# safe-autonomous-systems/fluidgym

Measured on AMD Instinct MI355X. Metric: env-steps/sec (batched) + pressure-Poisson HBM GB/s vs roofline, 1/2/4/8 GPUs, higher is better.
Workload: dtype f32; 1 GPU; ChannelJet2D-v0 (2D channel stand-in for 'cylinder Re=100 256x128'), 64 envs/GPU, 25 PISO steps/env step, random jets, stirred by a body force N(0,2.0) redrawn every env step; global_batch=64, parallelism=env-sharded x1, 1 bcast + 1 all_gather per step (RCCL), lanes_per_gpu=2, workload_modified=True, capped_solves=0, floor_released_solves=0, advection_solver_form=two-brick, velocity_solver=on-chip Jacobi sweeps (policy advection_jacobi; 11972 solves settled by

## Files before the change

### fluidgym_amd/csrc/fg_api.hip

```cpp
#include <stdio.h>
#include <string.h>

#include <cmath>
#include <string>
#include <vector>

#include <stdlib.h>

#include "fg_internal.h"
#include "fg_bicg.h"

static thread_local std::string g_last_error;
void fg_set_error(const std::string& msg) { g_last_error = msg; }

extern "C" int fg_abi_version(void) { return FG_ABI_VERSION; }
extern "C" const char* fg_last_error(void) { return g_last_error.c_str(); }

static FgBounds make_bounds(const fg_state* s, int channel) {
    FgBounds b;
    for (int f = 0; f < 6; ++f) {
        b.vel[f] = s->bvel[f];
        b.scal[f] = s->bscal[f];
        b.scalar_bc[f] = s->cfg.scalar_bc[f][channel < 0 ? 0 : channel];
    }
    return b;
}

static int check_bound(const fg_state* s, bool need_scalar) {
    FG_REQUIRE(s->velocity && s->pressure, FG_ERR_NOT_BOUND, "velocity/pressure not bound (fg_bind)");
    for (int f = 0; f < 2 * s->grid.dims; ++f) {
        if (!s->grid.fixed[f]) continue;
        FG_REQUIRE(s->bvel[f], FG_ERR_NOT_BOUND, "boundary velocity of a FIXED face not bound");
        if (need_scalar) FG_REQUIRE(s->bscal[f], FG_ERR_NOT_BOUND, "boundary scalar of a FIXED face not bound");
    }
    if (need_scalar) FG_REQUIRE(s->scalar, FG_ERR_NOT_BOUND, "passive scalar not bound");
    return FG_OK;
}

extern "C" int fg_create(const fg_config* cfg, const fg_real* hx, const fg_real* hy, const fg_real* hz, fg_handle* out) {
    FG_REQUIRE(cfg && out && hx && hy, FG_ERR_INVALID_ARG, "fg_create: null argument");
    FG_REQUIRE(cfg->dims == 2 || cfg->dims == 3, FG_ERR_INVALID_ARG, "dims must be 2 or 3");
    FG_REQUIRE(cfg->dims == 2 || hz, FG_ERR_INVALID_ARG, "hz required in 3-D");
    FG_REQUIRE(cfg->nx >= 3 && cfg->ny >= 3 && (cfg->dims == 2 ? cfg->nz == 1 : cfg->nz >= 3), FG_ERR_INVALID_ARG,
               "block needs >= 3 cells per axis (nz = 1 in 2-D)");
    FG_REQUIRE(cfg->batch >= 1, FG_ERR_INVALID_ARG, "batch must be >= 1");
    FG_REQUIRE(cfg->n_scalars >= 0 && cfg->n_scalars <= FG_MAX_SCALARS, FG_ERR_INVALID_ARG, "bad n_scalars");
    for (int a = 0; a < cfg->dims; ++a)
        FG_REQUIRE(cfg->face_type[2 * a] == cfg->face_type[2 * a + 1], FG_ERR_INVALID_ARG,
                   "a FIXED face needs a FIXED partner (CloseBoundary closes both, domain_structs.cpp:1981-2002)");
    FG_REQUIRE((long long)cfg->nx * cfg->ny * cfg->nz * cfg->batch * 6 < (1LL << 31), FG_ERR_UNSUPPORTED,
               "index space exceeds int32 (reference index_t is int32 as well)");
    FG_HIP_CHECK(hipSetDevice(cfg->device));

    fg_state* s = new fg_state();
    memset(s, 0, sizeof(*s));
    fg_switches_read(s);
    s->cfg = *cfg;
    FgGrid& g = s->grid;
    g.dims = cfg->dims; g.nx = cfg->nx; g.ny = cfg->ny; g.nz = cfg->nz;
    g.n = cfg->nx * cfg->ny * cfg->nz; g.B = cfg->batch;
    for (int f = 0; f < 6; ++f) g.fixed[f] = (f < 2 * cfg->dims) ? (cfg->face_type[f] == FG_FIXED) : 0;
    s->vec = (!FG_F64 && cfg->nx % 4 == 0) ? 4 : 1;
    s->viscosity = 0.f;

    const fg_real* hsrc[3] = {hx, hy, hz};
    const int hn[3] = {cfg->nx, cfg->ny, cfg->nz};
    for (int a = 0; a < 3; ++a) {
        std::vector<fg_real> h(hn[a], 1.f), rh(hn[a], 1.f);
        if (a < cfg->dims)
            for (int i = 0; i < hn[a]; ++i) {
                if (!(hsrc[a][i] > 0.f)) { delete s; fg_set_error("cell widths must be positive"); return FG_ERR_INVALID_ARG; }
                h[i] = hsrc[a][i]; rh[i] = 1.f / hsrc[a][i];
            }
        FG_HIP_CHECK(hipMalloc(&s->d_h[a], sizeof(fg_real) * hn[a]));
        FG_HIP_CHECK(hipMalloc(&s->d_rh[a], sizeof(fg_real) * hn[a]));
        FG_HIP_CHECK(hipMemcpy(s->d_h[a], h.data(), sizeof(fg_real) * hn[a], hipMemcpyHostToDevice));
        FG_HIP_CHECK(hipMemcpy(s->d_rh[a], rh.data(), sizeof(fg_real) * hn[a], hipMemcpyHostToDevice));
        g.h[a] = s->d_h[a]; g.rh[a] = s->d_rh[a];
    }
    const size_t BN = (size_t)g.B * g.n, d = g.dims;
    auto alloc = [&](fg_real** p, size_t count) -> hipError_t {
        hipError_t e = hipMalloc(p, sizeof(fg_real) * count);
        if (e == hipSuccess) e = hipMemset(*p, 0, sizeof(fg_real) * count);
        return e;
    };
    FG_HIP_CHECK(alloc(&s->A, BN));
    FG_HIP_CHECK(alloc(&s->rA, BN));
    FG_HIP_CHECK(alloc(&s->Coff, BN * 2 * d));
    FG_HIP_CHECK(alloc(&s->adv_rhs, BN * d));
    FG_HIP_CHECK(alloc(&s->vel_result, BN * d));
    FG_HIP_CHECK(alloc(&s->hvec, BN * d));
    FG_HIP_CHECK(alloc(&s->div, BN));
    FG_HIP_CHECK(alloc(&s->p_result, BN));
    FG_HIP_CHECK(alloc(&s->scal_result, BN));
    for (int i = 0; i < 8; ++i) FG_HIP_CHECK(alloc(&s->w[i], BN * d));
    const size_t nsys = (size_t)g.B * d;
    FG_HIP_CHECK(hipMalloc(&s->acc, sizeof(FgDacc) * nsys * FG_ACC_DOUBLES));
    FG_HIP_CHECK(hipMemset(s->acc, 0, sizeof(FgDacc) * nsys * FG_ACC_DOUBLES));
    FG_HIP_CHECK(hipMalloc(&s->flags, sizeof(int32_t) * nsys));
    FG_HIP_CHECK(hipMalloc(&s->info_dev, sizeof(fg_solve_info) * nsys));
    FG_HIP_CHECK(hipHostMalloc(&s->info_pinned, sizeof(fg_solve_info) * nsys));
    FG_HIP_CHECK(hipHostMalloc(&s->flags_pinned, sizeof(int32_t) * nsys));
    FG_HIP_CHECK(alloc(&s->scratch_B, (size_t)g.B * (4 + 2 * d)));
    FG_HIP_CHECK(hipMalloc(&s->d_bvel_ptrs, sizeof(fg_real*) * 6));
    FG_HIP_CHECK(hipMemset(s->d_bvel_ptrs, 0, sizeof(fg_real*) * 6));
    FG_HIP_CHECK(hipHostMalloc(&s->diag_pinned, sizeof(fg_real) * 2 * g.B));
    FG_HIP_CHECK(hipHostMalloc(&s->dt_pinned, sizeof(fg_real) * g.B));
    FG_HIP_CHECK(alloc(&s->dt_dev, g.B));
    FG_HIP_CHECK(hipMalloc(&s->env_sel_dev, sizeof(fg_env_sel) * g.B));
    s->t_rem_dev = nullptr;
#if !FG_F64
    FG_HIP_CHECK(hipMalloc(&s->t_rem_dev, sizeof(double) * g.B));
    FG_HIP_CHECK(hipMemset(s->t_rem_dev, 0, sizeof(double) * g.B));
#endif
    if (int rc = fg_poll_create(&s->poll, (int)(nsys > 2 * (size_t)g.B ? nsys : 2 * (size_t)g.B))) return rc;
    for (int k = 0; k < 4; ++k) { s->pred_bicg[k] = 2; s->pred_cg[k] = 1; }
    s->wall_forcing_axis = -1;
    s->ref64_inner = 1e-4f;
    s->fd_row_epoch = -1; s->rA_epoch = 0; s->fd_row_part_epoch = -1;
    for (int k = 0; k < 4; ++k) s->jac_hist[k] = FgJacHist{0, 0, 0};
    s->jac_solves = s->jac_fallbacks = 0;
    FG_HIP_CHECK(hipHostMalloc(&s->jac_prev, sizeof(float) * 4 * nsys));
    s->jac_rA_epoch = -1;
    FG_HIP_CHECK(hipMalloc(&s->fcg_alpha, sizeof(double) * 2 * (size_t)g.B));
    FG_HIP_CHECK(hipMemset(s->fcg_alpha, 0, sizeof(double) * 2 * (size_t)g.B));
    FG_HIP_CHECK(hipMalloc(&s->fcg_xsum, sizeof(FgDacc) * 2 * (size_t)g.B));
    FG_HIP_CHECK(hipMemset(s->fcg_xsum, 0, sizeof(FgDacc) * 2 * (size_t)g.B));
    FG_HIP_CHECK(hipMalloc(&s->fcg_lazy, sizeof(int32_t) * (size_t)g.B));
    FG_HIP_CHECK(hipMemset(s->fcg_lazy, 0, sizeof(int32_t) * (size_t)g.B));
    s->cg_return_best = 1;
    s->cg_reset_steps = 100;
    s->adv_from_result = 1;
    FG_HIP_CHECK(hipMalloc(&s->cg_acc, sizeof(FgDacc) * (size_t)g.B * 8 * 64));
    FG_HIP_CHECK(hipMemset(s->cg_acc, 0, sizeof(FgDacc) * (size_t)g.B * 8 * 64));
    FG_HIP_CHECK(hipMalloc(&s->cg_best.best_crit, sizeof(fg_real) * g.B));
    FG_HIP_CHECK(hipMalloc(&s->cg_best.saved_crit, sizeof(fg_real) * g.B));
    FG_HIP_CHECK(hipMalloc(&s->cg_best.save_at, sizeof(int32_t) * g.B));
    FG_HIP_CHECK(alloc(&s->cg_best.best_x, BN));
    *out = s;
    return FG_OK;
}

extern "C" int fg_destroy(fg_handle s) {
    if (!s) return FG_OK;
    for (int a = 0; a < 3; ++a) { (void)hipFree(s->d_h[a]); (void)hipFree(s->d_rh[a]); }
    fg_real* owned[] = {s->A, s->rA, s->Coff, s->adv_rhs, s->vel_result, s->hvec, s->div, s->p_result, s->scal_result,
                      s->scratch_B};
    for (fg_real* p : owned) (void)hipFree(p);
    for (int i = 0; i < 8; ++i) (void)hipFree(s->w[i]);
    (void)hipFree(s->acc); (void)hipFree(s->flags); (void)hipFree(s->info_dev);
    (void)hipHostFree(s->info_pinned); (void)hipHostFree(s->flags_pinned);
    fg_prof_destroy(s);
    fg_poll_destroy(&s->poll);
    (void)hipFree(s->d_bvel_ptrs); (void)hipHostFree(s->diag_pinned); (void)hipHostFree(s->dt_pinned); (void)hipFree(s->dt_dev); (void)hipFree(s->t_rem_dev); (void)hipFree(s->env_sel_dev);
    float* fd[] = {s->fd_Qx, s->fd_QxT, s->fd_Qz, s->fd_QzT, s->fd_lower, s->fd_inv, s->fd_cp};
    for (float* p : fd) if (p) (void)hipFree(p);
    if (s->fd_dct_tw) { (void)hipFree(s->fd_dct_tw); (void)hipFree(s->fd_dct_rot); }
    (void)hipFree(s->cg_acc); (void)hipFree(s->fcg_alpha); (void)hipFree(s->fcg_xsum); (void)hipFree(s->fcg_lazy);
    if (s->jac_prev) (void)hipHostFree(s->jac_prev);
    (void)hipFree(s->fd_row_part); (void)hipFree(s->fd_lam_x); (void)hipFree(s->fd_row_inv); (void)hipFree(s->fd_row_cp); (void)hipFree(s->fd_row_lower);
    (void)hipFree(s->line_inv); (void)hipFree(s->line_cp); (void)hipFree(s->ilu_d);
    (void)hipFree(s->r64_buf); (void)hipFree(s->r64_acc); (void)hipFree(s->ref64_x); (void)hipFree(s->force_uniform);
    (void)hipFree(s->fd_lam); (void)hipFree(s->helm_diag); (void)hipFree(s->helm_lower); (void)hipFree(s->helm_upper); (void)hipFree(s->helm_tmp); (void)hipFree(s->helm_lower_row); (void)hipFree(s->helm_lower_row2); (void)hipFree(s->line_inv2); (void)hipFree(s->line_cp2);
    (void)hipFree(s->cg_best.best_crit); (void)hipFree(s->cg_best.saved_crit); (void)hipFree(s->cg_best.save_at); (void)hipFree(s->cg_best.best_x);
    delete s;
    return FG_OK;
}

static int sync_bvel_ptrs(fg_state* s);
extern "C" int fg_bind(fg_handle s, int field, fg_real* ptr) {
    FG_REQUIRE(s, FG_ERR_INVALID_ARG, "null handle");
    if (field == FG_VELOCITY) s->velocity = ptr;
    else if (field == FG_PRESSURE) s->pressure = ptr;
    else if (field == FG_SCALAR) s->scalar = ptr;
    else if (field == FG_VELOCITY_SOURCE) s->velocity_source = ptr;
    else if (field == FG_VISCOSITY_FIELD) s->visc_field = ptr;
    else if (field >= FG_BOUND_VELOCITY && field < FG_BOUND_VELOCITY + 6) {
        s->bvel[field - FG_BOUND_VELOCITY] = ptr;
        return sync_bvel_ptrs(s);
    }
    else if (field >= FG_BOUND_SCALAR && field < FG_BOUND_SCALAR + 6) s->bscal[field - FG_BOUND_SCALAR] = ptr;
    else FG_REQUIRE(false, FG_ERR_INVALID_ARG, "fg_bind: unknown field id");
    return FG_OK;
}

extern "C" int fg_set_viscosity(fg_handle s, fg_real v) {
    FG_REQUIRE(s, FG_ERR_INVALID_ARG, "null handle");
    s->viscosity = v;
    return FG_OK;
}
extern "C" int fg_set_scalar_viscosity(fg_handle s, int ch, fg_real v) {
    FG_REQUIRE(s && ch >= 0 && ch < FG_MAX_SCALARS, FG_ERR_INVALID_ARG, "bad channel");
    s->scalar_viscosity[ch] = v;
    s->scalar_viscosity_set = true;
    return FG_OK;
}
extern "C" int fg_set_viscosity_batch(fg_handle s, const fg_real* nu_B) {
    FG_REQUIRE(s, FG_ERR_INVALID_ARG, "null handle");
    s->viscosity_B = nu_B;
    s->helm_pre_mask = 0;
    return FG_OK;
}
extern "C" int fg_set_scalar_viscosity_batch(fg_handle s, int ch, const fg_real* k_B) {
    FG_REQUIRE(s && ch >= 0 && ch < FG_MAX_SCALARS, FG_ERR_INVALID_ARG, "bad channel");
    s->scalar_viscosity_B[ch] = k_B;
    s->helm_pre_mask = 0;
    return FG_OK;
}

extern "C" int fg_set_fd_preconditioner(fg_handle s, const float* Qx, const float* QxT, const float* Qz, const float* QzT,
                                        const float* lower, const float* inv, const float* cp) {
    FG_REQUIRE(s && Qx && QxT && lower && inv && cp, FG_ERR_INVALID_ARG, "null argument");
    FG_REQUIRE(s->grid.fixed[2] && s->grid.fixed[3], FG_ERR_UNSUPPORTED, "FD preconditioner needs FIXED y faces");
    FG_REQUIRE(s->grid.dims == 2 || (Qz && QzT), FG_ERR_INVALID_ARG, "Qz required in 3-D");
#if !FG_F64
    FG_REQUIRE(s->grid.ny <= 640, FG_ERR_UNSUPPORTED, "FD preconditioner: at most 640 cells along y (LDS of the tridiagonal solve)");
#endif
    const size_t nx = s->grid.nx, ny = s->grid.ny, nz = s->grid.nz;
    auto up = [&](float** dst, const float* src, size_t count) -> hipError_t {
        if (*dst) (void)hipFree(*dst);
        hipError_t e = hipMalloc(dst, sizeof(float) * count);
        if (e == hipSuccess) e = hipMemcpy(*dst, src, sizeof(float) * count, hipMemcpyHostToDevice);
        return e;
    };
    FG_HIP_CHECK(up(&s->fd_Qx, Qx, nx * nx));
    FG_HIP_CHECK(up(&s->fd_QxT, QxT, nx * nx));
    if (s->grid.dims == 3) {
        FG_HIP_CHECK(up(&s->fd_Qz, Qz, nz * nz));
        FG_HIP_CHECK(up(&s->fd_QzT, QzT, nz * nz));
    }
    FG_HIP_CHECK(up(&s->fd_lower, lower, ny));
    FG_HIP_CHECK(up(&s->fd_inv, inv, nx * ny * nz));
    FG_HIP_CHECK(up(&s->fd_cp, cp, nx * ny * nz));
    s->fd_dct_x = 0;
    return FG_OK;
}

extern "C" int fg_set_return_best(fg_handle s, int on) {
    FG_REQUIRE(s, FG_ERR_INVALID_ARG, "null handle");
    s->cg_return_best = on ? 1 : 0;
    return FG_OK;
}

extern "C" int fg_set_cg_reset_steps(fg_handle s, int steps) {
    FG_REQUIRE(s && steps >= 0, FG_ERR_INVALID_ARG, "fg_set_cg_reset_steps: null handle or negative step count");
    s->cg_reset_steps = steps;
    return FG_OK;
}

extern "C" int fg_set_advection_start(fg_handle s, int from_result) {
    FG_REQUIRE(s, FG_ERR_INVALID_ARG, "null handle");
    s->adv_from_result = from_result ? 1 : 0;
    return FG_OK;
}

extern "C" int fg_set_wall_stress_forcing(fg_handle s, int axis, fg_real coef_lo, fg_real coef_hi) {
    FG_REQUIRE(s, FG_ERR_INVALID_ARG, "null handle");
    FG_REQUIRE(axis < s->grid.dims, FG_ERR_INVALID_ARG, "fg_set_wall_stress_forcing: bad axis");
    if (axis >= 0) {
        FG_REQUIRE(s->grid.fixed[2] && s->grid.fixed[3], FG_ERR_UNSUPPORTED, "fg_set_wall_stress_forcing: needs FIXED y faces (walls)");
        if (!s->force_uniform) {
            FG_HIP_CHECK(hipMalloc(&s->force_uniform, sizeof(fg_real) * (size_t)s->grid.B * s->grid.dims));
            FG_HIP_CHECK(hipMemset(s->force_uniform, 0, sizeof(fg_real) * (size_t)s->grid.B * s->grid.dims));
        }
    }
    s->wall_forcing_axis = axis; s->wall_forcing_coef[0] = coef_lo; s->wall_forcing_coef[1] = coef_hi;
    return FG_OK;
}

extern "C" int fg_set_advection_preconditioner(fg_handle s, int mode) {
    FG_REQUIRE(s, FG_ERR_INVALID_ARG, "null handle");
    FG_REQUIRE(mode >= 0 && mode <= 5, FG_ERR_INVALID_ARG, "fg_set_advection_preconditioner: mode must be 0 (off), 1 (line, always), 2 (line, fallback), 3 (Helmholtz, always), 4 (ILU(0), always) or 5 (ILU(0), fallback)");
    FG_REQUIRE(mode != 3 || s->fd_lam != nullptr, FG_ERR_INVALID_ARG, "fg_set_advection_preconditioner: mode 3 needs fg_set_fd_helmholtz");
    if (mode >= 4) { if (int rc = fg_ilu_alloc(s)) return rc; }
    else if (mode != 0)
        if (int rc = fg_line_alloc(s)) return rc;
    s->adv_precond = mode;
    return FG_OK;
}
extern "C" int fg_set_advection_jacobi(fg_handle s, int on) {
    FG_REQUIRE(s, FG_ERR_INVALID_ARG, "null handle");
    if (!s->adv_jacobi_env) s->adv_jacobi = on ? 1 : 0;
    for (int k = 0; k < 4; ++k) s->jac_hist[k] = FgJacHist{0, 0, 0};
    return FG_OK;
}
extern "C" int fg_advection_jacobi_counts(fg_handle s, int64_t* out2) {
    FG_REQUIRE(s && out2, FG_ERR_INVALID_ARG, "null argument");
    out2[0] = s->jac_solves; out2[1] = s->jac_fallbacks;
    return FG_OK;
}
extern "C" int fg_set_double_fallback(fg_handle s, int on) {
    FG_REQUIRE(s, FG_ERR_INVALID_ARG, "null handle");
    s->double_fallback = on ? 1 : 0;
    return FG_OK;
}
extern "C" int fg_ladder(fg_handle s, int64_t* out4, int32_t force_mask) {
    FG_REQUIRE(s && out4, FG_ERR_INVALID_ARG, "null argument");
    for (int k = 0; k < 4; ++k) out4[k] = s->rung_count[k];
    if (force_mask >= 0) s->ladder_force = force_mask;
    return FG_OK;
}
namespace {
struct FormsRecord {
    fg_state* s; int32_t* out; int32_t rec[FG_FORM_SLOTS] = {0};
    FormsRecord(fg_state* st, int32_t* o) : s(st), out(o) { s->forms_rec = rec; }
    ~FormsRecord() {
        s->forms_rec = nullptr;
        if (out) memcpy(out, rec, sizeof(rec));
    }
};
}

extern "C" int fg_debug_apply_preconditioner(fg_handle s, int mode, int nc, const fg_real* r, fg_real* z, int32_t* forms_out, void* stream) {
    FG_REQUIRE(s && r && z && nc >= 1 && nc <= s->grid.dims && (mode == 1 || mode == 3 || mode == 4), FG_ERR_INVALID_ARG,
               "fg_debug_apply_preconditioner: mode 1 (y-line), 3 (Helmholtz) or 4 (ILU(0)), 1 <= nc <= dims");
    hipStream_t st = (hipStream_t)stream;
    FormsRecord forms(s, forms_out);
    s->prepared.clear();
    FG_HIP_CHECK(hipMemsetAsync(s->flags, 0, sizeof(int32_t) * (size_t)s->grid.B * s->grid.dims, st));
    if (mode == 3) {
        FG_REQUIRE(s->fd_lam != nullptr, FG_ERR_UNSUPPORTED, "fg_debug_apply_preconditioner: mode 3 needs fg_set_fd_helmholtz (fp32 build)");
        FG_REQUIRE(s->adv_last_dt != nullptr, FG_ERR_INVALID_ARG, "fg_debug_apply_preconditioner: mode 3 needs a velocity fg_setup_advection first");
        if (int rc = fg_helm_factor(s, s->adv_last_dt, fg_nu(s), 1, 1, nc, st)) return rc;
        if (int rc = fg_fd_helmholtz_apply(s, nc, r, z, st)) return rc;
    } else if (mode == 4) {
// ... 147 lines not shown
            if (int rc = fg_launch_wall_forcing(s, (hipStream_t)stream)) return rc;
        a.force = s->wall_forcing_axis >= 0 ? s->force_uniform : nullptr;
        a.visc = s->visc_field;
        a.nu = fg_nu(s);
        a.rA = s->rA;
        s->adv_last_dt = dt_B;
        s->rA_epoch++;
        s->jac_rA_epoch = s->rA_epoch;
#if !FG_F64
        if (fg_fd_rowmean_ok(s) && s->vec == 4 && (s->grid.nx & 63) == 0) {
            if (!s->fd_row_part) FG_HIP_CHECK(hipMalloc(&s->fd_row_part, sizeof(float) * (size_t)s->grid.B * s->grid.ny * (s->grid.nx / 64)));
            a.row_part = s->fd_row_part;
            s->fd_row_part_epoch = s->rA_epoch;
        }
#endif
        if (buoy_axis >= 0) {
            a.buoy_T = s->scalar; a.buoy_stride = (long)s->cfg.n_scalars * s->grid.n; a.buoy_axis = buoy_axis; a.buoy_factor = buoy_factor;
            a.source_w = s->velocity_source;
        }
    }
    return fg_launch_adv_build(s, make_bounds(s, channel), a, (hipStream_t)stream);
}

static int advection_solve(fg_state* s, FgBicgArgs a, fg_solve_info* info, hipStream_t st, int for_scalar = 0, int channel = 0, bool* spec_ran = nullptr);

extern "C" int fg_solve_advection(fg_handle s, int for_scalar, int channel, fg_real tol, int max_iterations,
                                  fg_solve_info* info_host, void* stream) {
    FG_REQUIRE(s, FG_ERR_INVALID_ARG, "null handle");
    FgBicgArgs a;
    a.diag = s->A; a.off = s->Coff; a.rhs = s->adv_rhs;
    a.dt = s->cur_dt;
    a.tol = tol; a.max_iterations = max_iterations;
    if (for_scalar) { a.x = s->scal_result; a.nc = 1; a.use_x0 = 0; a.kind = 0; }
    else { a.x = s->vel_result; a.nc = s->grid.dims; a.use_x0 = s->adv_from_result; }
    return advection_solve(s, a, info_host, (hipStream_t)stream, for_scalar, channel);
}

extern "C" int fg_copy_scalar_result_to_blocks(fg_handle s, int channel, void* stream) {
    FG_REQUIRE(s && s->scalar, FG_ERR_NOT_BOUND, "scalar not bound");
    const int n = s->grid.n;
    if (s->cfg.n_scalars == 1) return fg_launch_copy_active(s, s->cur_dt, s->scal_result, s->scalar, 1, (hipStream_t)stream);
    FG_HIP_CHECK(hipMemcpy2DAsync(s->scalar + (size_t)channel * n, sizeof(fg_real) * n * s->cfg.n_scalars, s->scal_result,
                                  sizeof(fg_real) * n, sizeof(fg_real) * n, s->grid.B, hipMemcpyDeviceToDevice,
                                  (hipStream_t)stream));
    return FG_OK;
}

extern "C" int fg_setup_pressure_matrix(fg_handle s, void* stream) {
    FG_REQUIRE(s, FG_ERR_INVALID_ARG, "null handle");
    s->rA_epoch++;
    return fg_launch_pressure_setup(s, s->cur_dt, (hipStream_t)stream);
}

extern "C" int fg_setup_pressure_rhs(fg_handle s, const fg_real* dt_B, void* stream) {
    FG_REQUIRE(s && dt_B, FG_ERR_INVALID_ARG, "null argument");
    if (int rc = check_bound(s, false)) return rc;
    hipStream_t st = (hipStream_t)stream;
    if (int rc = fg_launch_h(s, dt_B, s->vel_result, st)) return rc;
    return fg_launch_div(s, make_bounds(s, 0), dt_B, s->hvec, s->div, st);
}

struct SpecH { fg_state* s; const fg_real* dt; const fg_step_options* opt; hipStream_t st; };
static int spec_h(void* p) {
    const SpecH* c = static_cast<const SpecH*>(p);
    fg_state* s = c->s;
    if (int rc = fg_launch_h(s, c->dt, s->vel_result, c->st)) return rc;
    return fg_launch_div(s, make_bounds(s, 0), c->dt, s->hvec, s->div, c->st, !c->opt->pressure_warm_start,
                         c->opt->pressure_method == FG_SOLVER_FDCG && s->fd_Qx != nullptr);
}

static int launch_corrector(fg_state* s, const fg_real* dt, const FgCgOutcome& o, bool last, hipStream_t st) {
    const bool mean_folded = last && o.mean_ready;
    FG_REQUIRE(!o.lazy_z || !last || mean_folded, FG_ERR_UNSUPPORTED, "fg_piso_step: an unmaterialised pressure without its folded mean");
    if (last && !mean_folded)
        if (int rc = fg_launch_mean_sub(s, dt, s->p_result, s->pressure, st)) return rc;
    const FgMeanRef mean = {s->fcg_xsum, s->info_dev, s->pressure, o.marks_valid ? s->fcg_lazy : nullptr, s->fcg_alpha};
    const FgLazyRef lazy = {s->fcg_lazy, s->fcg_alpha, last ? s->p_result : nullptr};
    const fg_real* p = o.lazy_z ? o.lazy_z : ((last && !mean_folded) ? s->pressure : s->p_result);
    return fg_launch_correct(s, dt, s->rA, s->hvec, p, s->vel_result, st, last ? s->velocity : nullptr, mean_folded ? &mean : nullptr, o.lazy_z ? &lazy : nullptr);
}

struct SpecCorrect { fg_state* s; const fg_real* dt; bool last; hipStream_t st; };
static int spec_correct(void* p, const FgCgOutcome& o) {
    const SpecCorrect* c = static_cast<const SpecCorrect*>(p);
    return launch_corrector(c->s, c->dt, o, c->last, c->st);
}

static int solve_pressure(fg_state* s, const fg_real* dt, int method, fg_real tol, int max_iterations, int use_previous,
                          fg_solve_info* info_host, hipStream_t st, bool finalize = true, int kind = 2, FgCgOutcome* out = nullptr,
                          FgCgSpec spec = FgCgSpec{}) {
    int rc = FG_OK;
    FgCgOutcome own;
    if (!out) out = &own;
    if (method == FG_SOLVER_CG || method == FG_SOLVER_FDCG) {
        FgCgArgs a;
        a.rA = s->rA; a.b = s->div; a.x = s->p_result;
        a.r = s->w[0]; a.p = s->w[1]; a.Ap = s->w[2];
        a.dt = dt; a.tol = tol; a.max_iterations = max_iterations; a.use_x0 = use_previous;
        a.reset_steps = s->cg_reset_steps;
        a.precond = (method == FG_SOLVER_FDCG);
        a.kind = kind;
        a.check_every = a.precond ? 2 : 16;
        a.lazy_ok = finalize ? 0 : 1;
        a.spec = spec;
#if !FG_F64
        if (s->ref64_outer > 0) a.lazy_ok = 0;
#endif
        rc = fg_cg_solve(s, a, info_host, st, out);
#if !FG_F64
        if (s->ref64_outer > 0 && (rc == FG_OK || rc == FG_ERR_NOT_CONVERGED)) rc = fg_refine64_pressure(s, a, info_host, st, out);
        if (s->double_fallback && (rc == FG_ERR_NOT_FINITE || (s->ladder_force & 2))) {
            std::vector<fg_solve_info> tmp;
            fg_solve_info* info = info_host;
            if (!info) { tmp.assign(s->info_pinned, s->info_pinned + s->grid.B); info = tmp.data(); }
            s->rung_count[2] += 1;
            rc = fg_rung64_cg(s, a, info, (s->ladder_force & 2) != 0, st, out);
        }
#endif
    } else {
        fg_set_error("fg_solve_pressure: only FG_SOLVER_CG drives the PISO step (Jacobi/RBGS are smoothers)");
        return FG_ERR_UNSUPPORTED;
    }
    if (rc != FG_OK && rc != FG_ERR_NOT_CONVERGED) return rc;
    if (finalize)
        if (int rc2 = fg_launch_mean_sub(s, dt, s->p_result, s->pressure, st)) return rc2;
    return rc;
}

extern "C" int fg_solve_pressure(fg_handle s, int method, fg_real tol, int max_iterations, int use_previous,
                                 fg_solve_info* info_host, void* stream) {
    FG_REQUIRE(s, FG_ERR_INVALID_ARG, "null handle");
    if (int rc = check_bound(s, false)) return rc;
    return solve_pressure(s, s->cur_dt, method, tol, max_iterations, use_previous, info_host, (hipStream_t)stream);
}

extern "C" int fg_set_pressure_refinement(fg_handle s, int32_t max_corrections, fg_real target_tol, fg_real inner_relative_tol) {
    FG_REQUIRE(s, FG_ERR_INVALID_ARG, "null handle");
    FG_REQUIRE(!FG_F64 || max_corrections <= 0, FG_ERR_UNSUPPORTED, "fg_set_pressure_refinement: the fp64 build solves in fp64 already");
    FG_REQUIRE(max_corrections <= 0 || (target_tol > 0 && inner_relative_tol > 0 && inner_relative_tol < 1), FG_ERR_INVALID_ARG,
               "fg_set_pressure_refinement: tolerances must be positive, the relative one below 1");
    s->ref64_outer = max_corrections > 0 ? max_corrections : 0;
    s->ref64_tol = (float)target_tol; s->ref64_inner = (float)inner_relative_tol;
    return FG_OK;
}

extern "C" int fg_correct_velocity(fg_handle s, void* stream) {
    FG_REQUIRE(s, FG_ERR_INVALID_ARG, "null handle");
    if (int rc = check_bound(s, false)) return rc;
    return fg_launch_correct(s, s->cur_dt, s->rA, s->hvec, s->pressure, s->vel_result, (hipStream_t)stream);
}

extern "C" int fg_copy_velocity_result_to_blocks(fg_handle s, void* stream) {
    FG_REQUIRE(s && s->velocity, FG_ERR_NOT_BOUND, "velocity not bound");
    return fg_launch_copy_active(s, s->cur_dt, s->vel_result, s->velocity, s->grid.dims, (hipStream_t)stream);
}
extern "C" int fg_copy_velocity_result_from_blocks(fg_handle s, void* stream) {
    FG_REQUIRE(s && s->velocity, FG_ERR_NOT_BOUND, "velocity not bound");
    return fg_launch_copy_active(s, nullptr, s->velocity, s->vel_result, s->grid.dims, (hipStream_t)stream);
}

static int max_iters(const fg_solve_info* info, int n) {
    int m = -1;
    for (int i = 0; i < n; ++i) m = info[i].used_iterations > m ? info[i].used_iterations : m;
    return m;
}

static int advection_solve(fg_state* s, FgBicgArgs a, fg_solve_info* info, hipStream_t st, int for_scalar, int channel, bool* spec_ran) {
    a.precond = (s->adv_precond == 1) ? 1 : (s->adv_precond == 3 ? 2 : (s->adv_precond == 4 ? 3 : 0));
    if (a.precond == 2 && !for_scalar && s->visc_field) a.precond = 0;
    if (a.precond == 2) {
        a.nu = fg_nu(s, for_scalar, channel);
        a.wall_lo = for_scalar ? (s->cfg.scalar_bc[2][channel] == FG_DIRICHLET) : 1;
        a.wall_hi = for_scalar ? (s->cfg.scalar_bc[3][channel] == FG_DIRICHLET) : 1;
    }
    const int nsys = s->grid.B * a.nc;
    std::vector<fg_solve_info> info_own;
    if (!info) { info_own.resize(nsys); info = info_own.data(); }
    int rc = fg_bicgstab_solve(s, a, info, st, spec_ran);
    bool failed = (rc == FG_ERR_NOT_CONVERGED || rc == FG_ERR_NOT_FINITE) || (s->ladder_force & 1);
#if !FG_F64
    if (failed && s->double_fallback && rc != FG_ERR_HIP) {
        s->rung_count[0] += 1;
        rc = fg_rung64_bicgstab(s, a, info, (s->ladder_force & 1) != 0, st);
        if (rc != FG_OK && rc != FG_ERR_NOT_CONVERGED && rc != FG_ERR_NOT_FINITE) return rc;
        failed = (rc != FG_OK) || (s->ladder_force & 4);
    }
#endif
    if (failed && (s->adv_precond == 2 || s->adv_precond == 5)) {
        s->line_retries += 1;
        s->rung_count[1] += 1;
        a.precond = s->adv_precond == 5 ? 3 : 1; a.use_x0 = 0;
        rc = fg_bicgstab_solve(s, a, info, st);
    }
    (void)nsys;
    return rc;
}

extern "C" int fg_piso_step(fg_handle s, const fg_real* dt_B, const fg_step_options* opt, int32_t* stats_host,
                            void* stream) {
    FG_REQUIRE(s && dt_B && opt, FG_ERR_INVALID_ARG, "null argument");
    const bool scalar = opt->advect_scalar && s->cfg.n_scalars > 0;
    if (int rc = check_bound(s, scalar)) return rc;
    FG_REQUIRE(opt->buoyancy_axis < s->grid.dims, FG_ERR_INVALID_ARG, "bad buoyancy axis");
    FG_REQUIRE(opt->buoyancy_axis < 0 || (s->velocity_source && s->scalar), FG_ERR_NOT_BOUND,
               "buoyancy needs velocity source and scalar bound");
    hipStream_t st = (hipStream_t)stream;
    const int B = s->grid.B, d = s->grid.dims;
    std::vector<fg_solve_info> info((size_t)B * d);
    int32_t stats[4] = {-1, -1, -1, -1};
    struct DropHelmRecord { fg_state* s; ~DropHelmRecord() { s->helm_pre_mask = 0; } } drop_helm_record{s};
    int status = FG_OK;
    auto soft = [&](int rc) {
        if (rc == FG_ERR_NOT_CONVERGED) { status = rc; return FG_OK; }
        return rc;
    };
#if !FG_F64
    const bool sweeps_first = s->adv_linesweep && s->grid.dims == 2 && s->jac_hist[0].skip == 0 && s->jac_hist[1].skip == 0;
    if (scalar && s->cfg.n_scalars == 1 && s->adv_precond == 3 && s->fd_lam && !s->visc_field && !sweeps_first) {
        const FgNu nu2[2] = {fg_nu(s, 1, 0), fg_nu(s)};
        const int wlo[2] = {s->cfg.scalar_bc[2][0] == FG_DIRICHLET, 1}, whi[2] = {s->cfg.scalar_bc[3][0] == FG_DIRICHLET, 1};
        if (int rc = fg_helm_factor_pair(s, dt_B, nu2, wlo, whi, st)) return rc;
    }
#endif
    if (scalar) {
        FgRange range_scalar("scalar_advection");
        for (int ch = 0; ch < s->cfg.n_scalars; ++ch) {
            if (int rc = fg_setup_advection(s, dt_B, 1, ch, stream)) return rc;
            FgBicgArgs a;
            a.diag = s->A; a.off = s->Coff; a.rhs = s->adv_rhs; a.x = s->scal_result; a.nc = 1;
            a.dt = dt_B; a.tol = opt->advection_tol; a.max_iterations = opt->max_iterations; a.use_x0 = 0; a.kind = 0;
            if (int rc = soft(advection_solve(s, a, info.data(), st, 1, ch))) return rc;
            const int m = max_iters(info.data(), B);
            stats[0] = m > stats[0] ? m : stats[0];
            s->ctr.add(0, info.data(), B);
            const int n = s->grid.n;
            if (s->cfg.n_scalars == 1) {
                if (int rc = fg_launch_copy_active(s, dt_B, s->scal_result, s->scalar, 1, st)) return rc;
            } else {
                (void)n;
                fg_set_error("multi-channel scalar copy with inactive envs not implemented");
                return FG_ERR_UNSUPPORTED;
            }
        }
    }
    fg_range_push("velocity_assembly_and_solve");
    struct PopOnce { bool armed = true; void fire() { if (armed) { fg_range_pop(); armed = false; } } ~PopOnce() { fire(); } } range_velocity;
    if (int rc = setup_advection(s, dt_B, 0, 0, stream, opt->buoyancy_axis, opt->buoyancy_factor)) return rc;
    bool h_div_ran = false;
    {
        FgBicgArgs a;
        a.diag = s->A; a.off = s->Coff; a.rhs = s->adv_rhs; a.x = s->vel_result; a.nc = d;
        a.dt = dt_B; a.tol = opt->advection_tol; a.max_iterations = opt->max_iterations; a.use_x0 = s->adv_from_result;
        SpecH spec_h_ctx = {s, dt_B, opt, st};
        if (opt->corrector_steps > 0) a.spec = FgSpecHook{spec_h, &spec_h_ctx};
        if (int rc = soft(advection_solve(s, a, info.data(), st, 0, 0, &h_div_ran))) return rc;
        stats[1] = max_iters(info.data(), B * d);
        s->ctr.add(1, info.data(), B * d);
    }
    range_velocity.fire();
    for (int c = 0; c < opt->corrector_steps; ++c) {
        FgRange range_corr(c == 0 ? "pressure_corrector_0" : "pressure_corrector_1+");
        const bool last = (c + 1 == opt->corrector_steps);
        if (!(c == 0 && h_div_ran)) {
            if (int rc = fg_launch_h(s, dt_B, s->vel_result, st)) return rc;
            if (int rc = fg_launch_div(s, make_bounds(s, 0), dt_B, s->hvec, s->div, st, !opt->pressure_warm_start,
                                       opt->pressure_method == FG_SOLVER_FDCG && s->fd_Qx != nullptr))
                return rc;
        }
        SpecCorrect spec_ctx = {s, dt_B, last, st};
        FgCgOutcome outcome;
        if (int rc = soft(solve_pressure(s, dt_B, opt->pressure_method, opt->pressure_tol, opt->max_iterations, opt->pressure_warm_start ? 1 : 0,
                                         info.data(), st, false, c == 0 ? 0 : 1, &outcome, FgCgSpec{spec_correct, &spec_ctx})))
            return rc;
        if (c < 2) { stats[2 + c] = max_iters(info.data(), B); s->ctr.add(2 + c, info.data(), B); }
        if (!outcome.spec_done)
            if (int rc = launch_corrector(s, dt_B, outcome, last, st)) return rc;
    }
    if (opt->corrector_steps <= 0)
        if (int rc = fg_launch_copy_active(s, dt_B, s->vel_result, s->velocity, d, st)) return rc;
    if (stats_host) memcpy(stats_host, stats, sizeof(stats));
    s->ctr.piso_steps += 1;
    return status;
}

extern "C" int fg_config_dump(fg_handle s, char* buf, int n) {
    FG_REQUIRE(s && buf && n > 0, FG_ERR_INVALID_ARG, "fg_config_dump: bad argument");
    std::string out = std::string("{\"build\": \"") + (FG_F64 ? "f64" : "f32") + "\"";
    fg_switches_json(s, out);
    const std::pair<const char*, long long> state[] = {
        {"fast_transform_x", s->fd_dct_x}, {"fd_preconditioner", s->fd_Qx ? 1 : 0}, {"helmholtz", s->fd_lam ? 1 : 0}, {"advection_preconditioner", s->adv_precond},
        {"advection_from_result", s->adv_from_result}, {"return_best", s->cg_return_best}, {"cg_reset_steps", s->cg_reset_steps}, {"double_fallback", s->double_fallback},
        {"wall_forcing_axis", s->wall_forcing_axis}, {"first_iterate_polls", s->fcg_first_polls}, {"unstored_pressure_solves", s->fcg_unstored},
        {"jacobi_speculation_misses", s->jac_spec_missed}, {"jacobi_floor_released", s->jac_floor_released}, {"pressure_refinement_corrections", s->ref64_corrections}};
    for (const auto& kv : state) fg_json_put(out, kv.first, kv.second);
    return fg_json_out(out + "}", buf, n);
}

extern "C" int fg_solver_unconverged(fg_handle s, int64_t* out4) {
    FG_REQUIRE(s != nullptr && out4 != nullptr, FG_ERR_INVALID_ARG, "fg_solver_unconverged: bad argument");
    for (int k = 0; k < 4; ++k) out4[k] = s->ctr.unconv[k];
    return FG_OK;
}

extern "C" int fg_solver_counters(fg_handle s, int64_t* out13, int32_t reset) {
    FG_REQUIRE(s != nullptr, FG_ERR_INVALID_ARG, "fg_solver_counters: null handle");
    if (out13) s->ctr.write(out13);
    if (reset) s->ctr.reset();
    return FG_OK;
}

extern "C" int fg_single_step(fg_handle s, const fg_sim_options* o, int32_t* out, fg_real* flux_host, void* stream);
extern "C" int fg_multi_step(fg_handle s, const fg_sim_options* o, int32_t n, const fg_real* const* bvel_schedule, int32_t* out_6n,
                             fg_real* flux_host, int32_t* steps_done, void* stream) {
    FG_REQUIRE(s && o && out_6n && n >= 0, FG_ERR_INVALID_ARG, "fg_multi_step: bad argument");
    if (steps_done) *steps_done = 0;
    for (int k = 0; k < n; ++k) {
        if (bvel_schedule)
            for (int f = 0; f < 2 * s->grid.dims; ++f)
                if (const fg_real* p = bvel_schedule[(size_t)k * 6 + f])
                    if (int rc = fg_bind(s, FG_BOUND_VELOCITY + f, const_cast<fg_real*>(p))) return rc;
        if (int rc = fg_single_step(s, o, out_6n + 6 * (size_t)k, flux_host, stream)) return rc;
        if (steps_done) *steps_done = k + 1;
        if (out_6n[6 * (size_t)k + 5] == 0 && !s->cg_return_best) break;
    }
    return FG_OK;
}

static inline bool is_close_zero(double a) { return std::fabs(a) <= 1e-8; }

extern "C" int fg_single_step(fg_handle s, const fg_sim_options* o, int32_t* out, fg_real* flux_host, void* stream) {
    fg_htrace("single_step_in");
    FgRange range_sim("fg_single_step");
    FG_REQUIRE(s && o && out, FG_ERR_INVALID_ARG, "null argument");
    if (int rc = check_bound(s, o->step.advect_scalar && s->cfg.n_scalars > 0)) return rc;
    hipStream_t st = (hipStream_t)stream;
    const int B = s->grid.B;
    const FgBounds bnd = make_bounds(s, 0);
    std::vector<double> t_rem(B, (double)o->time_step);
    int32_t stats[4] = {-1, -1, -1, -1};
    int substeps = 0, all_ok = 1;
    bool first = true;
    int fixed_left = o->adaptive ? 0 : (o->substeps > 0 ? o->substeps : 1);
    for (;;) {
        bool any = false;
        if (o->adaptive) {
            for (int b = 0; b < B; ++b) any = any || (t_rem[b] > 0 && !is_close_zero(t_rem[b]));
        } else {
            any = fixed_left > 0;
        }
        if (!any) break;
        auto advance = [&](int b, fg_real max_vel) -> fg_real {
            fg_real ts = 0.f;
            if (!o->adaptive) {
                ts = o->time_step;
            } else if (t_rem[b] > 0 && !is_close_zero(t_rem[b])) {
                const double mv = (double)max_vel;
                const double max_ts = is_close_zero(mv) ? t_rem[b] : (double)o->cfl / mv;
                double tsd;
                if (max_ts >= t_rem[b]) tsd = t_rem[b];
                else tsd = t_rem[b] / (double)(long long)std::ceil(t_rem[b] / max_ts);
                t_rem[b] -= tsd;
                ts = (fg_real)tsd;
            }
            return ts;
        };
        auto flux_guard = [&]() -> int {
            fg_real worst = 0.f;
            for (int b = 0; b < B; ++b) {
                if (flux_host) flux_host[b] = s->diag_pinned[b];
                const fg_real a = std::fabs(s->diag_pinned[b]);
                worst = (a > worst || a != a) ? a : worst;
            }
            if (!(worst <= o->flux_balance_tol)) {
                fg_set_error("Domain boundary fluxes not balanced, cannot proceed with simulation step.");
                return FG_ERR_FLUX_BALANCE;
            }
            return FG_OK;
        };
        bool deferred = false;
        FgPollOut po_cfl = FgPollOut{nullptr, 0};
        if (o->adaptive || first) {
            const FgPollOut po = fg_poll_next(&s->poll);
            po_cfl = po;
            if (first && !o->adaptive) { if (int rc = fg_launch_flux_balance(s, bnd, s->diag_pinned, st, FgPollOut{po.seq, po.value})) return rc; }
            if (o->adaptive) {
                deferred = po.gran != nullptr && s->dev_dt && s->t_rem_dev != nullptr;
                const FgDtRule rule = deferred ? FgDtRule{s->t_rem_dev, s->dt_dev, (float)o->cfl, (double)o->time_step, first ? 1 : 0}
                                               : FgDtRule{nullptr, nullptr, 0.f, 0.0, 0};
                if (int rc = fg_launch_max_velocity(s, bnd, s->scratch_B + B, st, s->diag_pinned + B, po.seq ? FgPollOut{po.seq + B, po.value, po.gran} : po,
                                                    first ? s->scratch_B : nullptr, first ? s->diag_pinned : nullptr, rule))
                    return rc;
            }
            fg_htrace("maxvel_launched");
            if (!deferred) {
                if (o->adaptive && po.gran) {
                    if (int rc = fg_poll_wait_words(&s->poll, po, 12 * B, first ? 2 * B : B, st)) return rc;
                    for (int b = 0; b < B; ++b) {
                        s->diag_pinned[B + b] = fg_poll_word_float(&s->poll, 12 * B + b);
                        if (first) s->diag_pinned[b] = fg_poll_word_float(&s->poll, 13 * B + b);
                    }
                } else if (int rc = fg_poll_wait(&s->poll, po, o->adaptive ? B : 0, o->adaptive ? 1 : B, st)) return rc;
                fg_htrace("maxvel_poll_done");
                if (first) if (int rc = flux_guard()) return rc;
            }
        }
        if (!deferred)
            for (int b = 0; b < B; ++b) s->dt_pinned[b] = advance(b, o->adaptive ? s->diag_pinned[B + b] : (fg_real)0);
        const bool folded = o->outflow_mask && fg_outflow_folds(s, o->outflow_mask);
        const bool dt_by_value = folded && B <= 64 && !deferred;
        if (!dt_by_value && !deferred) FG_HIP_CHECK(hipMemcpyAsync(s->dt_dev, s->dt_pinned, sizeof(fg_real) * B, hipMemcpyHostToDevice, st));
        if (o->outflow_mask) {
            for (int f = 0; f < 2 * s->grid.dims; ++f)
                if ((o->outflow_mask >> f) & 1) FG_REQUIRE(s->grid.fixed[f], FG_ERR_INVALID_ARG, "outflow face is not FIXED");
            if (!folded)
                for (int f = 0; f < 2 * s->grid.dims; ++f)
                    if ((o->outflow_mask >> f) & 1)
                        if (int rc = fg_launch_outflow(s, f, o->outflow_velm[f >> 1], s->dt_dev, st)) return rc;
            fg_real velm3[3] = {o->outflow_velm[0], o->outflow_velm[1], o->outflow_velm[2]};
            if (int rc = fg_launch_balance(s, bnd, o->outflow_mask, (fg_real)0.01 * o->outflow_tol, s->dt_dev, st, folded ? o->outflow_mask : 0, velm3,
                                           dt_by_value ? s->dt_pinned : nullptr))
                return rc;
        }
        int rc = fg_piso_step(s, s->dt_dev, &o->step, stats, stream);
        if (rc == FG_ERR_NOT_CONVERGED) all_ok = 0;
        else if (rc != FG_OK) return rc;
        if (deferred) {
            if (int rc2 = fg_poll_wait_words(&s->poll, po_cfl, 12 * B, first ? 2 * B : B, st)) return rc2;
            for (int b = 0; b < B; ++b) {
                s->diag_pinned[B + b] = fg_poll_word_float(&s->poll, 12 * B + b);
                if (first) s->diag_pinned[b] = fg_poll_word_float(&s->poll, 13 * B + b);
            }
            if (first) if (int rc2 = flux_guard()) return rc2;
            for (int b = 0; b < B; ++b) s->dt_pinned[b] = advance(b, s->diag_pinned[B + b]);
        }
        ++substeps;
        first = false;
        if (!o->adaptive) --fixed_left;
        if (substeps >= (o->max_substeps > 0 ? o->max_substeps : 100000)) break;
    }
    fg_htrace("single_step_out");
    for (int i = 0; i < 4; ++i) out[i] = stats[i];
    out[4] = substeps;
    out[5] = all_ok;
    return FG_OK;
}

extern "C" int fg_make_divergence_free(fg_handle s, fg_real tol, int max_iterations, fg_solve_info* info_host,
                                       void* stream) {
    FG_REQUIRE(s, FG_ERR_INVALID_ARG, "null handle");
    if (int rc = check_bound(s, false)) return rc;
    s->cur_dt = nullptr;
    hipStream_t st = (hipStream_t)stream;
    const size_t BN = (size_t)s->grid.B * s->grid.n;
    std::vector<fg_real> ones(BN, 1.f);
    FG_HIP_CHECK(hipMemcpyAsync(s->rA, ones.data(), sizeof(fg_real) * BN, hipMemcpyHostToDevice, st));
    s->rA_epoch++;
    FG_HIP_CHECK(hipStreamSynchronize(st));
    if (int rc = fg_launch_copy_active(s, nullptr, s->velocity, s->hvec, s->grid.dims, st)) return rc;
    if (int rc = fg_launch_div(s, make_bounds(s, 0), nullptr, s->hvec, s->div, st)) return rc;
    int rc = solve_pressure(s, nullptr, FG_SOLVER_CG, tol, max_iterations, 0, info_host, st);
    if (rc != FG_OK && rc != FG_ERR_NOT_CONVERGED) return rc;
    if (int rc2 = fg_launch_correct(s, nullptr, s->rA, s->hvec, s->pressure, s->vel_result, st)) return rc2;
    if (int rc2 = fg_launch_copy_active(s, nullptr, s->vel_result, s->velocity, s->grid.dims, st)) return rc2;
    return rc;
}

extern "C" int fg_reset_solver_state(fg_handle s, void* stream) {
    FG_REQUIRE(s && s->velocity, FG_ERR_NOT_BOUND, "velocity not bound");
    for (int k = 0; k < 4; ++k) s->jac_hist[k] = FgJacHist{0, 0, 0};
    FG_HIP_CHECK(hipMemsetAsync(s->p_result, 0, sizeof(fg_real) * (size_t)s->grid.B * s->grid.n, (hipStream_t)stream));
    return fg_launch_copy_active(s, nullptr, s->velocity, s->vel_result, s->grid.dims, (hipStream_t)stream);
}

extern "C" int fg_solver_hints(fg_handle s, int32_t* hints12, int32_t set) {
    FG_REQUIRE(s != nullptr && hints12 != nullptr, FG_ERR_INVALID_ARG, "fg_solver_hints: bad argument");
    for (int k = 0; k < 4; ++k) {
        FgJacHist& H = s->jac_hist[k];
        if (set) { H.sweeps = hints12[3 * k]; H.skip = hints12[3 * k + 1]; H.fails = hints12[3 * k + 2]; }
        else { hints12[3 * k] = H.sweeps; hints12[3 * k + 1] = H.skip; hints12[3 * k + 2] = H.fails; }
    }
    return FG_OK;
}

extern "C" int fg_get_buffer(fg_handle s, int which, fg_real** out_ptr, int64_t* out_count) {
    FG_REQUIRE(s && out_ptr && out_count, FG_ERR_INVALID_ARG, "null argument");
    const int64_t BN = (int64_t)s->grid.B * s->grid.n, d = s->grid.dims;
    switch (which) {
        case FG_BUF_A: *out_ptr = s->A; *out_count = BN; break;
        case FG_BUF_C_OFF: *out_ptr = s->Coff; *out_count = BN * 2 * d; break;
        case FG_BUF_ADV_RHS: *out_ptr = s->adv_rhs; *out_count = BN * d; break;
        case FG_BUF_VEL_RESULT: *out_ptr = s->vel_result; *out_count = BN * d; break;
        case FG_BUF_H: *out_ptr = s->hvec; *out_count = BN * d; break;
        case FG_BUF_DIV: *out_ptr = s->div; *out_count = BN; break;
        case FG_BUF_P_RESULT: *out_ptr = s->p_result; *out_count = BN; break;
        case FG_BUF_SCALAR_RESULT: *out_ptr = s->scal_result; *out_count = BN; break;
        default:
            if (which >= 100 && which < 108) { *out_ptr = s->w[which - 100]; *out_count = BN * d; break; }
            FG_REQUIRE(false, FG_ERR_INVALID_ARG, "unknown buffer id");
    }
    return FG_OK;
}

extern "C" int fg_read_buffer(fg_handle s, int which, fg_real* dst, void* stream) {
    fg_real* src = nullptr;
    int64_t count = 0;
    if (int rc = fg_get_buffer(s, which, &src, &count)) return rc;
    FG_REQUIRE(dst, FG_ERR_INVALID_ARG, "null destination");
    FG_HIP_CHECK(hipMemcpyAsync(dst, src, sizeof(fg_real) * count, hipMemcpyDeviceToDevice, (hipStream_t)stream));
    return FG_OK;
}

extern "C" int fg_poisson_apply(fg_handle s, const fg_real* rA, const fg_real* x, fg_real* y, void* stream) {
    FG_REQUIRE(s && rA && x && y, FG_ERR_INVALID_ARG, "null argument");
    return fg_poisson_apply_launch(s, rA, x, y, (hipStream_t)stream);
}

extern "C" int fg_poisson_jacobi(fg_handle s, const fg_real* rA, const fg_real* b, fg_real* x, int n_sweeps, fg_real omega,
                                 void* stream) {
    FG_REQUIRE(s && rA && b && x && n_sweeps >= 0, FG_ERR_INVALID_ARG, "bad argument");
    hipStream_t st = (hipStream_t)stream;
    fg_real* buf[2] = {x, s->w[5]};
    for (int i = 0; i < n_sweeps; ++i)
        if (int rc = fg_poisson_jacobi_launch(s, rA, b, buf[i & 1], buf[(i + 1) & 1], omega, st)) return rc;
    if (n_sweeps & 1)
        FG_HIP_CHECK(hipMemcpyAsync(x, s->w[5], sizeof(fg_real) * (size_t)s->grid.B * s->grid.n, hipMemcpyDeviceToDevice, st));
    return FG_OK;
}

extern "C" int fg_poisson_rbgs(fg_handle s, const fg_real* rA, const fg_real* b, fg_real* x, int n_sweeps, fg_real omega,
                               void* stream) {
    FG_REQUIRE(s && rA && b && x && n_sweeps >= 0, FG_ERR_INVALID_ARG, "bad argument");
    hipStream_t st = (hipStream_t)stream;
    for (int i = 0; i < n_sweeps; ++i) {
        if (int rc = fg_poisson_rbgs_launch(s, rA, b, x, omega, 0, st)) return rc;
        if (int rc = fg_poisson_rbgs_launch(s, rA, b, x, omega, 1, st)) return rc;
    }
    return FG_OK;
}

extern "C" int fg_poisson_cg(fg_handle s, const fg_real* rA, const fg_real* b, fg_real* x, fg_real tol, int max_iterations,
                             int use_x0, fg_solve_info* info_host, void* stream) {
    FG_REQUIRE(s && rA && b && x, FG_ERR_INVALID_ARG, "null argument");
    FgCgArgs a;
    a.rA = rA; a.b = b; a.x = x;
    a.r = s->w[0]; a.p = s->w[1]; a.Ap = s->w[2];
    a.dt = nullptr; a.tol = tol; a.max_iterations = max_iterations; a.use_x0 = use_x0;
    a.reset_steps = 100;
    a.precond = 0;
    a.check_every = (tol > 0.f) ? 16 : (1 << 30);
    return fg_cg_solve(s, a, info_host, (hipStream_t)stream);
}

extern "C" int fg_poisson_fdcg(fg_handle s, const fg_real* rA, const fg_real* b, fg_real* x, fg_real tol, int max_iterations,
                               int use_x0, fg_solve_info* info_host, void* stream) {
    FG_REQUIRE(s && rA && b && x, FG_ERR_INVALID_ARG, "null argument");
    FgCgArgs a;
    a.rA = rA; a.b = b; a.x = x;
    a.r = s->w[0]; a.p = s->w[1]; a.Ap = s->w[2];
    a.dt = nullptr; a.tol = tol; a.max_iterations = max_iterations; a.use_x0 = use_x0;
    a.reset_steps = 0;
    a.precond = 1;
    a.check_every = (tol > 0.f) ? 2 : (1 << 30);
    return fg_cg_solve(s, a, info_host, (hipStream_t)stream);
}

extern "C" int fg_coords_to_transforms(const float* coords, float* transforms, int dims, int nx, int ny, int nz,
                                       void* stream) {
    FG_REQUIRE(coords && transforms && (dims == 2 || dims == 3), FG_ERR_INVALID_ARG, "bad argument");
#if FG_F64
    fg_set_error("fg_coords_to_transforms is an fp32 entry point: use libfluidgym_hip.so");
    return FG_ERR_UNSUPPORTED;
#else
    return fg_metrics_launch(coords, transforms, dims, nx, ny, nz, (hipStream_t)stream);
#endif
}
```

### fluidgym_amd/csrc/fg_envrestore.hip

```cpp
#include <vector>

#include "fg_internal.h"

namespace {

constexpr int ER_TX = 64, ER_TY = 4, ER_PASSES = 4, ER_ROWS = ER_TY * ER_PASSES;

template <typename T>
__global__ __launch_bounds__(ER_TX * ER_TY) void k_env_restore(T* __restrict__ dst, const T* __restrict__ bank,
                                                               const fg_env_sel* __restrict__ sel, int C, int ez, int ey, int ex,
                                                               int tiles_x, int signed_components) {
    const fg_env_sel r = sel[blockIdx.y];
    const int tx = (int)(blockIdx.x % (unsigned)tiles_x), rg = (int)(blockIdx.x / (unsigned)tiles_x);
    const int rows = C * ez * ey;
    const size_t per_env = (size_t)rows * ex;
    T* __restrict__ d = dst + (size_t)r.env * per_env;
    const T* __restrict__ b = bank + (size_t)r.src * per_env;
    const int x = tx * ER_TX + (int)threadIdx.x;
    int xs = x - r.shift_x;
    if (xs < 0) xs += ex;
    if (r.flip_x) xs = ex - 1 - xs;
#pragma unroll
    for (int k = 0; k < ER_PASSES; ++k) {
        const int row = rg * ER_ROWS + k * ER_TY + (int)threadIdx.y;
        if (x < ex && row < rows) {
            const int y = row % ey, cz = row / ey;
            const int z = cz % ez, c = cz / ez;
            int zs = z - r.shift_z;
            if (zs < 0) zs += ez;
            if (r.flip_z) zs = ez - 1 - zs;
            const T v = b[((size_t)(c * ez + zs) * ey + y) * ex + xs];
            const bool neg = signed_components && ((c == 0 && r.flip_x) || (c == 2 && r.flip_z));
            d[(size_t)row * ex + x] = neg ? -v : v;
        }
    }
}

template <typename T>
__global__ __launch_bounds__(256) void k_env_reset_solver(const T* __restrict__ velocity, T* __restrict__ vel_result,
                                                          T* __restrict__ p_result, const fg_env_sel* __restrict__ sel, long n, int dims) {
    const int env = sel[blockIdx.y].env;
    const long dn = (long)dims * n;
    const T* __restrict__ u = velocity + (size_t)env * dn;
    T* __restrict__ ur = vel_result + (size_t)env * dn;
    T* __restrict__ pr = p_result + (size_t)env * n;
#pragma unroll
    for (int k = 0; k < 4; ++k) {
        const long i = ((long)blockIdx.x * 4 + k) * 256 + threadIdx.x;
        if (i < dn) ur[i] = u[i];
        if (i < n) pr[i] = (T)0;
    }
}

int check_envs(const fg_state* s, const fg_env_sel* sel, int32_t n_sel, const char* who) {
    const int B = s->grid.B;
    FG_REQUIRE(sel != nullptr, FG_ERR_INVALID_ARG, std::string(who) + ": null selection");
    FG_REQUIRE(n_sel >= 1 && n_sel <= B, FG_ERR_INVALID_ARG, std::string(who) + ": n_sel must be in 1..batch");
    FG_REQUIRE(n_sel <= 65535, FG_ERR_UNSUPPORTED, std::string(who) + ": at most 65535 envs per call");
    std::vector<char> seen((size_t)B, 0);
    for (int i = 0; i < n_sel; ++i) {
        FG_REQUIRE(sel[i].env >= 0 && sel[i].env < B, FG_ERR_INVALID_ARG, std::string(who) + ": env index out of range");
        FG_REQUIRE(!seen[sel[i].env], FG_ERR_INVALID_ARG, std::string(who) + ": an env is named twice");
        seen[sel[i].env] = 1;
    }
    return FG_OK;
}

}

extern "C" int fg_env_restore_field(fg_handle s, int which_field, const fg_real* bank, int32_t S, const fg_env_sel* sel, int32_t n_sel,
                                    int32_t signed_components, void* stream) {
    FG_REQUIRE(s != nullptr, FG_ERR_INVALID_ARG, "fg_env_restore_field: null handle");
    FG_REQUIRE(bank != nullptr && S >= 1, FG_ERR_INVALID_ARG, "fg_env_restore_field: null bank or S < 1");
    if (int rc = check_envs(s, sel, n_sel, "fg_env_restore_field")) return rc;
    const FgGrid& g = s->grid;
    fg_real* dst = nullptr;
    int C = 0, vector_field = 0, ext[3] = {g.nx, g.ny, g.nz};
    if (which_field == FG_VELOCITY) { dst = s->velocity; C = g.dims; vector_field = 1; }
    else if (which_field == FG_PRESSURE) { dst = s->pressure; C = 1; }
    else if (which_field == FG_SCALAR) { dst = s->scalar; C = s->cfg.n_scalars; }
    else if (which_field == FG_VELOCITY_SOURCE) { dst = s->velocity_source; C = g.dims; vector_field = 1; }
    else if (which_field >= FG_BOUND_VELOCITY && which_field < FG_BOUND_VELOCITY + 2 * g.dims) {
        const int f = which_field - FG_BOUND_VELOCITY;
        dst = s->bvel[f]; C = g.dims; vector_field = 1; ext[f >> 1] = 1;
    } else if (which_field >= FG_BOUND_SCALAR && which_field < FG_BOUND_SCALAR + 2 * g.dims) {
        const int f = which_field - FG_BOUND_SCALAR;
        dst = s->bscal[f]; C = s->cfg.n_scalars; ext[f >> 1] = 1;
    } else FG_REQUIRE(false, FG_ERR_INVALID_ARG, "fg_env_restore_field: unknown field id");
    FG_REQUIRE(signed_components == 0 || (signed_components == 1 && vector_field), FG_ERR_INVALID_ARG,
               "fg_env_restore_field: signed_components is 0, or 1 on a vector field");
    const bool x_periodic = !g.fixed[0] && !g.fixed[1], z_periodic = g.dims == 3 && !g.fixed[4] && !g.fixed[5];
    for (int i = 0; i < n_sel; ++i) {
        const fg_env_sel& r = sel[i];
        FG_REQUIRE(r.src >= 0 && r.src < S, FG_ERR_INVALID_ARG, "fg_env_restore_field: src index out of range");
        FG_REQUIRE((r.flip_x | 1) == 1 && (r.flip_z | 1) == 1, FG_ERR_INVALID_ARG, "fg_env_restore_field: a flip is 0 or 1");
        FG_REQUIRE(g.dims == 3 || (r.flip_z == 0 && r.shift_z == 0), FG_ERR_INVALID_ARG, "fg_env_restore_field: flip_z / shift_z on a 2-D grid");
        FG_REQUIRE(r.shift_x >= 0 && r.shift_x < g.nx && r.shift_z >= 0 && r.shift_z < g.nz, FG_ERR_INVALID_ARG,
                   "fg_env_restore_field: a shift must be in [0, n)");
        FG_REQUIRE(x_periodic || (r.flip_x == 0 && r.shift_x == 0), FG_ERR_INVALID_ARG, "fg_env_restore_field: flip / shift along x, which has FIXED faces");
        FG_REQUIRE(g.dims == 2 || z_periodic || (r.flip_z == 0 && r.shift_z == 0), FG_ERR_INVALID_ARG,
                   "fg_env_restore_field: flip / shift along z, which has FIXED faces");
    }
    FG_REQUIRE(dst != nullptr && C > 0, FG_ERR_NOT_BOUND, "fg_env_restore_field: the field is not bound");
    hipStream_t st = (hipStream_t)stream;
    FG_HIP_CHECK(hipMemcpyAsync(s->env_sel_dev, sel, sizeof(fg_env_sel) * n_sel, hipMemcpyHostToDevice, st));
    const int ex = ext[0], ey = ext[1], ez = ext[2];
    const int tiles_x = (ex + ER_TX - 1) / ER_TX;
    const long row_groups = ((long)C * ez * ey + ER_ROWS - 1) / ER_ROWS;
    hipLaunchKernelGGL(k_env_restore<fg_real>, dim3((unsigned)(tiles_x * row_groups), (unsigned)n_sel), dim3(ER_TX, ER_TY), 0, st, dst, bank,
                       (const fg_env_sel*)s->env_sel_dev, C, ez, ey, ex, tiles_x, (int)signed_components);
    FG_HIP_CHECK(hipGetLastError());
    return FG_OK;
}

extern "C" int fg_env_reset_solver_state(fg_handle s, const fg_env_sel* sel, int32_t n_sel, void* stream) {
    FG_REQUIRE(s != nullptr, FG_ERR_INVALID_ARG, "fg_env_reset_solver_state: null handle");
    if (int rc = check_envs(s, sel, n_sel, "fg_env_reset_solver_state")) return rc;
    FG_REQUIRE(s->velocity != nullptr, FG_ERR_NOT_BOUND, "velocity not bound");
    hipStream_t st = (hipStream_t)stream;
    FG_HIP_CHECK(hipMemcpyAsync(s->env_sel_dev, sel, sizeof(fg_env_sel) * n_sel, hipMemcpyHostToDevice, st));
    const long n = s->grid.n, dn = n * s->grid.dims;
    hipLaunchKernelGGL(k_env_reset_solver<fg_real>, dim3((unsigned)((dn + 1023) / 1024), (unsigned)n_sel), dim3(256), 0, st,
                       (const fg_real*)s->velocity, s->vel_result, s->p_result, (const fg_env_sel*)s->env_sel_dev, n, s->grid.dims);
    FG_HIP_CHECK(hipGetLastError());
    return FG_OK;
}

extern "C" int fg_mb_env_restore_field(fg_mb_handle, int, const fg_real*, int32_t, const fg_env_sel*, int32_t, int32_t, void*) {
    fg_set_error("fg_mb_env_restore_field: a multi-block handle has no per-env restore");
    return FG_ERR_UNSUPPORTED;
}

extern "C" int fg_mb_env_reset_solver_state(fg_mb_handle, const fg_env_sel*, int32_t, void*) {
    fg_set_error("fg_mb_env_reset_solver_state: a multi-block handle has no per-env restore");
    return FG_ERR_UNSUPPORTED;
}
```

### fluidgym_amd/csrc/fg_internal.h

```cpp
#pragma once
#include <hip/hip_runtime.h>
#include <hip/hip_ext.h>
#include <math.h>
#include <stdint.h>
#include <cstring>
#include <string>
#include <type_traits>

#include "../../include/fluidgym_hip.h"
#include "fg_switches.h"

#ifdef FG_REAL_DOUBLE
struct alignas(16) fg_real4 { double x, y, z, w; };
__host__ __device__ __forceinline__ fg_real4 make_fg_real4(double x, double y, double z, double w) { fg_real4 r; r.x = x; r.y = y; r.z = z; r.w = w; return r; }
#define FG_F64 1
#define FG_FMAX fmax
#define FG_FABS fabs
#define FG_SQRT sqrt
#else
typedef float4 fg_real4;
#define make_fg_real4 make_float4
#define FG_F64 0
#define FG_FMAX fmaxf
#define FG_FABS fabsf
// ... 473 lines not shown
__device__ __forceinline__ void fg_poll_publish_infos(const FgPollOut& p, fg_solve_info* mirror, const fg_solve_info* info, int sys, bool valid,
                                                      int first, int n, uint32_t* stage) {
    if (p.gran) {
        uint32_t w[2] = {0u, 0u};
        if (valid) { const fg_solve_info v = info[sys]; w[0] = __float_as_uint((float)v.final_residual); w[1] = fg_info_word(v); }
        fg_poll_publish_records<2>(p, first, n, sys - first, w, valid, stage);
    } else if (valid) {
        mirror[sys] = info[sys];
        fg_poll_publish(p, sys);
    }
}
__device__ __forceinline__ void fg_poll_publish_infos_waves(const FgPollOut& p, fg_solve_info* mirror, const fg_solve_info* info, int sys, bool valid,
                                                            int first, int n, uint32_t* stage) {
    if (mirror) fg_poll_publish_infos(p, mirror, info, sys, valid && (threadIdx.x & 63) == 0, first, n, stage);
}
__device__ __forceinline__ void fg_poll_publish(const FgPollOut& p, int i) {
    if (p.seq) __hip_atomic_store(p.seq + i, p.value, __ATOMIC_RELEASE, __HIP_MEMORY_SCOPE_SYSTEM);
}
#endif
struct FgPoll {
    int32_t* seq;
    int n; int32_t epoch; int spin, words;
    unsigned long long* gran; int n_gran;
};
int fg_poll_create(FgPoll* P, int n);
void fg_poll_destroy(FgPoll* P);
FgPollOut fg_poll_next(FgPoll* P);
int fg_poll_wait(FgPoll* P, const FgPollOut& out, int first, int count, hipStream_t st);
int fg_poll_wait_words(FgPoll* P, const FgPollOut& out, int first, int count, hipStream_t st);
int fg_poll_wait_infos(FgPoll* P, const FgPollOut& out, int first, int count, fg_solve_info* pinned, hipStream_t st);
int fg_poll_wait_active(FgPoll* P, const FgPollOut& out, int first, int count, fg_solve_info* pinned, hipStream_t st);
struct fg_state;
int fg_solve_infos_settle(fg_state* s, int count, bool fresh, hipStream_t st);
int fg_solve_infos_report(const fg_state* s, int count, fg_solve_info* info_host, int* used_max);
inline uint32_t fg_poll_word(const FgPoll* P, int i) { return (uint32_t)(__atomic_load_n(P->gran + i, __ATOMIC_RELAXED) & 0xffffffffull); }
inline float fg_poll_word_float(const FgPoll* P, int i) { const uint32_t u = fg_poll_word(P, i); float f; memcpy(&f, &u, 4); return f; }
inline void fg_poll_info(const FgPoll* P, int sys, fg_solve_info* out) {
    const uint32_t w = fg_poll_word(P, 2 * sys + 1);
    out->final_residual = fg_poll_word_float(P, 2 * sys);
    out->used_iterations = (int32_t)(w >> 2) - 1; out->converged = (w >> 1) & 1; out->is_finite = w & 1;
}
void fg_htrace(const char* tag);
void fg_range_push(const char* name);
void fg_range_pop();
struct FgRange { explicit FgRange(const char* name) { fg_range_push(name); } ~FgRange() { fg_range_pop(); } FgRange(const FgRange&) = delete; FgRange& operator=(const FgRange&) = delete; };

struct FgBest {
    fg_real* best_crit;
    fg_real* saved_crit;
    int32_t* save_at;
    fg_real* best_x;
};
#ifdef __HIPCC__
__device__ __forceinline__ void fg_best_decide(const FgBest& best, int b, fg_real crit, int it) {
    if (it >= 1 && crit < 0.5f * best.best_crit[b]) {
        best.best_crit[b] = crit;
        best.saved_crit[b] = crit;
        best.save_at[b] = it;
    }
}
#endif

struct FgCounters {
    long long sum[4] = {0, 0, 0, 0}, n[4] = {0, 0, 0, 0}, piso_steps = 0;
    long long unconv[4] = {0, 0, 0, 0};
    int max[4] = {0, 0, 0, 0};
    void add(int kind, const fg_solve_info* info, int count) {
        for (int i = 0; i < count; ++i) {
            const int it = info[i].used_iterations;
            if (it < 0 && info[i].final_residual == 0.f) continue;
            const int v = it + 1;
            sum[kind] += v; n[kind] += 1; max[kind] = v > max[kind] ? v : max[kind];
            if (!info[i].converged) unconv[kind] += 1;
        }
    }
    void reset() { *this = FgCounters(); }
    void write(int64_t* out) const {
        for (int k = 0; k < 4; ++k) { out[k] = sum[k]; out[4 + k] = n[k]; out[8 + k] = max[k]; }
        out[12] = piso_steps;
    }
};

struct FgPrepared {
    int bicg_nc; const fg_real* bicg_dt;
    int cg_ns, cg_best; const fg_real* cg_dt;
    int cg_start;
    void clear() { *this = FgPrepared{}; }
    void set_bicg(int nc, const fg_real* dt) { clear(); bicg_nc = nc; bicg_dt = dt; }
    void set_cg(int ns, int best, const fg_real* dt) { clear(); cg_ns = ns; cg_best = best; cg_dt = dt; }
    bool cg_for(const fg_real* dt) const { return cg_ns > 0 && cg_dt == dt; }
    void set_cg_start(int form) { cg_start = form; }
    bool take_bicg(int nc, const fg_real* dt) { const bool ready = bicg_nc == nc && bicg_dt == dt; clear(); return ready; }
    int take_cg(int ns, int best, const fg_real* dt) {
        const int got = (cg_ns == ns && cg_best == best && cg_dt == dt) ? cg_start : -1; clear(); return got;
    }
};

struct FgNu {
    fg_real v = 0; const fg_real* per_env = nullptr;
#ifdef __HIPCC__
    __device__ __forceinline__ fg_real at(int b) const { return per_env ? per_env[b] : v; }
#endif
    bool same(const FgNu& o) const { return v == o.v && per_env == o.per_env; }
};

struct fg_state {
    fg_config cfg;
    FgGrid grid;
    int vec;
    fg_real viscosity;
    fg_real scalar_viscosity[FG_MAX_SCALARS];
    bool scalar_viscosity_set;
    const fg_real* viscosity_B;
    const fg_real* scalar_viscosity_B[FG_MAX_SCALARS];
    fg_real* d_h[3];
    fg_real* d_rh[3];
    fg_real* velocity;
    fg_real* pressure;
    fg_real* scalar;
    fg_real* velocity_source;
    fg_real* visc_field;
    fg_real* bvel[6];
    fg_real* bscal[6];
    fg_real* A;
    fg_real* rA;
    fg_real* Coff;
    fg_real* adv_rhs;
    fg_real* vel_result;
    fg_real* hvec;
    fg_real* div;
    fg_real* p_result;
    fg_real* scal_result;
    fg_real* w[8];
    FgDacc* acc;
    int32_t* flags;
    fg_solve_info* info_dev;
    fg_solve_info* info_pinned;
    int32_t* flags_pinned;
    fg_real* scratch_B;
    FgProf prof;
    FgDacc* cg_acc;
    FgBest cg_best;
    int cg_return_best;
    int cg_reset_steps;
    int adv_from_result;
    int adv_precond; long long line_retries;
    int wall_forcing_axis; fg_real wall_forcing_coef[2]; fg_real* force_uniform;
    FG_SB_SWITCHES(FG_SW_MEMBER)
    double* fcg_alpha; FgDacc* fcg_xsum;
    int32_t* fcg_lazy;
    long jac_spec_missed;
    long jac_floor_released = 0;
    long fcg_unstored, fcg_first_polls;
    fg_real* line_inv; fg_real* line_cp;
    fg_real* ilu_d;
    int double_fallback; int ladder_force; long long rung_count[4];
    double* r64_buf; FgDacc* r64_acc;
    int ref64_outer; float ref64_tol, ref64_inner; double* ref64_x; long ref64_corrections;
    float* fd_Qx; float* fd_QxT; float* fd_Qz; float* fd_QzT; float* fd_lower; float* fd_inv; float* fd_cp;
    float* fd_lam; float* helm_diag; float* helm_lower; float* helm_upper; float* helm_tmp;
    float* helm_lower_row; float helm_rs; int helm_cb;
    float* line_inv2; float* line_cp2; float* helm_lower_row2; int helm_pre_mask; const fg_real* helm_pre_dt; FgNu helm_pre_nu[2]; int helm_pre_walls[2][2]; int helm_set;
    int fd_dct_x; float2* fd_dct_tw; float2* fd_dct_rot; float fd_dct_fwd[2]; float fd_dct_inv[2];
    float* fd_lam_x; float* fd_row_inv; float* fd_row_cp; float* fd_row_lower; long fd_row_epoch; mutable long rA_epoch;
    float* fd_row_part; long fd_row_part_epoch;
    int32_t* forms_rec;
    const fg_real* adv_last_dt;
    fg_real** d_bvel_ptrs;
    fg_real* diag_pinned;
    fg_real* dt_pinned;
    fg_real* dt_dev;
    double* t_rem_dev;
    int pred_bicg[4], pred_cg[4];
    int adv_jacobi, adv_jacobi_env; FgJacHist jac_hist[4]; float* jac_prev;
    long long jac_solves, jac_fallbacks;
    long jac_rA_epoch;
    FgCounters ctr;
    const fg_real* cur_dt;
    FgPoll poll;
    mutable int maxvel_clean;
    FgPrepared prepared;
    fg_env_sel* env_sel_dev;
    size_t n_cells() const { return (size_t)grid.n; }
};
inline FgNu fg_nu(const fg_state* s, int for_scalar = 0, int channel = 0) {
    FgNu n;
    if (for_scalar && s->scalar_viscosity_B[channel]) { n.v = s->scalar_viscosity[channel]; n.per_env = s->scalar_viscosity_B[channel]; }
    else if (for_scalar && s->scalar_viscosity_set) n.v = s->scalar_viscosity[channel];
    else { n.v = s->viscosity; n.per_env = s->viscosity_B; }
    return n;
}

void fg_set_error(const std::string& msg);
#define FG_REQUIRE(cond, code, msg)  \
    do {                             \
        if (!(cond)) {               \
            fg_set_error(msg);       \
            return code;             \
        }                            \
    } while (0)
#define FG_HIP_CHECK(expr)                                                                        \
    do {                                                                                          \
        hipError_t _e = (expr);                                                                   \
        if (_e != hipSuccess) {                                                                   \
            fg_set_error(std::string(#expr) + ": " + hipGetErrorString(_e));                      \
            return FG_ERR_HIP;                                                                    \
        }                                                                                         \
    } while (0)

#if FG_F64
#define FG_DISPATCH(s, ...)                                                       \
    do {                                                                          \
        if ((s)->grid.dims == 2) { constexpr int DIMS = 2, VEC = 1; __VA_ARGS__; } \
        else { constexpr int DIMS = 3, VEC = 1; __VA_ARGS__; }                    \
    } while (0)
#else
#define FG_DISPATCH(s, ...)                                                       \
    do {                                                                          \
        if ((s)->grid.dims == 2) {                                                \
            if ((s)->vec == 4) { constexpr int DIMS = 2, VEC = 4; __VA_ARGS__; }  \
            else { constexpr int DIMS = 2, VEC = 1; __VA_ARGS__; }                \
        } else {                                                                  \
            if ((s)->vec == 4) { constexpr int DIMS = 3, VEC = 4; __VA_ARGS__; }  \
            else { constexpr int DIMS = 3, VEC = 1; __VA_ARGS__; }                \
        }                                                                         \
    } while (0)
#endif

struct FgBicgBegin { FgDacc* acc; fg_real* sc; int32_t* flags; fg_solve_info* info; int nc; };
#ifdef __HIPCC__
__device__ __forceinline__ void fg_bicg_begin_sys(const FgBicgBegin& q, const fg_real* __restrict__ dt, int sys) {
    for (int k = 0; k < FG_ACC_DOUBLES; ++k) acc_st(q.acc + ((size_t)sys * FG_ACC_DOUBLES + k), 0.0);
    sc_st(q.sc + (sys * 2), 1.f); sc_st(q.sc + (sys * 2 + 1), 1.f);
    const bool active = (dt == nullptr) || (dt[sys / q.nc] > 0.f);
    flag_st(q.flags + (sys), active ? 0 : 3);
    q.info[sys].final_residual = 0.f;
    q.info[sys].used_iterations = -1;
    q.info[sys].converged = active ? 0 : 1;
    q.info[sys].is_finite = 1;
}
#endif
struct FgAdvArgs {
    const fg_real* vel;
    const fg_real* scal;
    long scal_env_stride;
    const fg_real* source;
    const fg_real* force;
    const fg_real* dt;
    FgNu nu;
    const fg_real* visc;
    int for_scalar;
    int channel, n_scalars;
    fg_real* A; fg_real* Coff; fg_real* rhs;
    fg_real* rA;
    FgBicgBegin begin;
    const fg_real* buoy_T; long buoy_stride; int buoy_axis; fg_real buoy_factor; fg_real* source_w;
    fg_real* row_part;
};
int fg_launch_adv_build(fg_state* s, const FgBounds& bnd, const FgAdvArgs& a, hipStream_t st);
int fg_launch_wall_forcing(const fg_state* s, hipStream_t st);
int fg_launch_sgs(const fg_state* s, const FgBounds& bnd, fg_real coefficient, fg_real* out, hipStream_t st);
int fg_launch_pressure_setup(const fg_state* s, const fg_real* dt, hipStream_t st);
int fg_launch_h(fg_state* s, const fg_real* dt, const fg_real* vel_result, hipStream_t st);
int fg_launch_div(fg_state* s, const FgBounds& bnd, const fg_real* dt, const fg_real* hvec, fg_real* div, hipStream_t st,
                  bool cg_from_zero = false,
                  bool fused_fwd = false);
struct FgMeanRef { const FgDacc* sums; const fg_solve_info* info; fg_real* p_copy; const int32_t* lazy; const double* alpha; };
struct FgLazyRef { const int32_t* lazy; const double* alpha; fg_real* p_res; };
int fg_launch_correct(const fg_state* s, const fg_real* dt, const fg_real* rA, const fg_real* hvec, const fg_real* p,
                      fg_real* vel_out, hipStream_t st, fg_real* vel_copy = nullptr, const FgMeanRef* mean = nullptr, const FgLazyRef* lazy = nullptr);
struct FgDtRule { double* t_rem; fg_real* dt_out; float cfl; double time_step; int reset; };
int fg_launch_max_velocity(const fg_state* s, const FgBounds& bnd, fg_real* out_B, hipStream_t st, fg_real* mirror_B = nullptr,
                           FgPollOut poll = FgPollOut{nullptr, 0}, fg_real* flux_B = nullptr, fg_real* flux_mirror = nullptr,
                           FgDtRule rule = FgDtRule{nullptr, nullptr, 0.f, 0.0, 0});
int fg_launch_flux_balance(const fg_state* s, const FgBounds& bnd, fg_real* out_B, hipStream_t st, FgPollOut poll = FgPollOut{nullptr, 0});
int fg_launch_copy_active(const fg_state* s, const fg_real* dt, const fg_real* src, fg_real* dst, int comps, hipStream_t st);
int fg_launch_buoyancy(const fg_state* s, const fg_real* dt, const fg_real* T, long t_env_stride, fg_real* source, int axis,
                       fg_real factor, hipStream_t st);
int fg_launch_outflow(const fg_state* s, int face, fg_real velm_axis, const fg_real* dt, hipStream_t st);
int fg_launch_balance(const fg_state* s, const FgBounds& bnd, int free_mask, fg_real atol, const fg_real* dt, hipStream_t st,
                      int outflow_mask = 0, const fg_real* outflow_velm = nullptr,
                      const fg_real* dt_host_values = nullptr);
bool fg_outflow_folds(const fg_state* s, int outflow_mask);
int fg_launch_mean_sub(const fg_state* s, const fg_real* active_dt, fg_real* p, fg_real* p_copy, hipStream_t st);

int fg_poisson_apply_launch(const fg_state* s, const fg_real* rA, const fg_real* x, fg_real* y, hipStream_t st);
int fg_poisson_jacobi_launch(const fg_state* s, const fg_real* rA, const fg_real* b, const fg_real* x, fg_real* xnew,
                             fg_real omega, hipStream_t st);
int fg_poisson_rbgs_launch(const fg_state* s, const fg_real* rA, const fg_real* b, fg_real* x, fg_real omega, int color,
                           hipStream_t st);
struct FgCgOutcome {
    const fg_real* lazy_z = nullptr;
    bool mean_ready = false;
    bool marks_valid = false;
    bool spec_done = false;
};
struct FgCgSpec { int (*fn)(void* ctx, const FgCgOutcome& o) = nullptr; void* ctx = nullptr; };
struct FgCgArgs {
    const fg_real* rA; const fg_real* b; fg_real* x;
    fg_real* r; fg_real* p; fg_real* Ap;
    const fg_real* dt;
    fg_real tol; int max_iterations; int use_x0; int reset_steps;
    int check_every;
    int precond;
    int kind = 2;
    int lazy_ok = 0;
    FgCgSpec spec;
};
int fg_cg_solve(fg_state* s, const FgCgArgs& a, fg_solve_info* info_host, hipStream_t st, FgCgOutcome* out = nullptr);

struct FgSpecHook { int (*fn)(void* ctx) = nullptr; void* ctx = nullptr; };
struct FgBicgArgs {
    const fg_real* diag; const fg_real* off;
    const fg_real* rhs; fg_real* x;
    int nc;
    const fg_real* dt;
    fg_real tol; int max_iterations; int use_x0;
    int precond = 0;
    FgNu nu; int wall_lo = 1, wall_hi = 1;
    int kind = 1;
    FgSpecHook spec;
};
int fg_bicgstab_solve(fg_state* s, const FgBicgArgs& a, fg_solve_info* info_host, hipStream_t st, bool* spec_ran = nullptr);
#if !FG_F64
enum FgSweepOutcome {
    FG_SWEEP_NOT_TRIED,
    FG_SWEEP_SOLVED,
    FG_SWEEP_SOLVED_SPEC,
    FG_SWEEP_GAVE_UP,
    FG_SWEEP_SPEC_MISSED,
};
bool fg_jacobi_ok(const fg_state* s, const FgBicgArgs& a);
bool fg_linesweep_ok(const fg_state* s, const FgBicgArgs& a);
int fg_linesweep_solve(fg_state* s, const FgBicgArgs& a, fg_solve_info* info_host, hipStream_t st, FgSweepOutcome* outcome);
int fg_jacobi_solve(fg_state* s, const FgBicgArgs& a, fg_solve_info* info_host, hipStream_t st, FgSweepOutcome* outcome);
#endif
int fg_rung64_bicgstab(fg_state* s, const FgBicgArgs& a, fg_solve_info* info_host, bool all_systems, hipStream_t st);
int fg_rung64_cg(fg_state* s, const FgCgArgs& a, fg_solve_info* info_host, bool all_envs, hipStream_t st, FgCgOutcome* out);

bool fg_zmarch_ok(const fg_state* s, int* zc_out);
int fg_zmarch_apply(const fg_state* s, const fg_real* rA, const fg_real* x, fg_real* y, int zc, hipStream_t st);
int fg_zmarch_relax(const fg_state* s, const fg_real* rA, const fg_real* b, const fg_real* x, fg_real* xnew, fg_real omega,
                    int color, int zc, hipStream_t st);
int fg_zmarch_cg_ap(const fg_state* s, const fg_real* rA, const fg_real* z, const fg_real* p_in, fg_real* p_out, fg_real* Ap,
                    FgDacc* acc, int32_t* flags, fg_solve_info* info, int prof_slot, fg_real tol, int it, int first,
                    int ns, int num_base, int zc, hipStream_t st);
#define FG_PROF_SELF ((const int32_t*)(uintptr_t)1)
int fg_prof_slot(const fg_state* s, int kind, const int32_t* flags, int nsys, double bytes_per_sys,
                 double flops_per_sys, hipStream_t st);
int fg_prof_collect(fg_state* s, hipStream_t st);
void fg_prof_prefetch(fg_state* s, hipStream_t st);
void fg_prof_destroy(fg_state* s);
bool fg_fd_dct_supported(int n);
struct FgCgJudge;
int fg_fd_dct_forward(fg_state* s, const fg_real* r, fg_real* out, hipStream_t st, int batch = 0, const FgCgJudge* judge = nullptr);
int fg_fd_dct_inverse(fg_state* s, const fg_real* u, fg_real* z, const fg_real* dot_with, FgDacc* dot_acc, int dot_stride,
                      int dot_ns, hipStream_t st, int batch = 0);
#define FG_LAUNCH_P(s, slot, kernel, grid, block, shmem, st, ...)                                              \
    do {                                                                                                       \
        const int slot__ = (slot);                                                                             \
        if (slot__ >= 0)                                                                                       \
            hipExtLaunchKernelGGL(kernel, grid, block, shmem, st, (s)->prof.ev[2 * slot__],                    \
                                  (s)->prof.ev[2 * slot__ + 1], 0, __VA_ARGS__);                               \
        else                                                                                                   \
            hipLaunchKernelGGL(kernel, grid, block, shmem, st, __VA_ARGS__);                                   \
    } while (0)
int fg_fd_apply(fg_state* s, const fg_real* r, fg_real* z, FgDacc* rz_acc, int rz_stride, int rz_ns, int expect_active,
                hipStream_t st, const FgCgJudge* judge = nullptr);
struct FgCgLead;
int fg_fd_tridiag(fg_state* s, float* cur, hipStream_t st, const FgCgLead* lead, bool use_rowmean = false, const float* factor_from = nullptr, const float* factor_dt = nullptr);
bool fg_fd_tridiag_can_factor(const fg_state* s);
bool fg_fd_rowmean_ok(const fg_state* s);
int fg_refine64_pressure(fg_state* s, const FgCgArgs& a0, fg_solve_info* info_host, hipStream_t st, FgCgOutcome* out);
int fg_fd_rowmean_factor(fg_state* s, const float* rA, const float* dt, hipStream_t st, const float* row_part = nullptr, int tiles_x = 0);
int fg_fd_rowmean_prefactor(fg_state* s, const fg_real* dt, hipStream_t st);
int fg_line_alloc(fg_state* s);
int fg_ilu_alloc(fg_state* s);
int fg_ilu_factor(fg_state* s, const fg_real* diag, const fg_real* off, hipStream_t st);
int fg_ilu_apply(fg_state* s, const fg_real* diag, const fg_real* off, int nc, const fg_real* r, fg_real* z, hipStream_t st);
int fg_helm_alloc(fg_state* s);
int fg_helm_factor(fg_state* s, const fg_real* dt, FgNu nu, int wall_lo, int wall_hi, int nc, hipStream_t st, int kind = -1);
int fg_helm_factor_pair(fg_state* s, const float* dt, const FgNu nu[2], const int wall_lo[2], const int wall_hi[2], hipStream_t st);
int fg_helm_apply(fg_state* s, int nc, const float* r, float* z, hipStream_t st);
int fg_fd_helmholtz_apply(fg_state* s, int nc, const fg_real* r, fg_real* z, hipStream_t st);
int fg_line_factor(fg_state* s, const fg_real* diag, const fg_real* off, int nc, hipStream_t st);
int fg_line_apply(fg_state* s, const fg_real* diag, const fg_real* off, int nc, const fg_real* r, fg_real* z, hipStream_t st);
int fg_metrics_launch(const float* coords, float* transforms, int dims, int nx, int ny, int nz, hipStream_t st);
```

### fluidgym_amd/csrc/fg_piso.hip

```cpp
#include "fg_internal.h"
#include "fg_cg.h"
#include "fg_fftcg.h"

namespace {

template <int VEC>
__device__ __forceinline__ fg_real fg_elem_mask(int e, fg_real lo_mask_or_hi, bool is_edge_elem) {
    return is_edge_elem ? lo_mask_or_hi : 1.f;
}

template <int DIMS, int VEC>
__device__ __forceinline__ int fg_slab_index(const FgGrid& g, const FgCtx<DIMS, VEC>& c, int a) {
    if (a == 0) return c.k * g.ny + c.j;
    if (a == 1) return c.k * g.nx + c.i0;
    return c.j * g.nx + c.i0;
}
__device__ __forceinline__ int fg_slab_size(const FgGrid& g, int a) {
    return (a == 0) ? g.ny * g.nz : (a == 1) ? g.nx * g.nz : g.nx * g.ny;
}

template <int DIMS, int VEC, bool SCALAR, bool VISC = false>
__global__ __launch_bounds__(FG_BLOCK) void k_adv_build(FgGrid g, FgBounds bnd, FgAdvArgs a, int tiles_x,
                                                         int tiles_y, int tiles) {
    const FgCtx<DIMS, VEC> c = fg_make_ctx<DIMS, VEC>(g, tiles_x, tiles_y, tiles);
// ... 116 lines not shown
        for (int e = 0; e < VEC; ++e) r.v[e] = 1.f / out.v[e];
        fg_store<VEC>(a.rA + (size_t)c.b * N + c.idx, r);
#if !FG_F64
        if constexpr (DIMS == 2 && VEC == 4) {
            if (a.row_part) {
                float v = (r.v[0] + r.v[1]) + (r.v[2] + r.v[3]);
#define FG_DPP16(x, ctrl) __int_as_float(__builtin_amdgcn_update_dpp(__float_as_int(x), __float_as_int(x), ctrl, 0xf, 0xf, false))
                v += FG_DPP16(v, 0xb1);
                v += FG_DPP16(v, 0x4e);
                v += FG_DPP16(v, 0x124);
                v += FG_DPP16(v, 0x128);
#undef FG_DPP16
                if ((threadIdx.x & 15) == 0) a.row_part[((size_t)c.b * g.ny + c.j) * tiles_x + c.i0 / 64] = v;
            }
        }
#endif
    }
#pragma unroll
    for (int f = 0; f < 2 * DIMS; ++f) {
#pragma unroll
        for (int e = 0; e < VEC; ++e) out.v[e] = off[f][e] * rJ[e];
        fg_store<VEC>(a.Coff + ((size_t)c.b * 2 * DIMS + f) * N + c.idx, out);
    }
    if constexpr (SCALAR) {
        const FgVec<VEC> T = fg_load<VEC>(a.scal + (size_t)c.b * a.scal_env_stride + c.idx);
#pragma unroll
        for (int e = 0; e < VEC; ++e) out.v[e] = (J[e] * T.v[e] * rdt + bsum[0][e]) * rJ[e];
        fg_store<VEC>(a.rhs + (size_t)c.b * N + c.idx, out);
    } else {
#pragma unroll
        for (int q = 0; q < DIMS; ++q) {
            FgVec<VEC> S;
            const bool have_s = a.source != nullptr || a.buoy_T != nullptr;
            if (a.buoy_T) {
                if (q == a.buoy_axis) {
                    S = fg_load<VEC>(a.buoy_T + (size_t)c.b * a.buoy_stride + c.idx);
#pragma unroll
                    for (int e = 0; e < VEC; ++e) S.v[e] = a.buoy_factor * S.v[e];
                } else {
#pragma unroll
                    for (int e = 0; e < VEC; ++e) S.v[e] = 0.f;
                }
                fg_store<VEC>(a.source_w + ((size_t)c.b * DIMS + q) * N + c.idx, S);
            } else if (a.source) S = fg_load<VEC>(a.source + ((size_t)c.b * DIMS + q) * N + c.idx);
            const fg_real F = a.force ? a.force[c.b * DIMS + q] : 0.f;
#pragma unroll
            for (int e = 0; e < VEC; ++e)
                out.v[e] = (J[e] * u[q].v[e] * rdt + bsum[q][e]) * rJ[e] + ((have_s ? S.v[e] : 0.f) + F);
            fg_store<VEC>(a.rhs + ((size_t)c.b * DIMS + q) * N + c.idx, out);
        }
    }
}

__global__ __launch_bounds__(FG_BLOCK) void k_reciprocal(const fg_real* __restrict__ A, fg_real* __restrict__ rA,
                                                          const fg_real* __restrict__ dt, int n, int n4) {
    const int b = blockIdx.y;
    if (dt && !(dt[b] > 0.f)) return;
    const fg_real4* src = reinterpret_cast<const fg_real4*>(A + (size_t)b * n);
    fg_real4* dst = reinterpret_cast<fg_real4*>(rA + (size_t)b * n);
    for (int i = blockIdx.x * blockDim.x + threadIdx.x; i < n4; i += gridDim.x * blockDim.x) {
        const fg_real4 v = src[i];
        dst[i] = make_fg_real4(1.f / v.x, 1.f / v.y, 1.f / v.z, 1.f / v.w);
    }
    if (blockIdx.x == 0) {
        for (int i = n4 * 4 + threadIdx.x; i < n; i += blockDim.x) rA[(size_t)b * n + i] = 1.f / A[(size_t)b * n + i];
    }
}

template <int DIMS, int VEC>
__global__ __launch_bounds__(FG_BLOCK) void k_h(FgGrid g, const fg_real* __restrict__ dt,
                                                 const fg_real* __restrict__ rA_, const fg_real* __restrict__ Coff,
                                                 const fg_real* __restrict__ rhs, const fg_real* __restrict__ velr,
                                                 fg_real* __restrict__ hvec, FgCgBegin begin, int tiles_x, int tiles_y, int tiles) {
    const FgCtx<DIMS, VEC> c = fg_make_ctx<DIMS, VEC>(g, tiles_x, tiles_y, tiles);
    if (begin.acc && fg_xcd_remap(blockIdx.x, gridDim.x) % (unsigned)tiles == 0) fg_cg_begin_env(begin, dt, c.b);
    if (!(dt[c.b] > 0.f) || !c.valid) return;
    const size_t N = g.n;
    const FgVec<VEC> rA = fg_load<VEC>(rA_ + (size_t)c.b * N + c.idx);
    FgVec<VEC> off[2 * DIMS];
#pragma unroll
    for (int f = 0; f < 2 * DIMS; ++f) off[f] = fg_load<VEC>(Coff + ((size_t)c.b * 2 * DIMS + f) * N + c.idx);
#pragma unroll
    for (int q = 0; q < DIMS; ++q) {
        const size_t base = ((size_t)c.b * DIMS + q) * N;
        const FgNbr<DIMS, VEC> u = fg_gather<DIMS, VEC>(velr + base, c);
        const FgVec<VEC> r = fg_load<VEC>(rhs + base + c.idx);
        FgVec<VEC> out;
#pragma unroll
        for (int e = 0; e < VEC; ++e) {
            fg_real H = off[0].v[e] * u.xm.v[e] + off[1].v[e] * u.xp.v[e] + off[2].v[e] * u.ym.v[e] +
                      off[3].v[e] * u.yp.v[e];
            if constexpr (DIMS == 3) H += off[4].v[e] * u.zm.v[e] + off[5].v[e] * u.zp.v[e];
            out.v[e] = rA.v[e] * (r.v[e] - H);
        }
        fg_store<VEC>(hvec + base + c.idx, out);
    }
}

template <int DIMS, int VEC>
__global__ __launch_bounds__(FG_BLOCK) void k_div(FgGrid g, FgBounds bnd, const fg_real* __restrict__ dt,
                                                   const fg_real* __restrict__ hvec, fg_real* __restrict__ div, FgCgStart start,
                                                   int tiles_x, int tiles_y, int tiles) {
    const FgCtx<DIMS, VEC> c = fg_make_ctx<DIMS, VEC>(g, tiles_x, tiles_y, tiles);
    if (dt && !(dt[c.b] > 0.f)) return;
    if (!c.valid && !start.acc) return;
    const size_t N = g.n;
    const FgMetric<DIMS, VEC> m = fg_metrics<DIMS, VEC>(g, c);
    fg_real acc[VEC];
#pragma unroll
    for (int e = 0; e < VEC; ++e) acc[e] = 0.f;
#pragma unroll
    for (int ax = 0; ax < DIMS; ++ax) {
        FgVec<VEC> ctr, lo, hi;
        fg_gather_axis<DIMS, VEC>(hvec + ((size_t)c.b * DIMS + ax) * N, c, ax, ctr, lo, hi);
        const int slab = fg_slab_index<DIMS, VEC>(g, c, ax);
        const int slab_n = fg_slab_size(g, ax);
#pragma unroll
        for (int e = 0; e < VEC; ++e) {
            fg_real area, mask_lo, mask_hi;
            if (ax == 0) { area = m.hy * m.hz; mask_lo = (e == 0) ? c.mxm : 1.f; mask_hi = (e == VEC - 1) ? c.mxp : 1.f; }
            else if (ax == 1) { area = m.hx[e] * m.hz; mask_lo = c.mym; mask_hi = c.myp; }
            else { area = m.hx[e] * m.hy; mask_lo = c.mzm; mask_hi = c.mzp; }
            const int bi = slab + ((ax == 0) ? 0 : e);
            fg_real F_hi, F_lo;
            if (mask_hi != 0.f) F_hi = 0.5f * (ctr.v[e] + hi.v[e]) * area;
            else F_hi = bnd.vel[2 * ax + 1][((size_t)c.b * DIMS + ax) * slab_n + bi] * area;
            if (mask_lo != 0.f) F_lo = 0.5f * (ctr.v[e] + lo.v[e]) * area;
            else F_lo = bnd.vel[2 * ax][((size_t)c.b * DIMS + ax) * slab_n + bi] * area;
            acc[e] += F_hi - F_lo;
        }
    }
    FgVec<VEC> out;
#pragma unroll
    for (int e = 0; e < VEC; ++e) out.v[e] = acc[e];
    if (c.valid) fg_store<VEC>(div + (size_t)c.b * N + c.idx, out);
    if (start.acc) {
        __shared__ fg_real lds[4];
        fg_real part[1] = {0.f};
        if (c.valid) {
            FgVec<VEC> z;
#pragma unroll
            for (int e = 0; e < VEC; ++e) { z.v[e] = 0.f; part[0] += out.v[e] * out.v[e]; }
            fg_store<VEC>(start.x + (size_t)c.b * N + c.idx, z);
            fg_store<VEC>(start.r + (size_t)c.b * N + c.idx, out);
        }
        fg_block_sum<1>(part, lds);
        if (threadIdx.x == 0) {
            const unsigned tile = fg_xcd_remap(blockIdx.x, gridDim.x) % tiles;
            fg_acc_add(fg_acc_ptr(start.acc, c.b, 0), start.ns, tile, (double)part[0]);
        }
    }
}

template <int DIMS, int VEC>
__global__ __launch_bounds__(FG_BLOCK) void k_correct(FgGrid g, const fg_real* __restrict__ dt,
                                                       const fg_real* __restrict__ rA_, const fg_real* __restrict__ hvec,
                                                       const fg_real* __restrict__ p, fg_real* __restrict__ vel_out,
                                                       fg_real* __restrict__ vel_copy, FgMeanRef mean, FgLazyRef lazy, int tiles_x, int tiles_y, int tiles) {
    const FgCtx<DIMS, VEC> c = fg_make_ctx<DIMS, VEC>(g, tiles_x, tiles_y, tiles);
    if ((dt && !(dt[c.b] > 0.f)) || !c.valid) return;
    const size_t N = g.n;
    const FgMetric<DIMS, VEC> m = fg_metrics<DIMS, VEC>(g, c);
    const FgVec<VEC> rA = fg_load<VEC>(rA_ + (size_t)c.b * N + c.idx);
    FgNbr<DIMS, VEC> P = fg_gather<DIMS, VEC>(p + (size_t)c.b * N, c);
    if (lazy.lazy) {
        const bool on = lazy.lazy[c.b] == 1;
        const fg_real sc = on ? (fg_real)lazy.alpha[2 * c.b] : (fg_real)0;
        auto scale = [&](FgVec<VEC>& v) {
#pragma unroll
            for (int e = 0; e < VEC; ++e) v.v[e] = on ? sc * v.v[e] : (fg_real)0;
        };
        scale(P.c); scale(P.xm); scale(P.xp); scale(P.ym); scale(P.yp);
        if constexpr (DIMS == 3) { scale(P.zm); scale(P.zp); }
        if (lazy.p_res) fg_store<VEC>(lazy.p_res + (size_t)c.b * N + c.idx, P.c);
    }
    if (mean.sums) {
        const int used = mean.info[c.b].used_iterations;
        const bool first_only = mean.lazy && mean.lazy[c.b] == 1;
        const fg_real mu = first_only ? (fg_real)(mean.alpha[2 * c.b] * acc_ld(mean.sums + (2 * c.b + 1)) / (double)g.n)
                           : used < 0 ? (fg_real)0 : (fg_real)(acc_ld(mean.sums + (2 * c.b + (used & 1))) / (double)g.n);
        FgVec<VEC> pc;
#pragma unroll
        for (int e = 0; e < VEC; ++e) pc.v[e] = P.c.v[e] - mu;
        fg_store<VEC>(mean.p_copy + (size_t)c.b * N + c.idx, pc);
    }
#pragma unroll
    for (int q = 0; q < DIMS; ++q) {
        const size_t base = ((size_t)c.b * DIMS + q) * N;
        const FgVec<VEC> h = fg_load<VEC>(hvec + base + c.idx);
        FgVec<VEC> out;
#pragma unroll
        for (int e = 0; e < VEC; ++e) {
            fg_real lo, hi, fac, rh;
            if (q == 0) {
                lo = P.xm.v[e]; hi = P.xp.v[e]; rh = m.rhx[e];
                const fg_real ml = (e == 0) ? c.mxm : 1.f, mh = (e == VEC - 1) ? c.mxp : 1.f;
                fac = (ml == 0.f || mh == 0.f) ? 1.f : 0.5f;
            } else if (q == 1) {
                lo = P.ym.v[e]; hi = P.yp.v[e]; rh = m.rhy;
                fac = (c.mym == 0.f || c.myp == 0.f) ? 1.f : 0.5f;
            } else {
                lo = P.zm.v[e]; hi = P.zp.v[e]; rh = m.rhz;
                fac = (c.mzm == 0.f || c.mzp == 0.f) ? 1.f : 0.5f;
            }
            out.v[e] = h.v[e] - rA.v[e] * ((hi - lo) * fac * rh);
        }
        fg_store<VEC>(vel_out + base + c.idx, out);
        if (vel_copy) fg_store<VEC>(vel_copy + base + c.idx, out);
    }
}

#if FG_F64
typedef long long fg_bits;
__device__ __forceinline__ fg_bits fg_real_bits(fg_real v) { return __double_as_longlong(v); }
__device__ __forceinline__ fg_real fg_bits_real(fg_bits b) { return __longlong_as_double(b); }
#else
typedef int fg_bits;
__device__ __forceinline__ fg_bits fg_real_bits(fg_real v) { return __float_as_int(v); }
__device__ __forceinline__ fg_real fg_bits_real(fg_bits b) { return __int_as_float(b); }
#endif
template <int DIMS>
__device__ __forceinline__ double fg_flux_balance_block(const FgGrid& g, const FgBounds& bnd, int b) {
    double acc = 0.0;
    const int lane = threadIdx.x & 63, wave = threadIdx.x >> 6;
    for (int f = 0; f < 2 * DIMS; ++f) {
        if (!g.fixed[f]) continue;
        const int ax = f >> 1;
        const int slab_n = fg_slab_size(g, ax);
        const double sgn = (f & 1) ? 1.0 : -1.0;
        const int n0 = (ax == 0) ? g.ny : g.nx;
        const int n1 = (DIMS == 3) ? ((ax == 2) ? g.ny : g.nz) : 1;
        const fg_real* __restrict__ h0 = (ax == 0) ? g.h[1] : g.h[0];
        const fg_real* __restrict__ h1 = (DIMS == 3) ? ((ax == 2) ? g.h[1] : g.h[2]) : nullptr;
        const fg_real* __restrict__ v = bnd.vel[f] + ((size_t)b * DIMS + ax) * slab_n;
        constexpr int RU = 4, WV = FG_BLOCK / 64;
        for (int i1b = wave; i1b < n1; i1b += WV * RU) {
            for (int i0 = lane; i0 < n0; i0 += 64) {
                fg_real val[RU], a1[RU];
#pragma unroll
                for (int u = 0; u < RU; ++u) {
                    const int i1 = i1b + u * WV;
                    const bool ok = i1 < n1;
                    a1[u] = ok ? (h1 ? h1[i1] : (fg_real)1) : (fg_real)0;
                    val[u] = ok ? v[(size_t)i1 * n0 + i0] : (fg_real)0;
                }
                const fg_real w0 = h0[i0];
#pragma unroll
                for (int u = 0; u < RU; ++u) acc += sgn * (double)(val[u] * (w0 * a1[u]));
            }
        }
    }
    __shared__ double lds_fb[4];
#pragma unroll
    for (int o = 32; o > 0; o >>= 1) acc += __shfl_down(acc, o, 64);
    if ((threadIdx.x & 63) == 0) lds_fb[threadIdx.x >> 6] = acc;
    __syncthreads();
    return lds_fb[0] + lds_fb[1] + lds_fb[2] + lds_fb[3];
}
__device__ __forceinline__ void fg_publish_max(fg_real* out_B, int32_t* done_B, fg_real* mirror_B, int b, fg_real mx, const FgPollOut& poll, int B,
                                               fg_real* flux_B = nullptr, fg_real* flux_mirror = nullptr, const FgDtRule& rule = FgDtRule{nullptr, nullptr, 0.f, 0.0, 0}) {
    const int lane = threadIdx.x & 63;
    int last_of_all = 0;
    if (lane == 0) {
        if (!mirror_B) {
            atomicMax(reinterpret_cast<fg_bits*>(out_B) + b, fg_real_bits(mx));
        } else {
            fg_bits prev = atomicMax(reinterpret_cast<fg_bits*>(out_B) + b, fg_real_bits(mx));
#if FG_F64
            asm volatile("" ::"v"((int)(prev >> 32)), "v"((int)prev));
#else
            asm volatile("" ::"v"(prev));
#endif
            if (atomicAdd(done_B + b, 1) == (int)gridDim.x - 1) last_of_all = (atomicAdd(done_B + B, 1) == B - 1);
        }
    }
    if (!mirror_B) return;
    if (__shfl(last_of_all, 0, 64)) {
#if !FG_F64
        if (poll.gran) {
            for (int e = lane; e < B; e += 64) {
                const fg_bits mbits = __hip_atomic_exchange(reinterpret_cast<fg_bits*>(out_B) + e, (fg_bits)0, __ATOMIC_RELAXED, __HIP_MEMORY_SCOPE_AGENT);
                if (rule.t_rem) {
                    double tr = rule.reset ? rule.time_step : rule.t_rem[e];
                    float ts = 0.f;
                    if (tr > 0.0 && !(fabs(tr) <= 1e-8)) {
                        const double mv = (double)__uint_as_float(mbits);
                        const double max_ts = (fabs(mv) <= 1e-8) ? tr : (double)rule.cfl / mv;
                        const double tsd = (max_ts >= tr) ? tr : tr / (double)(long long)ceil(tr / max_ts);
                        tr -= tsd;
                        ts = (float)tsd;
                    }
                    rule.t_rem[e] = tr;
                    rule.dt_out[e] = ts;
                }
                fg_poll_publish_word(poll, 12 * B + e, mbits);
                if (flux_B) fg_poll_publish_word(poll, 13 * B + e, __hip_atomic_exchange(reinterpret_cast<fg_bits*>(flux_B) + e, (fg_bits)0, __ATOMIC_RELAXED, __HIP_MEMORY_SCOPE_AGENT));
                atomicExch(done_B + e, 0);
            }
            if (lane == 0) atomicExch(done_B + B, 0);
            return;
        }
#endif
        for (int e = lane; e < B; e += 64) {
            mirror_B[e] = fg_bits_real(__hip_atomic_exchange(reinterpret_cast<fg_bits*>(out_B) + e, (fg_bits)0, __ATOMIC_RELAXED, __HIP_MEMORY_SCOPE_AGENT));
            if (flux_B) flux_mirror[e] = fg_bits_real(__hip_atomic_exchange(reinterpret_cast<fg_bits*>(flux_B) + e, (fg_bits)0, __ATOMIC_RELAXED, __HIP_MEMORY_SCOPE_AGENT));
            atomicExch(done_B + e, 0);
        }
        if (lane == 0) {
            atomicExch(done_B + B, 0);
            fg_poll_publish(poll, 0);
        }
    }
}

template <int DIMS>
__global__ __launch_bounds__(FG_BLOCK) void k_max_velocity(FgGrid g, FgBounds bnd, const fg_real* __restrict__ vel,
                                                            fg_real* __restrict__ out_B, int32_t* __restrict__ done_B,
                                                            fg_real* __restrict__ mirror_B, FgPollOut poll, fg_real* flux_B, fg_real* flux_mirror, FgDtRule rule) {
    const int b = blockIdx.y;
    const size_t N = g.n;
    fg_real mx = 0.f;
    for (int idx = blockIdx.x * blockDim.x + threadIdx.x; idx < g.n; idx += gridDim.x * blockDim.x) {
        const int i = idx % g.nx;
        const int j = (idx / g.nx) % g.ny;
        const int k = idx / (g.nx * g.ny);
        const fg_real rh[3] = {g.rh[0][i], g.rh[1][j], DIMS == 3 ? g.rh[2][k] : 1.f};
#pragma unroll
        for (int q = 0; q < DIMS; ++q) mx = FG_FMAX(mx, FG_FABS(vel[((size_t)b * DIMS + q) * N + idx] * rh[q]));
    }
    {
#pragma unroll
        for (int f = 0; f < 2 * DIMS; ++f) {
            if (!g.fixed[f]) continue;
            const int ax = f >> 1;
            const int slab_n = fg_slab_size(g, ax);
            const int edge = (f & 1) ? ((ax == 0) ? g.nx - 1 : (ax == 1) ? g.ny - 1 : g.nz - 1) : 0;
            for (int s = blockIdx.x * blockDim.x + threadIdx.x; s < slab_n; s += gridDim.x * blockDim.x) {
                int i, j, k;
                if (ax == 0) { i = edge; j = s % g.ny; k = s / g.ny; }
                else if (ax == 1) { j = edge; i = s % g.nx; k = s / g.nx; }
                else { k = edge; i = s % g.nx; j = s / g.nx; }
                const fg_real rh[3] = {g.rh[0][i], g.rh[1][j], DIMS == 3 ? g.rh[2][k] : 1.f};
#pragma unroll
                for (int q = 0; q < DIMS; ++q)
                    mx = FG_FMAX(mx, FG_FABS(bnd.vel[f][((size_t)b * DIMS + q) * slab_n + s] * rh[q]));
            }
        }
    }
    __shared__ fg_real lds[4];
    mx = fg_wave_max(mx);
    if ((threadIdx.x & 63) == 0) lds[threadIdx.x >> 6] = mx;
    __syncthreads();
    if (flux_B && blockIdx.x == 0) {
        const double total = fg_flux_balance_block<DIMS>(g, bnd, b);
        if (threadIdx.x == 0) {
            fg_bits prevf = __hip_atomic_exchange(reinterpret_cast<fg_bits*>(flux_B) + b, fg_real_bits((fg_real)total), __ATOMIC_RELAXED, __HIP_MEMORY_SCOPE_AGENT);
#if FG_F64
            asm volatile("" ::"v"((int)(prevf >> 32)), "v"((int)prevf));
#else
            asm volatile("" ::"v"(prevf));
#endif
        }
    }
    if (threadIdx.x < 64) {
        mx = FG_FMAX(FG_FMAX(lds[0], lds[1]), FG_FMAX(lds[2], lds[3]));
        fg_publish_max(out_B, done_B, mirror_B, b, mx, poll, (int)gridDim.y, flux_B, flux_mirror, rule);
    }
}

template <int DIMS>
__global__ __launch_bounds__(FG_BLOCK) void k_max_velocity_rows(FgGrid g, FgBounds bnd, const fg_real* __restrict__ vel,
                                                                 fg_real* __restrict__ out_B, int32_t* __restrict__ done_B,
                                                                 fg_real* __restrict__ mirror_B, int rows_per_block, FgPollOut poll,
                                                                 fg_real* flux_B, fg_real* flux_mirror, FgDtRule rule) {
    const int b = blockIdx.y;
    const size_t N = g.n;
    const int lane = threadIdx.x & 63, wave = threadIdx.x >> 6;
    const int rows = g.ny * g.nz, nx4 = g.nx >> 2;
    const int r_end = min(rows, (int)(blockIdx.x + 1) * rows_per_block);
    fg_real mx = 0.f;
    for (int r = blockIdx.x * rows_per_block + wave; r < r_end; r += FG_BLOCK / 64) {
        const int k = r / g.ny, j = r - k * g.ny;
        const fg_real rhy = g.rh[1][j], rhz = (DIMS == 3) ? g.rh[2][k] : 1.f;
        for (int i4 = lane; i4 < nx4; i4 += 64) {
            const fg_real4 rhx = *reinterpret_cast<const fg_real4*>(g.rh[0] + 4 * i4);
            const size_t o = (size_t)r * g.nx + 4 * i4;
            const fg_real4 u = *reinterpret_cast<const fg_real4*>(vel + ((size_t)b * DIMS + 0) * N + o);
            const fg_real4 v = *reinterpret_cast<const fg_real4*>(vel + ((size_t)b * DIMS + 1) * N + o);
            mx = FG_FMAX(mx, FG_FMAX(FG_FMAX(FG_FABS(u.x * rhx.x), FG_FABS(u.y * rhx.y)), FG_FMAX(FG_FABS(u.z * rhx.z), FG_FABS(u.w * rhx.w))));
            mx = FG_FMAX(mx, rhy * FG_FMAX(FG_FMAX(FG_FABS(v.x), FG_FABS(v.y)), FG_FMAX(FG_FABS(v.z), FG_FABS(v.w))));
            if constexpr (DIMS == 3) {
                const fg_real4 w = *reinterpret_cast<const fg_real4*>(vel + ((size_t)b * DIMS + 2) * N + o);
                mx = FG_FMAX(mx, rhz * FG_FMAX(FG_FMAX(FG_FABS(w.x), FG_FABS(w.y)), FG_FMAX(FG_FABS(w.z), FG_FABS(w.w))));
            }
        }
    }
    {
#pragma unroll
        for (int f = 0; f < 2 * DIMS; ++f) {
            if (!g.fixed[f]) continue;
            const int ax = f >> 1;
            const int slab_n = fg_slab_size(g, ax);
            const int edge = (f & 1) ? ((ax == 0) ? g.nx - 1 : (ax == 1) ? g.ny - 1 : g.nz - 1) : 0;
            for (int s = blockIdx.x * blockDim.x + threadIdx.x; s < slab_n; s += gridDim.x * blockDim.x) {
                int i, j, k;
                if (ax == 0) { i = edge; j = s % g.ny; k = s / g.ny; }
                else if (ax == 1) { j = edge; i = s % g.nx; k = s / g.nx; }
                else { k = edge; i = s % g.nx; j = s / g.nx; }
                const fg_real rh[3] = {g.rh[0][i], g.rh[1][j], DIMS == 3 ? g.rh[2][k] : 1.f};
#pragma unroll
                for (int q = 0; q < DIMS; ++q)
                    mx = FG_FMAX(mx, FG_FABS(bnd.vel[f][((size_t)b * DIMS + q) * slab_n + s] * rh[q]));
            }
        }
    }
    __shared__ fg_real lds[4];
    mx = fg_wave_max(mx);
    if (lane == 0) lds[wave] = mx;
    __syncthreads();
    if (flux_B && blockIdx.x == 0) {
        const double total = fg_flux_balance_block<DIMS>(g, bnd, b);
        if (threadIdx.x == 0) {
            fg_bits prevf = __hip_atomic_exchange(reinterpret_cast<fg_bits*>(flux_B) + b, fg_real_bits((fg_real)total), __ATOMIC_RELAXED, __HIP_MEMORY_SCOPE_AGENT);
#if FG_F64
            asm volatile("" ::"v"((int)(prevf >> 32)), "v"((int)prevf));
#else
            asm volatile("" ::"v"(prevf));
#endif
        }
    }
    if (threadIdx.x < 64) {
        mx = FG_FMAX(FG_FMAX(lds[0], lds[1]), FG_FMAX(lds[2], lds[3]));
        fg_publish_max(out_B, done_B, mirror_B, b, mx, poll, (int)gridDim.y, flux_B, flux_mirror, rule);
    }
}

template <int DIMS>
__global__ __launch_bounds__(FG_BLOCK) void k_flux_balance(FgGrid g, FgBounds bnd, fg_real* __restrict__ out_B, FgPollOut poll) {
    const int b = blockIdx.x;
    const double total = fg_flux_balance_block<DIMS>(g, bnd, b);
    if (threadIdx.x == 0) {
        out_B[b] = (fg_real)total;
        fg_poll_publish(poll, b);
    }
}

__global__ __launch_bounds__(FG_BLOCK) void k_copy_active(const fg_real* __restrict__ dt, const fg_real* __restrict__ src,
                                                           fg_real* __restrict__ dst, long per_env) {
    const int b = blockIdx.y;
    if (dt && !(dt[b] > 0.f)) return;
    const fg_real* s = src + (size_t)b * per_env;
    fg_real* d = dst + (size_t)b * per_env;
    const long n4 = (per_env % 4 == 0) ? per_env / 4 : 0;
    for (long i = blockIdx.x * (long)blockDim.x + threadIdx.x; i < n4; i += (long)gridDim.x * blockDim.x)
        reinterpret_cast<fg_real4*>(d)[i] = reinterpret_cast<const fg_real4*>(s)[i];
    if (blockIdx.x == 0)
        for (long i = n4 * 4 + threadIdx.x; i < per_env; i += blockDim.x) d[i] = s[i];
}

__global__ __launch_bounds__(FG_BLOCK) void k_buoyancy(const fg_real* __restrict__ dt, const fg_real* __restrict__ T,
                                                        long t_env_stride, fg_real* __restrict__ source, int dims,
                                                        int n, int axis, fg_real factor) {
    const int b = blockIdx.y;
    if (dt && !(dt[b] > 0.f)) return;
    for (int i = blockIdx.x * blockDim.x + threadIdx.x; i < n; i += gridDim.x * blockDim.x) {
        const fg_real t = T[(size_t)b * t_env_stride + i];
        for (int q = 0; q < dims; ++q) source[((size_t)b * dims + q) * n + i] = (q == axis) ? factor * t : 0.f;
    }
}

__global__ __launch_bounds__(FG_BLOCK) void k_sum_env(const fg_real* __restrict__ dt, const fg_real* __restrict__ p,
                                                       FgDacc* __restrict__ sums, int n) {
    const int b = blockIdx.y;
    if (dt && !(dt[b] > 0.f)) return;
    const fg_real* __restrict__ pb = p + (size_t)b * n;
    fg_real acc = 0.f;
    const int n4 = ((n & 3) == 0 && (reinterpret_cast<size_t>(pb) & 15) == 0) ? n >> 2 : 0;
    for (int i = blockIdx.x * blockDim.x + threadIdx.x; i < n4; i += gridDim.x * blockDim.x) {
        const fg_real4 v = reinterpret_cast<const fg_real4*>(pb)[i];
        acc += (v.x + v.y) + (v.z + v.w);
    }
    for (int i = n4 * 4 + blockIdx.x * blockDim.x + threadIdx.x; i < n; i += gridDim.x * blockDim.x) acc += pb[i];
    __shared__ fg_real lds[4];
    fg_real v[1] = {acc};
    fg_block_sum<1>(v, lds);
    if (threadIdx.x == 0) acc_add(sums + b, (double)v[0]);
}
__global__ __launch_bounds__(FG_BLOCK) void k_sub_mean(const fg_real* __restrict__ dt, fg_real* __restrict__ p,
                                                        fg_real* __restrict__ p_copy, const FgDacc* __restrict__ sums,
                                                        int n) {
    const int b = blockIdx.y;
    if (dt && !(dt[b] > 0.f)) return;
    const fg_real mean = (fg_real)(acc_ld(sums + b) / (double)n);
    fg_real* __restrict__ pb = p + (size_t)b * n;
    fg_real* __restrict__ cb = p_copy ? p_copy + (size_t)b * n : nullptr;
    const bool al = (n & 3) == 0 && (reinterpret_cast<size_t>(pb) & 15) == 0 && (!cb || (reinterpret_cast<size_t>(cb) & 15) == 0);
    const int n4 = al ? n >> 2 : 0;
    for (int i = blockIdx.x * blockDim.x + threadIdx.x; i < n4; i += gridDim.x * blockDim.x) {
        fg_real4 v = reinterpret_cast<fg_real4*>(pb)[i];
        v.x -= mean; v.y -= mean; v.z -= mean; v.w -= mean;
        reinterpret_cast<fg_real4*>(pb)[i] = v;
        if (cb) reinterpret_cast<fg_real4*>(cb)[i] = v;
    }
    for (int i = n4 * 4 + blockIdx.x * blockDim.x + threadIdx.x; i < n; i += gridDim.x * blockDim.x) {
        const fg_real v = pb[i] - mean;
        pb[i] = v;
        if (cb) cb[i] = v;
    }
}

template <int DIMS>
__global__ __launch_bounds__(FG_BLOCK) void k_outflow(FgGrid g, int face, fg_real velm_axis, const fg_real* __restrict__ dt,
                                                       const fg_real* __restrict__ vel, fg_real* __restrict__ bvel,
                                                       const fg_real* __restrict__ scal, fg_real* __restrict__ bscal,
                                                       int n_scalars) {
    const int b = blockIdx.y;
    const fg_real dtb = dt[b];
    if (!(dtb > 0.f)) return;
    const int ax = face >> 1;
    const int slab_n = fg_slab_size(g, ax);
    const int edge = (face & 1) ? ((ax == 0) ? g.nx - 1 : (ax == 1) ? g.ny - 1 : g.nz - 1) : 0;
    const fg_real tcoef = 1.f - 1.f / (1.f + 2.f * dtb * velm_axis * g.rh[ax][edge]);
    const size_t N = g.n;
    for (int s = blockIdx.x * blockDim.x + threadIdx.x; s < slab_n; s += gridDim.x * blockDim.x) {
        int i, j, k;
        if (ax == 0) { i = edge; j = s % g.ny; k = s / g.ny; }
        else if (ax == 1) { j = edge; i = s % g.nx; k = s / g.nx; }
        else { k = edge; i = s % g.nx; j = s / g.nx; }
        const size_t cell = ((size_t)k * g.ny + j) * g.nx + i;
#pragma unroll
        for (int q = 0; q < DIMS; ++q) {
            fg_real* pb = bvel + ((size_t)b * DIMS + q) * slab_n + s;
            const fg_real vb = *pb;
            *pb = vb - tcoef * (vb - vel[((size_t)b * DIMS + q) * N + cell]);
        }
        for (int ch = 0; ch < n_scalars; ++ch) {
            fg_real* pb = bscal + ((size_t)b * n_scalars + ch) * slab_n + s;
            const fg_real sb = *pb;
            *pb = sb - tcoef * (sb - scal[((size_t)b * n_scalars + ch) * N + cell]);
        }
    }
}

struct FgOutflowFold {
    int dt_n; fg_real dt_v[64]; fg_real* dt_out;
    int mask;
    fg_real velm[3];
    const fg_real* vel; const fg_real* scal;
    fg_real* bscal[6]; int nsc[6];
};
struct FgBvelRw { fg_real* p[6]; };
template <int DIMS>
__global__ __launch_bounds__(FG_BLOCK) void k_balance_fluxes(FgGrid g, FgBounds bnd, FgBvelRw bvel_rw_, int free_mask,
                                                              fg_real atol, const fg_real* __restrict__ dt, FgOutflowFold fold) {
    const int b = blockIdx.x;
    const fg_real dtb = fold.dt_n ? fold.dt_v[b] : (dt ? dt[b] : (fg_real)1);
    if (fold.dt_n && threadIdx.x == 0) fold.dt_out[b] = dtb;
    if ((dt || fold.dt_n) && !(dtb > 0.f)) return;
    if (fold.mask) {
        for (int face = 0; face < 2 * DIMS; ++face) {
            if (!((fold.mask >> face) & 1)) continue;
            const int ax = face >> 1;
            const int slab_n = fg_slab_size(g, ax);
            const int edge = (face & 1) ? ((ax == 0) ? g.nx - 1 : (ax == 1) ? g.ny - 1 : g.nz - 1) : 0;
            const fg_real tcoef = 1.f - 1.f / (1.f + 2.f * dtb * fold.velm[ax] * g.rh[ax][edge]);
            const size_t N = g.n;
            fg_real* bvel = bvel_rw_.p[face];
            for (int s = threadIdx.x; s < slab_n; s += blockDim.x) {
                int i, j, k;
                if (ax == 0) { i = edge; j = s % g.ny; k = s / g.ny; }
                else if (ax == 1) { j = edge; i = s % g.nx; k = s / g.nx; }
                else { k = edge; i = s % g.nx; j = s / g.nx; }
                const size_t cell = ((size_t)k * g.ny + j) * g.nx + i;
#pragma unroll
                for (int q = 0; q < DIMS; ++q) {
                    fg_real* pb = bvel + ((size_t)b * DIMS + q) * slab_n + s;
                    const fg_real vb = *pb;
                    *pb = vb - tcoef * (vb - fold.vel[((size_t)b * DIMS + q) * N + cell]);
                }
                for (int ch = 0; ch < fold.nsc[face]; ++ch) {
                    fg_real* pb = fold.bscal[face] + ((size_t)b * fold.nsc[face] + ch) * slab_n + s;
                    const fg_real sb = *pb;
                    *pb = sb - tcoef * (sb - fold.scal[((size_t)b * fold.nsc[face] + ch) * N + cell]);
                }
            }
        }
        __syncthreads();
    }
    double fixed = 0.0, freef = 0.0;
    for (int f = 0; f < 2 * DIMS; ++f) {
        if (!g.fixed[f]) continue;
        const int ax = f >> 1;
        const int slab_n = fg_slab_size(g, ax);
        const double sgn = (f & 1) ? 1.0 : -1.0;
        double acc = 0.0;
        for (int s = threadIdx.x; s < slab_n; s += blockDim.x) {
            int i = 0, j = 0, k = 0;
            if (ax == 0) { j = s % g.ny; k = s / g.ny; }
            else if (ax == 1) { i = s % g.nx; k = s / g.nx; }
            else { i = s % g.nx; j = s / g.nx; }
            fg_real area;
            if (ax == 0) area = g.h[1][j] * (DIMS == 3 ? g.h[2][k] : 1.f);
            else if (ax == 1) area = g.h[0][i] * (DIMS == 3 ? g.h[2][k] : 1.f);
            else area = g.h[0][i] * g.h[1][j];
            acc += sgn * (double)(bnd.vel[f][((size_t)b * DIMS + ax) * slab_n + s] * area);
        }
        if ((free_mask >> f) & 1) freef += acc; else fixed += acc;
    }
    __shared__ double lds[8];
#pragma unroll
    for (int o = 32; o > 0; o >>= 1) { fixed += __shfl_down(fixed, o, 64); freef += __shfl_down(freef, o, 64); }
    if ((threadIdx.x & 63) == 0) { lds[threadIdx.x >> 6] = fixed; lds[4 + (threadIdx.x >> 6)] = freef; }
    __syncthreads();
    fixed = lds[0] + lds[1] + lds[2] + lds[3];
    freef = lds[4] + lds[5] + lds[6] + lds[7];
    if (!(fabs(fixed + freef) > (double)atol)) return;
    const fg_real scale = (fg_real)(-fixed / freef);
    for (int f = 0; f < 2 * DIMS; ++f) {
        if (!((free_mask >> f) & 1) || !g.fixed[f]) continue;
        const int slab_n = fg_slab_size(g, f >> 1);
        fg_real* v = bvel_rw_.p[f] + (size_t)b * DIMS * slab_n;
        for (int s = threadIdx.x; s < DIMS * slab_n; s += blockDim.x) v[s] *= scale;
    }
}

inline unsigned fg_reduce_wgs(const fg_state* s) {
    if (s->reduce_wgs > 0) return (unsigned)s->reduce_wgs;
    const unsigned per_env = (512 + s->grid.B - 1) / s->grid.B;
    return per_env < 8 ? 8 : (per_env > 64 ? 64 : per_env);
}

inline dim3 stride_grid(const fg_state* s, long per_env_elems) {
    long blocks = (per_env_elems / 4 + FG_BLOCK - 1) / FG_BLOCK;
    const long cap = (2048 + s->grid.B - 1) / s->grid.B;
    if (blocks > cap) blocks = cap;
    if (blocks < 1) blocks = 1;
    return dim3((unsigned)blocks, (unsigned)s->grid.B, 1);
}

}


int fg_launch_adv_build(fg_state* s, const FgBounds& bnd, const FgAdvArgs& a_in, hipStream_t st) {
    FgAdvArgs a = a_in;
    a.begin.acc = s->acc; a.begin.sc = s->scratch_B + 4 * s->grid.B; a.begin.flags = s->flags; a.begin.info = s->info_dev;
    a.begin.nc = a.for_scalar ? 1 : s->grid.dims;
    s->prepared.set_bicg(a.begin.nc, a.dt);
    const double nd = (double)s->grid.n;
    const int slot = fg_prof_slot(s, FG_PK_ADV_BUILD, nullptr, s->grid.B, (s->grid.dims == 3 ? 56.0 : 44.0) * nd, 30.0 * nd, st);
    FG_DISPATCH(s, {
        const FgLaunch L = fg_launch_geometry<DIMS, VEC>(s->grid);
        if (a.for_scalar)
            FG_LAUNCH_P(s, slot, (k_adv_build<DIMS, VEC, true>), L.grid, dim3(FG_BLOCK), 0, st, s->grid, bnd, a, L.tiles_x,
                        L.tiles_y, L.tiles);
        else if (a.visc)
            FG_LAUNCH_P(s, slot, (k_adv_build<DIMS, VEC, false, true>), L.grid, dim3(FG_BLOCK), 0, st, s->grid, bnd, a, L.tiles_x,
                        L.tiles_y, L.tiles);
        else
            FG_LAUNCH_P(s, slot, (k_adv_build<DIMS, VEC, false>), L.grid, dim3(FG_BLOCK), 0, st, s->grid, bnd, a, L.tiles_x,
                        L.tiles_y, L.tiles);
    });
    FG_HIP_CHECK(hipGetLastError());
    return FG_OK;
}

template <int DIMS>
__global__ __launch_bounds__(FG_BLOCK) void k_sgs_smagorinsky(FgGrid g, FgBounds bnd, const fg_real* __restrict__ vel, fg_real coefficient,
                                                               fg_real* __restrict__ out) {
    const int b = blockIdx.y, c = blockIdx.x * FG_BLOCK + threadIdx.x;
    if (c >= g.n) return;
    const int ext[3] = {g.nx, g.ny, DIMS == 3 ? g.nz : 1};
    const int pos[3] = {c % g.nx, (c / g.nx) % g.ny, c / (g.nx * g.ny)};
    const int stride[3] = {1, g.nx, g.nx * g.ny};
    const fg_real* u = vel + (size_t)b * DIMS * g.n;
    fg_real grad[DIMS][DIMS];
    fg_real delta = 0.f;
#pragma unroll
    for (int a = 0; a < DIMS; ++a) {
        const fg_real h = g.h[a][pos[a]];
        delta = FG_FMAX(delta, h * h);
        fg_real dist = 2.f;
        fg_real diff[DIMS];
#pragma unroll
        for (int q = 0; q < DIMS; ++q) diff[q] = 0.f;
#pragma unroll
        for (int up = 0; up < 2; ++up) {
            const int f = 2 * a + up;
            const bool at = up ? (pos[a] + 1 == ext[a]) : (pos[a] == 0);
            if (at && g.fixed[f]) {
                int si = 0, mul = 1;
#pragma unroll
                for (int t = 0; t < DIMS; ++t) if (t != a) { si += pos[t] * mul; mul *= ext[t]; }
                const fg_real* bv = bnd.vel[f] + (size_t)b * DIMS * mul;
#pragma unroll
                for (int q = 0; q < DIMS; ++q) diff[q] += (up ? 1.f : -1.f) * bv[q * mul + si];
                dist -= 0.5f;
            } else {
                const int n = at ? (up ? c - (ext[a] - 1) * stride[a] : c + (ext[a] - 1) * stride[a]) : (up ? c + stride[a] : c - stride[a]);
#pragma unroll
                for (int q = 0; q < DIMS; ++q) diff[q] += (up ? 1.f : -1.f) * u[(size_t)q * g.n + n];
            }
        }
#pragma unroll
        for (int q = 0; q < DIMS; ++q) grad[q][a] = diff[q] / dist * g.rh[a][pos[a]];
    }
    fg_real d = 0.f;
#pragma unroll
    for (int i = 0; i < DIMS; ++i)
#pragma unroll
        for (int j = i; j < DIMS; ++j) {
            fg_real sij = 0.5f * (grad[i][j] + grad[j][i]);
            sij *= sij;
            d += (i != j) ? 2.f * sij : sij;
        }
    out[(size_t)b * g.n + c] = coefficient * delta * FG_SQRT(2.f * d);
}

__global__ __launch_bounds__(1024) void k_wall_forcing(FgGrid g, const fg_real* __restrict__ vel, int axis, fg_real coef_lo, fg_real coef_hi,
                                                        fg_real* __restrict__ force, int dims) {
    const int b = blockIdx.x;
    const size_t N = g.n;
    const fg_real* __restrict__ u = vel + ((size_t)b * dims + axis) * N;
    double lo = 0.0, hi = 0.0;
    const int rows = g.nz;
    for (int idx = threadIdx.x; idx < rows * g.nx; idx += blockDim.x) {
        const int k = idx / g.nx, i = idx - k * g.nx;
        lo += (double)u[((size_t)k * g.ny + 0) * g.nx + i];
        hi += (double)u[((size_t)k * g.ny + (g.ny - 1)) * g.nx + i];
    }
    __shared__ double lds[2][16];
#pragma unroll
    for (int o = 32; o > 0; o >>= 1) { lo += __shfl_down(lo, o, 64); hi += __shfl_down(hi, o, 64); }
    if ((threadIdx.x & 63) == 0) { lds[0][threadIdx.x >> 6] = lo; lds[1][threadIdx.x >> 6] = hi; }
    __syncthreads();
    if (threadIdx.x == 0) {
        double sl = 0.0, sh = 0.0;
        for (int w = 0; w < (int)(blockDim.x >> 6); ++w) { sl += lds[0][w]; sh += lds[1][w]; }
        const double n = (double)rows * g.nx;
        const fg_real tau_lo = coef_lo * (fg_real)(sl / n), tau_hi = coef_hi * (fg_real)(sh / n);
        for (int q = 0; q < dims; ++q) force[b * dims + q] = (q == axis) ? (fg_real)0.5 * (tau_lo + tau_hi) : (fg_real)0;
    }
}

int fg_launch_wall_forcing(const fg_state* s, hipStream_t st) {
    hipLaunchKernelGGL(k_wall_forcing, dim3(s->grid.B), dim3(1024), 0, st, s->grid, (const fg_real*)s->velocity, s->wall_forcing_axis,
                       s->wall_forcing_coef[0], s->wall_forcing_coef[1], s->force_uniform, s->grid.dims);
    FG_HIP_CHECK(hipGetLastError());
    return FG_OK;
}

int fg_launch_sgs(const fg_state* s, const FgBounds& bnd, fg_real coefficient, fg_real* out, hipStream_t st) {
    const dim3 grid((s->grid.n + FG_BLOCK - 1) / FG_BLOCK, s->grid.B);
    if (s->grid.dims == 2) hipLaunchKernelGGL(k_sgs_smagorinsky<2>, grid, dim3(FG_BLOCK), 0, st, s->grid, bnd, (const fg_real*)s->velocity, coefficient, out);
    else hipLaunchKernelGGL(k_sgs_smagorinsky<3>, grid, dim3(FG_BLOCK), 0, st, s->grid, bnd, (const fg_real*)s->velocity, coefficient, out);
    FG_HIP_CHECK(hipGetLastError());
    return FG_OK;
}

int fg_launch_pressure_setup(const fg_state* s, const fg_real* dt, hipStream_t st) {
    const int n = s->grid.n;
    hipLaunchKernelGGL(k_reciprocal, stride_grid(s, n), dim3(FG_BLOCK), 0, st, s->A, s->rA, dt, n, (n % 4 == 0) ? n / 4 : 0);
    FG_HIP_CHECK(hipGetLastError());
    return FG_OK;
}

int fg_launch_h(fg_state* s, const fg_real* dt, const fg_real* vel_result, hipStream_t st) {
    fg_htrace("h_launch_in");
    FgCgBegin begin;
    begin.acc = s->cg_acc; begin.flags = s->flags; begin.info = s->info_dev; begin.mean_sums = s->acc; begin.best = s->cg_best;
    begin.track_best = s->cg_return_best; begin.ns = fg_cg_slots(s); begin.xsum = s->fcg_xsum;
    s->prepared.set_cg(begin.ns, begin.track_best, dt);
    const int slot_h = fg_prof_slot(s, FG_PK_H, nullptr, s->grid.B, (s->grid.dims == 3 ? 68.0 : 52.0) * (double)s->grid.n, 6.0 * s->grid.dims * s->grid.dims * (double)s->grid.n, st);
    FG_DISPATCH(s, {
        const FgLaunch L = fg_launch_geometry<DIMS, VEC>(s->grid);
        FG_LAUNCH_P(s, slot_h, (k_h<DIMS, VEC>), L.grid, dim3(FG_BLOCK), 0, st, s->grid, dt, s->rA, s->Coff, s->adv_rhs,
                    vel_result, s->hvec, begin, L.tiles_x, L.tiles_y, L.tiles);
    });
    FG_HIP_CHECK(hipGetLastError());
    fg_htrace("h_launch_out");
    return FG_OK;
}

int fg_launch_div(fg_state* s, const FgBounds& bnd, const fg_real* dt, const fg_real* hvec, fg_real* div,
                  hipStream_t st, bool cg_from_zero, bool fused_fwd) {
    FgCgStart start = {nullptr, nullptr, nullptr, 1};
    s->prepared.set_cg_start(0);
    if (cg_from_zero && dt != nullptr && s->prepared.cg_for(dt) && div == s->div) {
#if !FG_F64
        if (fused_fwd && fg_fcg_ok(s)) {
            s->prepared.set_cg_start(2);
            return fg_fcg_div_fwd(s, bnd, dt, hvec, div, s->prepared.cg_ns, st);
        }
#endif
        start.acc = s->cg_acc; start.r = s->w[0]; start.x = s->p_result; start.ns = s->prepared.cg_ns;
        s->prepared.set_cg_start(1);
    }
    const int slot_d = fg_prof_slot(s, FG_PK_DIV, nullptr, s->grid.B, 28.0 * (double)s->grid.n, 4.0 * s->grid.dims * (double)s->grid.n, st);
    FG_DISPATCH(s, {
        const FgLaunch L = fg_launch_geometry<DIMS, VEC>(s->grid);
        FG_LAUNCH_P(s, slot_d, (k_div<DIMS, VEC>), L.grid, dim3(FG_BLOCK), 0, st, s->grid, bnd, dt, hvec, div, start, L.tiles_x,
                    L.tiles_y, L.tiles);
    });
    FG_HIP_CHECK(hipGetLastError());
    return FG_OK;
}

int fg_launch_correct(const fg_state* s, const fg_real* dt, const fg_real* rA, const fg_real* hvec, const fg_real* p,
                      fg_real* vel_out, hipStream_t st, fg_real* vel_copy, const FgMeanRef* mean, const FgLazyRef* lazy) {
    fg_htrace("correct_in");
    const FgMeanRef mr = mean ? *mean : FgMeanRef{nullptr, nullptr, nullptr, nullptr, nullptr};
    const FgLazyRef lz = lazy ? *lazy : FgLazyRef{nullptr, nullptr, nullptr};
    const double cb = (s->grid.dims == 3 ? 36.0 : 28.0) + (vel_copy ? 4.0 * s->grid.dims : 0.0) + ((mean && mean->sums) || (lazy && lazy->p_res) ? 4.0 : 0.0);
    const int slot_c = fg_prof_slot(s, FG_PK_CORRECT, nullptr, s->grid.B, cb * (double)s->grid.n, 5.0 * s->grid.dims * (double)s->grid.n, st);
    FG_DISPATCH(s, {
        const FgLaunch L = fg_launch_geometry<DIMS, VEC>(s->grid);
        FG_LAUNCH_P(s, slot_c, (k_correct<DIMS, VEC>), L.grid, dim3(FG_BLOCK), 0, st, s->grid, dt, rA, hvec, p, vel_out, vel_copy, mr, lz,
                    L.tiles_x, L.tiles_y, L.tiles);
    });
    FG_HIP_CHECK(hipGetLastError());
    fg_htrace("correct_out");
    return FG_OK;
}

int fg_launch_max_velocity(const fg_state* s, const FgBounds& bnd, fg_real* out_B, hipStream_t st, fg_real* mirror_B, FgPollOut poll,
                           fg_real* flux_B, fg_real* flux_mirror, FgDtRule rule) {
    FG_REQUIRE(!rule.t_rem || (poll.gran && mirror_B && !FG_F64), FG_ERR_INVALID_ARG, "the device-side sub-step rule needs the result-word form");
    FG_REQUIRE(!flux_B || (mirror_B && flux_mirror), FG_ERR_INVALID_ARG, "the flux balance rides in the mirrored form only");
    int32_t* done_B = reinterpret_cast<int32_t*>(out_B + s->grid.B);
    FG_REQUIRE(!mirror_B || out_B == s->scratch_B + s->grid.B, FG_ERR_INVALID_ARG, "mirror needs the scratch row as out_B");
    if (!mirror_B || !s->maxvel_clean)
        FG_HIP_CHECK(hipMemsetAsync(out_B, 0, mirror_B ? sizeof(fg_real) * s->grid.B + sizeof(int32_t) * (s->grid.B + 1) : sizeof(fg_real) * s->grid.B, st));
    s->maxvel_clean = mirror_B ? 1 : 0;
    if ((s->grid.nx & 3) == 0) {
        const int rows = s->grid.ny * s->grid.nz;
        int rpb = 4;
        while ((long)((rows + 2 * rpb - 1) / (2 * rpb)) * s->grid.B >= 2048) rpb *= 2;
        while ((rows + rpb - 1) / rpb > (int)fg_reduce_wgs(s)) rpb *= 2;
        dim3 grid((rows + rpb - 1) / rpb, s->grid.B);
        const int slot_m = fg_prof_slot(s, FG_PK_MAXVEL, nullptr, s->grid.B, 4.0 * s->grid.dims * (double)s->grid.n, 2.0 * s->grid.dims * (double)s->grid.n, st);
        if (s->grid.dims == 2)
            FG_LAUNCH_P(s, slot_m, k_max_velocity_rows<2>, grid, dim3(FG_BLOCK), 0, st, s->grid, bnd, s->velocity, out_B, done_B,
                        mirror_B, rpb, poll, flux_B, flux_mirror, rule);
        else
            FG_LAUNCH_P(s, slot_m, k_max_velocity_rows<3>, grid, dim3(FG_BLOCK), 0, st, s->grid, bnd, s->velocity, out_B, done_B,
                        mirror_B, rpb, poll, flux_B, flux_mirror, rule);
        FG_HIP_CHECK(hipGetLastError());
        return FG_OK;
    }
    dim3 grid = stride_grid(s, (long)s->grid.n * 4);
    if (s->grid.dims == 2)
        hipLaunchKernelGGL(k_max_velocity<2>, grid, dim3(FG_BLOCK), 0, st, s->grid, bnd, s->velocity, out_B, done_B, mirror_B, poll, flux_B, flux_mirror, rule);
    else
        hipLaunchKernelGGL(k_max_velocity<3>, grid, dim3(FG_BLOCK), 0, st, s->grid, bnd, s->velocity, out_B, done_B, mirror_B, poll, flux_B, flux_mirror, rule);
    FG_HIP_CHECK(hipGetLastError());
    return FG_OK;
}

int fg_launch_flux_balance(const fg_state* s, const FgBounds& bnd, fg_real* out_B, hipStream_t st, FgPollOut poll) {
    if (s->grid.dims == 2)
        hipLaunchKernelGGL(k_flux_balance<2>, dim3(s->grid.B), dim3(FG_BLOCK), 0, st, s->grid, bnd, out_B, poll);
    else
        hipLaunchKernelGGL(k_flux_balance<3>, dim3(s->grid.B), dim3(FG_BLOCK), 0, st, s->grid, bnd, out_B, poll);
    FG_HIP_CHECK(hipGetLastError());
    return FG_OK;
}

int fg_launch_copy_active(const fg_state* s, const fg_real* dt, const fg_real* src, fg_real* dst, int comps,
                          hipStream_t st) {
    const long per_env = (long)comps * s->grid.n;
    hipLaunchKernelGGL(k_copy_active, stride_grid(s, per_env), dim3(FG_BLOCK), 0, st, dt, src, dst, per_env);
    FG_HIP_CHECK(hipGetLastError());
    return FG_OK;
}

int fg_launch_buoyancy(const fg_state* s, const fg_real* dt, const fg_real* T, long t_env_stride, fg_real* source, int axis,
                       fg_real factor, hipStream_t st) {
    hipLaunchKernelGGL(k_buoyancy, stride_grid(s, (long)s->grid.n * 4), dim3(FG_BLOCK), 0, st, dt, T, t_env_stride,
                       source, s->grid.dims, s->grid.n, axis, factor);
    FG_HIP_CHECK(hipGetLastError());
    return FG_OK;
}

int fg_launch_mean_sub(const fg_state* s, const fg_real* dt, fg_real* p, fg_real* p_copy, hipStream_t st) {
    FgDacc* sums = s->acc;
    dim3 grid = stride_grid(s, (long)s->grid.n * 4);
    dim3 rgrid(grid.x > fg_reduce_wgs(s) ? fg_reduce_wgs(s) : grid.x, grid.y);
    hipLaunchKernelGGL(k_sum_env, rgrid, dim3(FG_BLOCK), 0, st, dt, p, sums, s->grid.n);
    hipLaunchKernelGGL(k_sub_mean, grid, dim3(FG_BLOCK), 0, st, dt, p, p_copy, sums, s->grid.n);
    FG_HIP_CHECK(hipGetLastError());
    return FG_OK;
}

int fg_launch_outflow(const fg_state* s, int face, fg_real velm_axis, const fg_real* dt, hipStream_t st) {
    const int slab_n = (face >> 1) == 0 ? s->grid.ny * s->grid.nz : (face >> 1) == 1 ? s->grid.nx * s->grid.nz : s->grid.nx * s->grid.ny;
    dim3 grid((slab_n + FG_BLOCK - 1) / FG_BLOCK, s->grid.B);
    const int nsc = (s->scalar && s->bscal[face]) ? s->cfg.n_scalars : 0;
    if (s->grid.dims == 2)
        hipLaunchKernelGGL(k_outflow<2>, grid, dim3(FG_BLOCK), 0, st, s->grid, face, velm_axis, dt, s->velocity, s->bvel[face],
                           s->scalar, s->bscal[face], nsc);
    else
        hipLaunchKernelGGL(k_outflow<3>, grid, dim3(FG_BLOCK), 0, st, s->grid, face, velm_axis, dt, s->velocity, s->bvel[face],
                           s->scalar, s->bscal[face], nsc);
    FG_HIP_CHECK(hipGetLastError());
    return FG_OK;
}

int fg_launch_balance(const fg_state* s, const FgBounds& bnd, int free_mask, fg_real atol, const fg_real* dt, hipStream_t st,
                      int outflow_mask, const fg_real* outflow_velm, const fg_real* dt_host_values) {
    FgOutflowFold fold;
    fold = FgOutflowFold{};
    if (dt_host_values) {
        fold.dt_n = s->grid.B; fold.dt_out = s->dt_dev;
        for (int b = 0; b < s->grid.B; ++b) fold.dt_v[b] = dt_host_values[b];
    }
    if (outflow_mask) {
        fold.mask = outflow_mask; fold.vel = s->velocity; fold.scal = s->scalar;
        for (int a = 0; a < 3; ++a) fold.velm[a] = outflow_velm[a];
        for (int f = 0; f < 6; ++f) { fold.bscal[f] = s->bscal[f]; fold.nsc[f] = (s->scalar && s->bscal[f]) ? s->cfg.n_scalars : 0; }
    }
    FgBvelRw rw;
    for (int f = 0; f < 6; ++f) rw.p[f] = s->bvel[f];
    if (s->grid.dims == 2)
        hipLaunchKernelGGL(k_balance_fluxes<2>, dim3(s->grid.B), dim3(FG_BLOCK), 0, st, s->grid, bnd, rw, free_mask, atol, dt, fold);
    else
        hipLaunchKernelGGL(k_balance_fluxes<3>, dim3(s->grid.B), dim3(FG_BLOCK), 0, st, s->grid, bnd, rw, free_mask, atol, dt, fold);
    FG_HIP_CHECK(hipGetLastError());
    return FG_OK;
}

bool fg_outflow_folds(const fg_state* s, int outflow_mask) {
    for (int f = 0; f < 2 * s->grid.dims; ++f) {
        if (!((outflow_mask >> f) & 1)) continue;
        const int ax = f >> 1;
        const long slab_n = ax == 0 ? (long)s->grid.ny * s->grid.nz : ax == 1 ? (long)s->grid.nx * s->grid.nz : (long)s->grid.nx * s->grid.ny;
        if (slab_n > 4 * FG_BLOCK) return false;
    }
    return outflow_mask != 0;
}
```

### fluidgym_amd/csrc/fg_poisson.hip

```cpp
#include <math.h>
#include <cmath>
#include <vector>

#include "fg_internal.h"
#include "fg_cg.h"
#include "fg_rung64.h"
#include "fg_fftcg.h"

namespace {

template <int DIMS, int VEC>
struct FgCoef {
    fg_real xm[VEC], xp[VEC], ym[VEC], yp[VEC], zm[VEC], zp[VEC];
};

template <int DIMS, int VEC>
__device__ __forceinline__ FgCoef<DIMS, VEC> fg_poisson_coef(const FgCtx<DIMS, VEC>& c, const FgMetric<DIMS, VEC>& m,
                                                             const FgNbr<DIMS, VEC>& rA) {
    FgCoef<DIMS, VEC> k;
    const fg_real ayz = m.hy * m.hz;
#pragma unroll
    for (int e = 0; e < VEC; ++e) {
        const fg_real rh_lo = (e == 0) ? m.rhx_m : m.rhx[e > 0 ? e - 1 : 0];
        const fg_real rh_hi = (e == VEC - 1) ? m.rhx_p : m.rhx[e < VEC - 1 ? e + 1 : VEC - 1];
// ... 304 lines not shown
                           omega, 0, L.tiles_x, L.tiles_y, L.tiles);
    });
    FG_HIP_CHECK(hipGetLastError());
    return FG_OK;
}

int fg_poisson_rbgs_launch(const fg_state* s, const fg_real* rA, const fg_real* b, fg_real* x, fg_real omega, int color,
                           hipStream_t st) {
    int zc;
    if (fg_zmarch_ok(s, &zc)) return fg_zmarch_relax(s, rA, b, x, x, omega, color, zc, st);
    FG_DISPATCH(s, {
        const FgLaunch L = fg_launch_geometry<DIMS, VEC>(s->grid);
        hipLaunchKernelGGL((k_poisson_relax<DIMS, VEC, true>), L.grid, dim3(FG_BLOCK), 0, st, s->grid, rA, b, x, x,
                           omega, color, L.tiles_x, L.tiles_y, L.tiles);
    });
    FG_HIP_CHECK(hipGetLastError());
    return FG_OK;
}

int fg_fd_rowmean_prefactor(fg_state* s, const fg_real* dt, hipStream_t st) {
#if !FG_F64
    if (!(s->fd_Qx && fg_fcg_ok(s) && fg_fd_rowmean_ok(s)) || s->fd_row_epoch == s->rA_epoch || dt == nullptr) return FG_OK;
    const bool parts = s->fd_row_part && s->fd_row_part_epoch == s->rA_epoch;
    if (parts && fg_fd_tridiag_can_factor(s)) return FG_OK;
    if (int rc = fg_fd_rowmean_factor(s, s->rA, dt, st, parts ? s->fd_row_part : nullptr, (s->grid.nx + 63) / 64)) return rc;
    s->fd_row_epoch = s->rA_epoch;
#else
    (void)s; (void)dt; (void)st;
#endif
    return FG_OK;
}

int fg_cg_slots(const fg_state* s) {
    int tiles_per_env = 1;
    FG_DISPATCH(s, { tiles_per_env = fg_launch_geometry<DIMS, VEC>(s->grid).tiles; });
    int ns = 1;
    while (ns < FG_CG_SLOTS && tiles_per_env / ns > 256) ns *= 2;
    return ns;
}

namespace {
struct CgRun {
    int ns, nb, check_every, next_poll;
    fg_real* zvec;
    FgDacc* mean_sums;
    FgCgJudge judge;
    bool fused;
    bool start_ready = false;
    bool start_fwd = false;
    bool done = false, info_fresh = false;
};
}

static int cg_begin(fg_state* s, const FgCgArgs& a, CgRun& c, hipStream_t st) {
    const int B = s->grid.B, n = s->grid.n;
    const int ns = c.ns = fg_cg_slots(s);
    {
        const int prep = s->prepared.take_cg(ns, s->cg_return_best, a.dt);
        c.start_ready = prep > 0 && !a.use_x0 && a.b == s->div && a.r == s->w[0] && a.x == s->p_result;
        c.start_fwd = c.start_ready && prep == 2;
        if (prep < 0) {
            FgCgBegin q;
            q.acc = s->cg_acc; q.flags = s->flags; q.info = s->info_dev; q.mean_sums = s->acc; q.best = s->cg_best;
            q.track_best = s->cg_return_best; q.ns = ns; q.xsum = s->fcg_xsum;
            hipLaunchKernelGGL(k_cg_begin, dim3(B), dim3(64), 0, st, a.dt, q, B);
        }
    }
    if (!c.start_ready)
    FG_DISPATCH(s, {
        const FgLaunch L = fg_launch_geometry<DIMS, VEC>(s->grid);
        hipLaunchKernelGGL((k_cg_residual<DIMS, VEC>), L.grid, dim3(FG_BLOCK), 0, st, s->grid, a.rA, a.b, a.x, a.r,
                           s->cg_acc, s->flags, a.use_x0, 0, ns, L.tiles_x, L.tiles_y, L.tiles);
    });
    c.check_every = a.check_every > 0 ? a.check_every : 16;
    c.nb = a.precond ? 5 : 0;
    c.zvec = a.precond ? s->w[5] : a.r;
    c.judge.acc = s->cg_acc; c.judge.flags = s->flags; c.judge.info = s->info_dev; c.judge.tol = a.tol; c.judge.it = -1; c.judge.n = n; c.judge.ns = ns;
#if !FG_F64
    c.fused = a.precond && s->fd_Qx && fg_fcg_ok(s);
#else
    c.fused = false;
#endif
    if (a.precond && !c.fused) {
        if (!s->fd_Qx) { fg_set_error("preconditioned CG requested but fg_set_fd_preconditioner was not called"); return FG_ERR_INVALID_ARG; }
        if (int rc = fg_fd_apply(s, a.r, c.zvec, s->cg_acc + (size_t)(c.nb + 0) * FG_CG_SLOTS, FG_CG_NAMES * FG_CG_SLOTS, ns, B, st, &c.judge)) return rc;
    }
    c.next_poll = a.precond ? (s->pred_cg[a.kind & 3] + 1 > 1 ? s->pred_cg[a.kind & 3] + 1 : 1) : c.check_every;
    c.mean_sums = (!a.use_x0 && a.x == s->p_result && s->fcg_xsum) ? s->fcg_xsum : nullptr;
    return FG_OK;
}

#if !FG_F64
static int cg_iterate_fused(fg_state* s, const FgCgArgs& a, CgRun& c, FgCgOutcome& o, hipStream_t st) {
    const int B = s->grid.B, n = s->grid.n, ns = c.ns;
    FgCgJudge& judge = c.judge;
    FcgVectors v;
    v.x = a.x; v.r = a.r; v.t1 = s->w[3]; v.z = c.zvec; v.w = s->w[4]; v.p = a.p; v.s = a.Ap;
    FgCgLead lead;
    lead.best = s->cg_best;
    const bool rowm = fg_fd_rowmean_ok(s);
    const float* factor_from = nullptr;
    if (rowm && !(a.rA == s->rA && s->fd_row_epoch == s->rA_epoch)) {
        const bool parts = a.rA == s->rA && s->fd_row_part && s->fd_row_part_epoch == s->rA_epoch;
        if (parts && fg_fd_tridiag_can_factor(s)) factor_from = s->fd_row_part;
        else if (int rc = fg_fd_rowmean_factor(s, a.rA, a.dt, st, parts ? s->fd_row_part : nullptr, (s->grid.nx + 63) / 64)) return rc;
        s->fd_row_epoch = (a.rA == s->rA) ? s->rA_epoch : -1;
    }
    judge.it = -1;
    if (!c.start_fwd)
        if (int rc = fg_fd_dct_forward(s, a.r, v.t1, st, 0, &judge)) return rc;
    lead.judge = judge;
    if (int rc = fg_fd_tridiag(s, v.t1, st, &lead, rowm, factor_from, a.dt)) return rc;
    const fg_real* r0 = c.start_fwd ? a.b : nullptr;
    {
        FcgVectors v0 = v;
        if (r0) v0.r = const_cast<fg_real*>(r0);
        if (int rc = fg_fcg_inv_apply(s, v0, a.rA, 0, ns, st, s->fcg_first)) return rc;
    }
    if (s->fcg_first && a.max_iterations >= 1) {
        const bool poll0 = c.next_poll <= 1;
        if (poll0) fg_prof_prefetch(s, st);
        const FgPollOut po = poll0 ? fg_poll_next(&s->poll) : FgPollOut{nullptr, 0};
        if (int rc = fg_fcg_check0(s, a.tol, ns, st, po, &o.marks_valid)) return rc;
        bool spec = false;
        if (poll0 && s->fcg_spec && a.spec.fn && a.lazy_ok && r0 && c.mean_sums) {
            FgCgOutcome ahead;
            ahead.lazy_z = v.z; ahead.mean_ready = true; ahead.marks_valid = true;
            if (int rc = a.spec.fn(a.spec.ctx, ahead)) return rc;
            spec = true;
        }
        if (poll0) {
            fg_htrace("cg_check_launched");
            const int active = fg_poll_wait_active(&s->poll, po, 0, B, s->info_pinned, st);
            if (active < 0) return active;
            fg_htrace("cg_poll_done");
            c.info_fresh = true;
            s->fcg_first_polls += 1;
            if (active == 0) {
                bool all_ok = true;
                for (int b = 0; b < B; ++b) all_ok = all_ok && s->info_pinned[b].converged && s->info_pinned[b].is_finite;
                if (a.lazy_ok && r0 && all_ok && c.mean_sums) {
                    o.lazy_z = v.z; s->fcg_unstored += 1; o.spec_done = spec;
                } else {
                    if (int rc = fg_fcg_update_fwd(s, v, 0, 1, ns, st, o.marks_valid, r0)) return rc;
                }
                c.done = true;
            } else {
                c.next_poll = 2;
            }
        }
    }
    int first = 1;
    const int fused_reset = (a.reset_steps > 0 && a.reset_steps < 10) ? a.reset_steps : 10;
    for (int it = 0; it < a.max_iterations && !c.done; ++it) {
        if (int rc = fg_fcg_update_fwd(s, v, it, first, ns, st, o.marks_valid, it == 0 ? r0 : nullptr)) return rc;
        if (first) {
            fg_real* t = v.p; v.p = v.z; v.z = t;
            t = v.s; v.s = v.w; v.w = t;
            first = 0;
        }
        const bool poll = (it + 1 >= c.next_poll || it + 1 == a.max_iterations);
        if (poll) {
            c.next_poll = it + 1 + c.check_every;
            const int final_pass = (it + 1 == a.max_iterations);
            fg_prof_prefetch(s, st);
            const FgPollOut po = fg_poll_next(&s->poll);
            hipLaunchKernelGGL(k_cg_check, dim3((B + CG_CHECK_WAVES - 1) / CG_CHECK_WAVES), dim3(64 * CG_CHECK_WAVES), 0, st, s->cg_acc, s->flags, s->info_dev, s->info_pinned, a.tol, it,
                               n, B, final_pass, ns, po);
            fg_htrace("cg_check_launched");
            const int active = fg_poll_wait_active(&s->poll, po, 0, B, s->info_pinned, st);
            if (active < 0) return active;
            fg_htrace("cg_poll_done");
            c.info_fresh = true;
            c.done = (active == 0);
            if (c.done) break;
        }
        if (it + 1 < a.max_iterations) {
            judge.it = it;
            if ((it + 2) % fused_reset == 0) {
                hipLaunchKernelGGL(k_zero_name, dim3(B), dim3(64), 0, st, s->cg_acc, (it + 1) % 3, B);
                FG_DISPATCH(s, {
                    const FgLaunch L = fg_launch_geometry<DIMS, VEC>(s->grid);
                    hipLaunchKernelGGL((k_cg_residual<DIMS, VEC>), L.grid, dim3(FG_BLOCK), 0, st, s->grid, a.rA, a.b, a.x,
                                       a.r, s->cg_acc, s->flags, 1, (it + 1) % 3, ns, L.tiles_x, L.tiles_y, L.tiles);
                });
                if (int rc = fg_fd_dct_forward(s, a.r, v.t1, st, 0, nullptr)) return rc;
                first = 1;
            }
            lead.judge = judge;
            if (int rc = fg_fd_tridiag(s, v.t1, st, &lead, rowm)) return rc;
            if (int rc = fg_fcg_inv_apply(s, v, a.rA, it + 1, ns, st)) return rc;
        }
    }
    o.mean_ready = !a.use_x0;
    return FG_OK;
}
#endif

static int cg_iterate_classic(fg_state* s, const FgCgArgs& a, CgRun& c, FgCgOutcome& o, hipStream_t st) {
    const int B = s->grid.B, n = s->grid.n, ns = c.ns, nb = c.nb;
    fg_real* pbuf[2] = {a.p, s->w[6]};
    int zc = 0;
    const bool zmarch = fg_zmarch_ok(s, &zc);
    int active_est = (B + 3) / 4;
    for (int it = 0; it < a.max_iterations && !c.done; ++it) {
        int first = (it == 0);
        if (a.reset_steps > 0 && it > 0 && (it + 1) % a.reset_steps == 0) {
            hipLaunchKernelGGL(k_zero_name, dim3(B), dim3(64), 0, st, s->cg_acc, it % 3, B);
            FG_DISPATCH(s, {
                const FgLaunch L = fg_launch_geometry<DIMS, VEC>(s->grid);
                hipLaunchKernelGGL((k_cg_residual<DIMS, VEC>), L.grid, dim3(FG_BLOCK), 0, st, s->grid, a.rA, a.b, a.x,
                                   a.r, s->cg_acc, s->flags, 1, it % 3, ns, L.tiles_x, L.tiles_y, L.tiles);
            });
            first = 1;
        }
        const fg_real* p_in = pbuf[(it + 1) & 1];
        fg_real* p_out = pbuf[it & 1];
        const int slot_ap = fg_prof_slot(s, FG_PK_CG_AP, FG_PROF_SELF, B, (double)n * (first ? 16.0 : 20.0),
                                         (double)n * (4.0 * s->grid.dims + 5.0), st);
        if (zmarch) {
            if (int rc = fg_zmarch_cg_ap(s, a.rA, c.zvec, p_in, p_out, a.Ap, s->cg_acc, s->flags, s->info_dev, slot_ap,
                                         a.tol, it, first, ns, nb, zc, st))
                return rc;
        } else {
            FG_DISPATCH(s, {
                const FgLaunch L = fg_launch_geometry<DIMS, VEC>(s->grid);
                FG_LAUNCH_P(s, slot_ap, (k_cg_ap<DIMS, VEC>), L.grid, dim3(FG_BLOCK), 0, st, s->grid, a.rA, c.zvec, p_in,
                            p_out, a.Ap, s->cg_acc, s->flags, s->info_dev,
                            slot_ap >= 0 ? s->prof.active_dev + slot_ap : nullptr, s->cg_best, a.tol, it, first, ns,
                            nb, L.tiles_x, L.tiles_y, L.tiles);
            });
        }
        const int slot_up = fg_prof_slot(s, FG_PK_CG_UPDATE, s->flags, B, (double)n * 24.0, (double)n * 6.0, st);
        FG_DISPATCH(s, {
            const FgLaunch L = fg_launch_geometry<DIMS, VEC>(s->grid);
            FG_LAUNCH_P(s, slot_up, (k_cg_update<DIMS, VEC>), L.grid, dim3(FG_BLOCK), 0, st, s->grid, p_out, a.Ap, a.x,
                        a.r, s->cg_acc, s->flags, s->cg_best, a.tol, it, ns, nb, c.mean_sums, L.tiles_x, L.tiles_y, L.tiles);
        });
        const bool poll = (it + 1 >= c.next_poll || it + 1 == a.max_iterations);
        if (poll) c.next_poll = it + 1 + c.check_every;
        if (poll) {
            const int final_pass = (it + 1 == a.max_iterations);
            fg_prof_prefetch(s, st);
            const FgPollOut po = fg_poll_next(&s->poll);
            hipLaunchKernelGGL(k_cg_check, dim3((B + CG_CHECK_WAVES - 1) / CG_CHECK_WAVES), dim3(64 * CG_CHECK_WAVES), 0, st, s->cg_acc, s->flags, s->info_dev, s->info_pinned, a.tol, it,
                               n, B, final_pass, ns, po);
            const int active = fg_poll_wait_active(&s->poll, po, 0, B, s->info_pinned, st);
            if (active < 0) return active;
            c.info_fresh = true;
            c.done = (active == 0);
            if (c.done) break;
            active_est = active;
        }
        if (a.precond && it + 1 < a.max_iterations) {
            c.judge.it = it;
            if (int rc = fg_fd_apply(s, a.r, c.zvec, s->cg_acc + (size_t)(nb + (it + 1) % 3) * FG_CG_SLOTS, FG_CG_NAMES * FG_CG_SLOTS, ns, active_est, st, &c.judge))
                return rc;
        }
    }
    if (c.mean_sums) o.mean_ready = true;
    return FG_OK;
}

static int cg_finish(fg_state* s, const FgCgArgs& a, const CgRun& c, FgCgOutcome& o, fg_solve_info* info_host, hipStream_t st) {
    const int B = s->grid.B, n = s->grid.n;
    if (int rc = fg_solve_infos_settle(s, B, c.info_fresh, st)) return rc;
    bool failed = false;
    for (int b = 0; b < B; ++b) failed = failed || !s->info_pinned[b].converged;
    if (failed) {
        o.mean_ready = false;
        hipLaunchKernelGGL(k_cg_restore_best, dim3(32, B), dim3(FG_BLOCK), 0, st, a.x, s->info_dev, s->info_pinned, s->cg_best, n);
        FG_HIP_CHECK(hipStreamSynchronize(st));
    }
    int used_max = 0;
    const int rc = fg_solve_infos_report(s, B, info_host, &used_max);
    if (a.precond) s->pred_cg[a.kind & 3] = used_max;
    return rc;
}

int fg_cg_solve(fg_state* s, const FgCgArgs& a, fg_solve_info* info_host, hipStream_t st, FgCgOutcome* out) {
    CgRun c;
    FgCgOutcome o;
    if (int rc = cg_begin(s, a, c, st)) return rc;
#if !FG_F64
    if (c.fused) { if (int rc = cg_iterate_fused(s, a, c, o, st)) return rc; }
    else
#endif
    if (int rc = cg_iterate_classic(s, a, c, o, st)) return rc;
    const int rc = cg_finish(s, a, c, o, info_host, st);
    if (out) *out = o;
    return rc;
}

#if !FG_F64
namespace {
template <int DIMS>
__global__ __launch_bounds__(FG_BLOCK) void k64_papply(FgGrid g, const float* __restrict__ rA_, const double* __restrict__ x, double* __restrict__ y,
                                                       int tiles_x, int tiles_y, int tiles) {
    const FgCtx<DIMS, 1> c = fg_make_ctx<DIMS, 1>(g, tiles_x, tiles_y, tiles);
    if (!c.valid) return;
    const FgMetric<DIMS, 1> m = fg_metrics<DIMS, 1>(g, c);
    const FgNbr<DIMS, 1> rA = fg_gather<DIMS, 1>(rA_, c);
    const FgCoef<DIMS, 1> k = fg_poisson_coef<DIMS, 1>(c, m, rA);
    const R64Nbr<DIMS> X = r64_gather<DIMS>(x, c);
    double v = (double)k.xm[0] * (X.xm - X.c) + (double)k.xp[0] * (X.xp - X.c) + (double)k.ym[0] * (X.ym - X.c) + (double)k.yp[0] * (X.yp - X.c);
    if constexpr (DIMS == 3) v += (double)k.zm[0] * (X.zm - X.c) + (double)k.zp[0] * (X.zp - X.c);
    y[c.idx] = v;
}
}

int fg_rung64_cg(fg_state* s, const FgCgArgs& a, fg_solve_info* info, bool all_envs, hipStream_t st, FgCgOutcome* out) {
    R64 w;
    if (int rc = w.init(s, st)) return rc;
    const int B = s->grid.B, n = s->grid.n, d = s->grid.dims;
    FgGrid g1 = s->grid; g1.B = 1;
    double *r = w.v[0], *p = w.v[1], *Ap = w.v[2], *x = w.v[3], *bb = w.v[4];
    auto apply = [&](int b, const double* in, double* out) {
        const float* rA = a.rA + (size_t)b * n;
        if (d == 2) { FgLaunch L = fg_launch_geometry<2, 1>(g1); hipLaunchKernelGGL((k64_papply<2>), L.grid, dim3(FG_BLOCK), 0, st, g1, rA, in, out, L.tiles_x, L.tiles_y, L.tiles); }
        else { FgLaunch L = fg_launch_geometry<3, 1>(g1); hipLaunchKernelGGL((k64_papply<3>), L.grid, dim3(FG_BLOCK), 0, st, g1, rA, in, out, L.tiles_x, L.tiles_y, L.tiles); }
    };
    auto rms = [&](double q) { return sqrt(q / (double)n); };
    std::vector<float> dt_host;
    if (a.dt) { dt_host.resize(B); FG_HIP_CHECK(hipMemcpyAsync(dt_host.data(), a.dt, sizeof(float) * B, hipMemcpyDeviceToHost, st)); FG_HIP_CHECK(hipStreamSynchronize(st)); }
    int rc_all = FG_OK;
    for (int b = 0; b < B; ++b) {
        if (a.dt && !(dt_host[b] > 0.f)) continue;
        fg_solve_info& I = info[b];
// ... 123 lines not shown
```

### fluidgym_amd/csrc/fg_switches.h

```cpp
#pragma once
#include <string>

enum FgSwitchRule { FG_SW_INT, FG_SW_POS, FG_SW_ON, FG_SW_OFF, FG_SW_ONE, FG_SW_SET, FG_SW_TRI, FG_SW_ALL };
int fg_switch_parse(const char* text, FgSwitchRule rule, int def);

#define FG_COMMON_SWITCHES(X) \
    X(FG_POLL_SPIN, poll.spin, 1, ON, HANDLE, no, "0: host polls wait with hipStreamSynchronize instead of spinning on pinned sequence words") \
    X(FG_POLL_WORDS, poll.words, 1, ON, HANDLE, no, "0: polled verdicts through the host-pinned mirror + a system-scope release (one L2 write-back per verdict kernel) instead of travelling in the 8-byte result words the host spins on (A/B runs: 8 790 against 9 600 env-steps/s on the headline, one lane); reported as 0 where the handle has no result words (fp64 build, FG_POLL_SPIN=0)") \
    X(FG_ADV_JACOBI, adv_jacobi, 0, INT, HANDLE, bits, "velocity systems of uniform 2-D grids and of the multi-block meshes: 1 Jacobi sweeps first (fg_jacobi.hip, mb_jacobi), 0 BiCGStab always; unset = what fg_set_advection_jacobi / fg_mb_set_advection_jacobi says (the Simulation turns it on: policy advection_jacobi)")

#define FG_SB_SWITCHES(X) \
    X(FG_CG_FUSED, cg_fused, 1, INT, HANDLE, bits, "1 (default): three-launch preconditioned pressure CG on 2-D fast-transform grids (fg_fftcg.hip); 0: the five kernels") \
    X(FG_BICG_PFUSED, bicg_pfused, 1, INT, HANDLE, bits, "1 (default): six-launch Helmholtz-preconditioned BiCGStab (fg_fftbicg.hip); 0: eleven launches per iteration") \
    X(FG_BICG_FUSED, bicg_fused, 1, INT, HANDLE, bits, "1 (default): two-kernel BiCGStab iteration in 2-D; 0: five kernels; 2: two kernels in 3-D bricks too") \
    X(FG_BICG_SUB, bicg_sub, -1, INT, HANDLE, no, "envs per sub-batch of the 2-D two-kernel BiCGStab (unset: by working set; 0: never)") \
    X(FG_BICG3, bicg3_force, -1, INT, HANDLE, bits, "z-marching 3-D BiCGStab (fg_bicgstab3d.hip): 0 never, N always with z-chunk N (tests on small grids), unset: when the grid fits the tiles and fills the chip") \
    X(FG_BICG3_BXL, bicg3_bxl, 0, INT, HANDLE, no, "tile lanes along x of the z-marching BiCGStab (16 / 32)") \
    X(FG_BICG3_MIX, bicg3_mix, 3, INT, HANDLE, bits, "debugging: bit 0 kernel a, bit 1 kernel b as z-march, bit 2 keep the init kernel") \
    X(FG_REDUCE_WGS, reduce_wgs, 0, INT, HANDLE, no, "workgroups per env of the reduction kernels (0 = the rule of fg_reduce_wgs)") \
    X(FG_HELM_ROWFORM, helm_rowform, 1, ON, HANDLE, bits, "0: Helmholtz factors through k_helm_coeffs + the array-form line kernels (IEEE division instead of the hardware reciprocal)") \
    X(FG_ADV_LINESWEEP, adv_linesweep, 0, INT, HANDLE, bits, "1: the advection-diffusion systems of the Helmholtz-preconditioned family (wall-refined 2-D grids: RBC) go to line sweeps x <- (D + O_y)^-1 (b - O_x x) first (k_line_sweep_y, fg_linepre.hip), BiCGStab takes what they do not settle; 0 (default): the preconditioned BiCGStab always -- measured on the RBC leg: 16-17 sweeps per velocity solve at the bench state's sub-step, 775 against 793 env-steps/s") \
    X(FG_FD_FACFUSE, fd_facfuse, 1, INT, HANDLE, no, "1 (default): the first tridiagonal solve after 1/A changed makes the per-env row-mean factors itself (k_tridiag_y_lds<.., FAC>: same arithmetic, same bits); 0: k_fd_rowmean_factor as a launch of its own (A/B runs)") \
    X(FG_FD_ROWMEAN, fd_rowmean, 1, INT, HANDLE, bits, "1 (default): the fused pressure CG is preconditioned by the row-mean operator (per-env factors, one factorisation per PISO step); 0: the grid's A = 1 factors") \
    X(FG_FCG_FIRST, fcg_first, 1, ON, HANDLE, bits, "1 (default): the fused CG judges its first iterate from I'(0)'s dot products (k_fcg_check0) and stores no pressure when every env ends there; 0: the verdict on the updated residual (A/B runs, tests)") \
    X(FG_FCG_SPEC, fcg_spec, 1, ON, HANDLE, no, "0: the corrector waits for the verdict on the first iterate instead of being launched behind the verdict kernel (A/B runs)") \
    X(FG_JAC_SPEC, jac_spec, 1, ON, HANDLE, no, "0: k_h and the divergence kernel of the first corrector wait for the verdict on the velocity sweeps instead of being launched behind the check kernel (A/B runs)") \
    X(FG_JAC_PREFACTOR, jac_prefactor, 1, ON, HANDLE, no, "0: the row-mean factors of the pressure preconditioner are made in front of the first tridiagonal solve instead of behind the sweeps' check kernel (A/B runs)") \
    X(FG_JAC_WARM, jac_warm, -1, TRI, HANDLE, bits, "start vector of the Jacobi sweeps of a step's velocity systems: 1 the block velocity, 0 the BiCGStab start vector (zero on the non-orthogonal branch); unset: the block velocity on on-chip grids of 2^17 cells and more (where it saves a pass)") \
    X(FG_JAC_XCD, jac_xcd, 1, INT, HANDLE, no, "0: the on-chip Jacobi regions in launch order instead of one XCD per run of an env's regions (A/B runs)") \
    X(FG_JAC_SHAPE, jac_shape, 0, INT, HANDLE, bits, "A/B runs of the Jacobi sweeps: 1 full-row regions only, 2 bands only (unset: the cheaper of the two for the grid)") \
    X(FG_JAC_SWEEPS, jac_sweeps, 0, INT, HANDLE, bits, "A/B runs: sweeps per pass of the Jacobi sweeps, clamped to what the region allows (unset: 4 / 6 / 8 for full rows, 8 / 12 for bands, by region depth)") \
    X(FG_FORCE_ZMARCH, zmarch_force, 0, INT, HANDLE, bits, "z-march chunk length of the 3-D Poisson kernels (tests on small grids; -1 = brick kernels)") \
    X(FG_ZMARCH_SB, zmarch_sb, -1, INT, HANDLE, no, "single-barrier ring of the z-march kernels: bit per mode forces it on with the caller's chunk length, 0 never, unset = where the launch is one full round") \
    X(FG_DEV_DT, dev_dt, 1, INT, HANDLE, no, "0: fg_single_step waits for the CFL maxima and computes the adaptive sub-steps on the host before the PISO step, instead of the CFL kernel's last workgroup taking them on the device (FgDtRule: same doubles, same bits) and the host reading the maxima after the step (A/B runs)") \
    X(FG_PROF_PERIOD, prof_period, 64, POS, HANDLE, no, "sampling period of the live kernel timing: every 64th launch of a kind is timed (8 cost the timed region ~5 %: a count kernel + two events per sample)")

#define FG_MB_SWITCHES(X) \
    X(FG_MB_BICG_VEC4, dbg_vec_mask, 31, ALL, HANDLE, no, "bit per multi-block BiCGStab kernel: four-cell form (1 p, 2 v, 4 s, 8 t, 16 x; 1 or 31 = all)") \
    X(FG_MB_BICG_FUSE, dbg_fuse_st, 2, INT, HANDLE, bits, "multi-block BiCGStab: 0 five kernels, 1 s/t fused, 2 (default) also p/v") \
    X(FG_MB_ML_FUSE, dbg_ml_fuse, 1, INT, HANDLE, bits, "multilevel BiCGStab forms p / s inside the restriction: 0 never, 1 up to 32 systems, 2 always") \
    X(FG_MB_ML_TRY_CAP, dbg_ml_cap, 200, POS, HANDLE, policy, "iteration cap of an attempt of the multilevel trial (200; tests force 2)") \
    X(FG_MB_TRACE, dbg_trace, 0, SET, HANDLE, no, "residual / verification trace of the pressure BiCGStab on stderr") \
    X(FG_MB_TRACE_FAIL, dbg_fail, 0, SET, HANDLE, no, "recurrence words of a system that ends non-finite") \
    X(FG_MB_COMPACT, dbg_compact, 1, INT, HANDLE, no, "0: every multi-block Krylov launch covers all systems of the batch") \
    X(FG_MB_OC_RTG_NT, oc_rtg_nt, 1024, INT, HANDLE, bits, "register-resident on-chip CG with a global residual copy on 16-24 k-cell meshes instead of k_mbc_l2: workgroup size of that instance (1024 x 24 or 512 x 48 cells per thread)") \
    X(FG_MB_ONCHIP, onchip_mode, 1, ON, HANDLE, bits, "0: no whole-solve on-chip CG (chunked CG kernels)") \
    X(FG_MB_OC_AGG, dbg_oc_agg, 1, ON, HANDLE, bits, "0: cell-ordered on-chip CG instead of the aggregate-owned one") \
    X(FG_MB_OC_VARIANT, oc_variant, 0, INT, HANDLE, no, "on-chip CG variant bits (bit 0: no compiler fences in the stencil pass; bit 1: split [F][N] coefficient layout)") \
    X(FG_MB_CLUSTER, cl_mode, 1, INT, HANDLE, bits, "pressure CG of an env by a cluster of four workgroups (fg_mb_cluster.hip): 0 never (the one-workgroup kernels), 1 (default) meshes beyond 8 k cells, 2 every mesh its tables fit (tests)") \
    X(FG_MB_CL_JACOBI, cl_jacobi, 1, ON, HANDLE, bits, "0: the velocity sweeps of the meshes the cluster CG takes stay one launch per sweep (k_mbj_sweep_env) instead of one launch per solve by the clusters (k_mbj_cluster; A/B runs: 2 552 against 3 045 env-steps/s on the cylinder mesh)") \
    X(FG_MB_CL_HALF, cl_half, 1, ON, HANDLE, bits, "0: meshes whose rows of the coarse inverse do not fit LDS as fp32 stream them from L2 instead of holding them as fp16 (A/B runs: 19.7 against 16.8 us per iteration on 23 k cells)") \
    X(FG_MB_CL_MAXCL, cl_max_clusters, 0, INT, HANDLE, no, "cap on the clusters of one launch of the cluster CG (tests: envs beyond it queue inside the kernel; same bits)") \
    X(FG_MB_CL_NEAR, cl_near, 1, ON, HANDLE, no, "0: granule stores of the cluster CG always write through to memory, also when a cluster's workgroups reported one XCD (A/B runs: 10.0 against 8.6 us per iteration)") \
    X(FG_MB_RUNG_ILU, dbg_rung_ilu, 1, ON, HANDLE, bits, "0: column-scaled preconditioned rung instead of ILU(0)") \
    X(FG_MB_PCG_KERNEL, dbg_pcg_kernel, 0, ONE, HANDLE, bits, "1 (fp32 build, debugging): the multilevel-preconditioned pressure CG as the kernel-form loop of mb_cg (five launches per iteration, `k_mbc_ap<.., MBC_PRE>` / `k_mbc_update<.., true>`: what the fp64 build runs) instead of the on-chip / cluster kernels; 0 (default)")

extern int fg_htrace_on, fg_roctx_on;
#define FG_PROCESS_SWITCHES(X) \
    X(FG_HTRACE, fg_htrace_on, 0, OFF, PROCESS, no, "1: host time stamps around the polls and the launches behind them (fg_poll.hip), per-pair averages printed at exit") \
    X(FG_ROCTX, fg_roctx_on, 0, OFF, PROCESS, no, "1: named roctx ranges around the phases of a step (fg_single_step, scalar / velocity assembly and solve, pressure correctors; mb_velocity_solve, mb_pressure_solve) for rocprofv3 --marker-trace; the library is dlopen'ed, off by default")

#define FG_SW_MEMBER(var, member, def, rule, scope, results, what) int member = def;

void fg_switches_read(struct fg_state* s);
void fg_switches_read(struct fg_mb_state* s);
void fg_switches_json(const struct fg_state* s, std::string& json);
void fg_switches_json(const struct fg_mb_state* s, std::string& json);
void fg_json_put(std::string& json, const char* key, long long value);
int fg_json_out(const std::string& json, char* buf, int n);
```

Measured before the change: 10380 env-steps/s.

## Fuse CFL maxima into corrector and add one-launch step head kernel

The last velocity corrector now records per-tile CFL maxima as it writes the velocity. When those maxima are still valid, a new k_step_head kernel (one workgroup per env) reduces them, applies the guard and the adaptive sub-step rule, and does the balance work in a single launch. This replaces the separate full CFL pass over the velocity plus the balance launch. Separately, the fused pressure CG now launches the corrector speculatively behind its first poll. Validity tracking via cfl_valid must be invalidated on every velocity write, and a mispredicted speculation costs wasted work.

New measurement: 10600 env-steps/s (median of 6 runs). About the same (+2.1%).

```diff
diff --git a/fluidgym_amd/csrc/fg_api.hip b/fluidgym_amd/csrc/fg_api.hip
--- a/fluidgym_amd/csrc/fg_api.hip
+++ b/fluidgym_amd/csrc/fg_api.hip
@@ -113,6 +113,9 @@
     FG_HIP_CHECK(hipMalloc(&s->t_rem_dev, sizeof(double) * g.B));
     FG_HIP_CHECK(hipMemset(s->t_rem_dev, 0, sizeof(double) * g.B));
 #endif
+    FG_DISPATCH(s, { s->cfl_tiles = fg_launch_geometry<DIMS, VEC>(g).tiles; });
+    FG_HIP_CHECK(alloc(&s->cfl_part, (size_t)g.B * s->cfl_tiles));
+    s->cfl_valid = 0;
     if (int rc = fg_poll_create(&s->poll, (int)(nsys > 2 * (size_t)g.B ? nsys : 2 * (size_t)g.B))) return rc;
     for (int k = 0; k < 4; ++k) { s->pred_bicg[k] = 2; s->pred_cg[k] = 1; }
     s->wall_forcing_axis = -1;
@@ -152,7 +155,7 @@
     (void)hipHostFree(s->info_pinned); (void)hipHostFree(s->flags_pinned);
     fg_prof_destroy(s);
     fg_poll_destroy(&s->poll);
-    (void)hipFree(s->d_bvel_ptrs); (void)hipHostFree(s->diag_pinned); (void)hipHostFree(s->dt_pinned); (void)hipFree(s->dt_dev); (void)hipFree(s->t_rem_dev); (void)hipFree(s->env_sel_dev);
+    (void)hipFree(s->d_bvel_ptrs); (void)hipHostFree(s->diag_pinned); (void)hipHostFree(s->dt_pinned); (void)hipFree(s->dt_dev); (void)hipFree(s->t_rem_dev); (void)hipFree(s->cfl_part); (void)hipFree(s->env_sel_dev);
     float* fd[] = {s->fd_Qx, s->fd_QxT, s->fd_Qz, s->fd_QzT, s->fd_lower, s->fd_inv, s->fd_cp};
     for (float* p : fd) if (p) (void)hipFree(p);
     if (s->fd_dct_tw) { (void)hipFree(s->fd_dct_tw); (void)hipFree(s->fd_dct_rot); }
@@ -170,7 +173,7 @@
 static int sync_bvel_ptrs(fg_state* s);
 extern "C" int fg_bind(fg_handle s, int field, fg_real* ptr) {
     FG_REQUIRE(s, FG_ERR_INVALID_ARG, "null handle");
-    if (field == FG_VELOCITY) s->velocity = ptr;
+    if (field == FG_VELOCITY) { s->velocity = ptr; s->cfl_valid = 0; }
     else if (field == FG_PRESSURE) s->pressure = ptr;
     else if (field == FG_SCALAR) s->scalar = ptr;
     else if (field == FG_VELOCITY_SOURCE) s->velocity_source = ptr;
@@ -624,6 +627,7 @@
 
 extern "C" int fg_copy_velocity_result_to_blocks(fg_handle s, void* stream) {
     FG_REQUIRE(s && s->velocity, FG_ERR_NOT_BOUND, "velocity not bound");
+    s->cfl_valid = 0;
     return fg_launch_copy_active(s, s->cur_dt, s->vel_result, s->velocity, s->grid.dims, (hipStream_t)stream);
 }
 extern "C" int fg_copy_velocity_result_from_blocks(fg_handle s, void* stream) {
@@ -748,8 +752,10 @@
         if (!outcome.spec_done)
             if (int rc = launch_corrector(s, dt_B, outcome, last, st)) return rc;
     }
-    if (opt->corrector_steps <= 0)
+    if (opt->corrector_steps <= 0) {
+        s->cfl_valid = 0;
         if (int rc = fg_launch_copy_active(s, dt_B, s->vel_result, s->velocity, d, st)) return rc;
+    }
     if (stats_host) memcpy(stats_host, stats, sizeof(stats));
     s->ctr.piso_steps += 1;
     return status;
@@ -763,7 +769,9 @@
         {"fast_transform_x", s->fd_dct_x}, {"fd_preconditioner", s->fd_Qx ? 1 : 0}, {"helmholtz", s->fd_lam ? 1 : 0}, {"advection_preconditioner", s->adv_precond},
         {"advection_from_result", s->adv_from_result}, {"return_best", s->cg_return_best}, {"cg_reset_steps", s->cg_reset_steps}, {"double_fallback", s->double_fallback},
         {"wall_forcing_axis", s->wall_forcing_axis}, {"first_iterate_polls", s->fcg_first_polls}, {"unstored_pressure_solves", s->fcg_unstored},
-        {"jacobi_speculation_misses", s->jac_spec_missed}, {"jacobi_floor_released", s->jac_floor_released}, {"pressure_refinement_corrections", s->ref64_corrections}};
+        {"jacobi_speculation_misses", s->jac_spec_missed}, {"jacobi_floor_released", s->jac_floor_released}, {"pressure_refinement_corrections", s->ref64_corrections},
+        {"step_head_launches", s->step_head_launches}, {"straggler_speculations", s->fcg_strag_spec},
+        {"straggler_speculation_misses", s->fcg_strag_missed}};
     for (const auto& kv : state) fg_json_put(out, kv.first, kv.second);
     return fg_json_out(out + "}", buf, n);
 }
@@ -781,17 +789,18 @@
     return FG_OK;
 }
 
-extern "C" int fg_single_step(fg_handle s, const fg_sim_options* o, int32_t* out, fg_real* flux_host, void* stream);
+static int single_step(fg_handle s, const fg_sim_options* o, int32_t* out, fg_real* flux_host, void* stream);
 extern "C" int fg_multi_step(fg_handle s, const fg_sim_options* o, int32_t n, const fg_real* const* bvel_schedule, int32_t* out_6n,
                              fg_real* flux_host, int32_t* steps_done, void* stream) {
     FG_REQUIRE(s && o && out_6n && n >= 0, FG_ERR_INVALID_ARG, "fg_multi_step: bad argument");
     if (steps_done) *steps_done = 0;
+    s->cfl_valid = 0;
     for (int k = 0; k < n; ++k) {
         if (bvel_schedule)
             for (int f = 0; f < 2 * s->grid.dims; ++f)
                 if (const fg_real* p = bvel_schedule[(size_t)k * 6 + f])
                     if (int rc = fg_bind(s, FG_BOUND_VELOCITY + f, const_cast<fg_real*>(p))) return rc;
-        if (int rc = fg_single_step(s, o, out_6n + 6 * (size_t)k, flux_host, stream)) return rc;
+        if (int rc = single_step(s, o, out_6n + 6 * (size_t)k, flux_host, stream)) return rc;
         if (steps_done) *steps_done = k + 1;
         if (out_6n[6 * (size_t)k + 5] == 0 && !s->cg_return_best) break;
     }
@@ -801,6 +810,11 @@
 static inline bool is_close_zero(double a) { return std::fabs(a) <= 1e-8; }
 
 extern "C" int fg_single_step(fg_handle s, const fg_sim_options* o, int32_t* out, fg_real* flux_host, void* stream) {
+    if (s) s->cfl_valid = 0;
+    return single_step(s, o, out, flux_host, stream);
+}
+
+static int single_step(fg_handle s, const fg_sim_options* o, int32_t* out, fg_real* flux_host, void* stream) {
     fg_htrace("single_step_in");
     FgRange range_sim("fg_single_step");
     FG_REQUIRE(s && o && out, FG_ERR_INVALID_ARG, "null argument");
@@ -850,6 +864,7 @@
             return FG_OK;
         };
         bool deferred = false;
+        bool head = false;
         FgPollOut po_cfl = FgPollOut{nullptr, 0};
         if (o->adaptive || first) {
             const FgPollOut po = fg_poll_next(&s->poll);
@@ -859,7 +874,13 @@
                 deferred = po.gran != nullptr && s->dev_dt && s->t_rem_dev != nullptr;
                 const FgDtRule rule = deferred ? FgDtRule{s->t_rem_dev, s->dt_dev, (float)o->cfl, (double)o->time_step, first ? 1 : 0}
                                                : FgDtRule{nullptr, nullptr, 0.f, 0.0, 0};
-                if (int rc = fg_launch_max_velocity(s, bnd, s->scratch_B + B, st, s->diag_pinned + B, po.seq ? FgPollOut{po.seq + B, po.value, po.gran} : po,
+                head = deferred && fg_step_head_ok(s);
+                if (head) {
+                    for (int f = 0; f < 2 * s->grid.dims; ++f)
+                        if ((o->outflow_mask >> f) & 1) FG_REQUIRE(s->grid.fixed[f], FG_ERR_INVALID_ARG, "outflow face is not FIXED");
+                    const fg_real velm3[3] = {o->outflow_velm[0], o->outflow_velm[1], o->outflow_velm[2]};
+                    if (int rc = fg_launch_step_head(s, bnd, st, po, first, rule, o->outflow_mask, (fg_real)0.01 * o->outflow_tol, velm3)) return rc;
+                } else if (int rc = fg_launch_max_velocity(s, bnd, s->scratch_B + B, st, s->diag_pinned + B, po.seq ? FgPollOut{po.seq + B, po.value, po.gran} : po,
                                                     first ? s->scratch_B : nullptr, first ? s->diag_pinned : nullptr, rule))
                     return rc;
             }
@@ -881,7 +902,7 @@
         const bool folded = o->outflow_mask && fg_outflow_folds(s, o->outflow_mask);
         const bool dt_by_value = folded && B <= 64 && !deferred;
         if (!dt_by_value && !deferred) FG_HIP_CHECK(hipMemcpyAsync(s->dt_dev, s->dt_pinned, sizeof(fg_real) * B, hipMemcpyHostToDevice, st));
-        if (o->outflow_mask) {
+        if (o->outflow_mask && !head) {
             for (int f = 0; f < 2 * s->grid.dims; ++f)
                 if ((o->outflow_mask >> f) & 1) FG_REQUIRE(s->grid.fixed[f], FG_ERR_INVALID_ARG, "outflow face is not FIXED");
             if (!folded)
@@ -922,6 +943,7 @@
     FG_REQUIRE(s, FG_ERR_INVALID_ARG, "null handle");
     if (int rc = check_bound(s, false)) return rc;
     s->cur_dt = nullptr;
+    s->cfl_valid = 0;
     hipStream_t st = (hipStream_t)stream;
     const size_t BN = (size_t)s->grid.B * s->grid.n;
     std::vector<fg_real> ones(BN, 1.f);
@@ -940,6 +962,7 @@
 extern "C" int fg_reset_solver_state(fg_handle s, void* stream) {
     FG_REQUIRE(s && s->velocity, FG_ERR_NOT_BOUND, "velocity not bound");
     for (int k = 0; k < 4; ++k) s->jac_hist[k] = FgJacHist{0, 0, 0};
+    s->cfl_valid = 0;
     FG_HIP_CHECK(hipMemsetAsync(s->p_result, 0, sizeof(fg_real) * (size_t)s->grid.B * s->grid.n, (hipStream_t)stream));
     return fg_launch_copy_active(s, nullptr, s->velocity, s->vel_result, s->grid.dims, (hipStream_t)stream);
 }
diff --git a/fluidgym_amd/csrc/fg_envrestore.hip b/fluidgym_amd/csrc/fg_envrestore.hip
--- a/fluidgym_amd/csrc/fg_envrestore.hip
+++ b/fluidgym_amd/csrc/fg_envrestore.hip
@@ -76,7 +76,7 @@
     const FgGrid& g = s->grid;
     fg_real* dst = nullptr;
     int C = 0, vector_field = 0, ext[3] = {g.nx, g.ny, g.nz};
-    if (which_field == FG_VELOCITY) { dst = s->velocity; C = g.dims; vector_field = 1; }
+    if (which_field == FG_VELOCITY) { dst = s->velocity; C = g.dims; vector_field = 1; s->cfl_valid = 0; }
     else if (which_field == FG_PRESSURE) { dst = s->pressure; C = 1; }
     else if (which_field == FG_SCALAR) { dst = s->scalar; C = s->cfg.n_scalars; }
     else if (which_field == FG_VELOCITY_SOURCE) { dst = s->velocity_source; C = g.dims; vector_field = 1; }
diff --git a/fluidgym_amd/csrc/fg_internal.h b/fluidgym_amd/csrc/fg_internal.h
--- a/fluidgym_amd/csrc/fg_internal.h
+++ b/fluidgym_amd/csrc/fg_internal.h
@@ -649,6 +649,7 @@
     long jac_spec_missed;
     long jac_floor_released = 0;
     long fcg_unstored, fcg_first_polls;
+    long fcg_strag_spec, fcg_strag_missed;
     fg_real* line_inv; fg_real* line_cp;
     fg_real* ilu_d;
     int double_fallback; int ladder_force; long long rung_count[4];
@@ -668,6 +669,8 @@
     fg_real* dt_pinned;
     fg_real* dt_dev;
     double* t_rem_dev;
+    fg_real* cfl_part; int cfl_tiles; mutable int cfl_valid;
+    mutable long step_head_launches;
     int pred_bicg[4], pred_cg[4];
     int adv_jacobi, adv_jacobi_env; FgJacHist jac_hist[4]; float* jac_prev;
     long long jac_solves, jac_fallbacks;
@@ -779,6 +782,10 @@
                       int outflow_mask = 0, const fg_real* outflow_velm = nullptr,
                       const fg_real* dt_host_values = nullptr);
 bool fg_outflow_folds(const fg_state* s, int outflow_mask);
+bool fg_step_head_grid(const fg_state* s);
+inline bool fg_step_head_ok(const fg_state* s) { return s->cfl_valid && fg_step_head_grid(s); }
+int fg_launch_step_head(const fg_state* s, const FgBounds& bnd, hipStream_t st, FgPollOut poll, bool first, FgDtRule rule, int outflow_mask,
+                        fg_real atol, const fg_real* outflow_velm);
 int fg_launch_mean_sub(const fg_state* s, const fg_real* active_dt, fg_real* p, fg_real* p_copy, hipStream_t st);
 
 int fg_poisson_apply_launch(const fg_state* s, const fg_real* rA, const fg_real* x, fg_real* y, hipStream_t st);
diff --git a/fluidgym_amd/csrc/fg_piso.hip b/fluidgym_amd/csrc/fg_piso.hip
--- a/fluidgym_amd/csrc/fg_piso.hip
+++ b/fluidgym_amd/csrc/fg_piso.hip
@@ -292,13 +292,10 @@
     }
 }
 
-template <int DIMS, int VEC>
-__global__ __launch_bounds__(FG_BLOCK) void k_correct(FgGrid g, const fg_real* __restrict__ dt,
-                                                       const fg_real* __restrict__ rA_, const fg_real* __restrict__ hvec,
-                                                       const fg_real* __restrict__ p, fg_real* __restrict__ vel_out,
-                                                       fg_real* __restrict__ vel_copy, FgMeanRef mean, FgLazyRef lazy, int tiles_x, int tiles_y, int tiles) {
-    const FgCtx<DIMS, VEC> c = fg_make_ctx<DIMS, VEC>(g, tiles_x, tiles_y, tiles);
-    if ((dt && !(dt[c.b] > 0.f)) || !c.valid) return;
+template <int DIMS, int VEC, bool CFL>
+__device__ __forceinline__ void fg_correct_cells(const FgGrid& g, const FgCtx<DIMS, VEC>& c, const fg_real* __restrict__ rA_,
+                                                 const fg_real* __restrict__ hvec, const fg_real* __restrict__ p, fg_real* __restrict__ vel_out,
+                                                 fg_real* __restrict__ vel_copy, const FgMeanRef& mean, const FgLazyRef& lazy, fg_real& cfl_mx) {
     const size_t N = g.n;
     const FgMetric<DIMS, VEC> m = fg_metrics<DIMS, VEC>(g, c);
     const FgVec<VEC> rA = fg_load<VEC>(rA_ + (size_t)c.b * N + c.idx);
@@ -347,6 +344,39 @@
         }
         fg_store<VEC>(vel_out + base + c.idx, out);
         if (vel_copy) fg_store<VEC>(vel_copy + base + c.idx, out);
+        if constexpr (CFL) {
+            if (q == 0) {
+#pragma unroll
+                for (int e = 0; e < VEC; ++e) cfl_mx = FG_FMAX(cfl_mx, FG_FABS(out.v[e] * m.rhx[e]));
+            } else {
+                fg_real a = 0.f;
+#pragma unroll
+                for (int e = 0; e < VEC; ++e) a = FG_FMAX(a, FG_FABS(out.v[e]));
+                cfl_mx = FG_FMAX(cfl_mx, (q == 1 ? m.rhy : m.rhz) * a);
+            }
+        }
+    }
+}
+
+template <int DIMS, int VEC, bool CFL = false>
+__global__ __launch_bounds__(FG_BLOCK) void k_correct(FgGrid g, const fg_real* __restrict__ dt,
+                                                       const fg_real* __restrict__ rA_, const fg_real* __restrict__ hvec,
+                                                       const fg_real* __restrict__ p, fg_real* __restrict__ vel_out,
+                                                       fg_real* __restrict__ vel_copy, FgMeanRef mean, FgLazyRef lazy, int tiles_x, int tiles_y, int tiles,
+                                                       fg_real* __restrict__ cfl_part = nullptr) {
+    const FgCtx<DIMS, VEC> c = fg_make_ctx<DIMS, VEC>(g, tiles_x, tiles_y, tiles);
+    if (dt && !(dt[c.b] > 0.f)) return;
+    fg_real cfl_mx = 0.f;
+    if (c.valid) fg_correct_cells<DIMS, VEC, CFL>(g, c, rA_, hvec, p, vel_out, vel_copy, mean, lazy, cfl_mx);
+    if constexpr (CFL) {
+        __shared__ fg_real lds_cfl[FG_BLOCK / 64];
+        cfl_mx = fg_wave_max(cfl_mx);
+        if ((threadIdx.x & 63) == 0) lds_cfl[threadIdx.x >> 6] = cfl_mx;
+        __syncthreads();
+        if (threadIdx.x == 0) {
+            const unsigned tile = fg_xcd_remap(blockIdx.x, gridDim.x) % (unsigned)tiles;
+            cfl_part[(size_t)c.b * tiles + tile] = FG_FMAX(FG_FMAX(lds_cfl[0], lds_cfl[1]), FG_FMAX(lds_cfl[2], lds_cfl[3]));
+        }
     }
 }
 
@@ -397,6 +427,24 @@
     __syncthreads();
     return lds_fb[0] + lds_fb[1] + lds_fb[2] + lds_fb[3];
 }
+#if !FG_F64
+__device__ __forceinline__ float fg_dt_rule_env(const FgDtRule& rule, int e, float max_vel, double tr) {
+    float ts = 0.f;
+    if (tr > 0.0 && !(fabs(tr) <= 1e-8)) {
+        const double mv = (double)max_vel;
+        const double max_ts = (fabs(mv) <= 1e-8) ? tr : (double)rule.cfl / mv;
+        const double tsd = (max_ts >= tr) ? tr : tr / (double)(long long)ceil(tr / max_ts);
+        tr -= tsd;
+        ts = (float)tsd;
+    }
+    rule.t_rem[e] = tr;
+    rule.dt_out[e] = ts;
+    return ts;
+}
+__device__ __forceinline__ float fg_dt_rule_env(const FgDtRule& rule, int e, float max_vel) {
+    return fg_dt_rule_env(rule, e, max_vel, rule.reset ? rule.time_step : rule.t_rem[e]);
+}
+#endif
 __device__ __forceinline__ void fg_publish_max(fg_real* out_B, int32_t* done_B, fg_real* mirror_B, int b, fg_real mx, const FgPollOut& poll, int B,
                                                fg_real* flux_B = nullptr, fg_real* flux_mirror = nullptr, const FgDtRule& rule = FgDtRule{nullptr, nullptr, 0.f, 0.0, 0}) {
     const int lane = threadIdx.x & 63;
@@ -420,19 +468,7 @@
         if (poll.gran) {
             for (int e = lane; e < B; e += 64) {
                 const fg_bits mbits = __hip_atomic_exchange(reinterpret_cast<fg_bits*>(out_B) + e, (fg_bits)0, __ATOMIC_RELAXED, __HIP_MEMORY_SCOPE_AGENT);
-                if (rule.t_rem) {
-                    double tr = rule.reset ? rule.time_step : rule.t_rem[e];
-                    float ts = 0.f;
-                    if (tr > 0.0 && !(fabs(tr) <= 1e-8)) {
-                        const double mv = (double)__uint_as_float(mbits);
-                        const double max_ts = (fabs(mv) <= 1e-8) ? tr : (double)rule.cfl / mv;
-                        const double tsd = (max_ts >= tr) ? tr : tr / (double)(long long)ceil(tr / max_ts);
-                        tr -= tsd;
-                        ts = (float)tsd;
-                    }
-                    rule.t_rem[e] = tr;
-                    rule.dt_out[e] = ts;
-                }
+                if (rule.t_rem) fg_dt_rule_env(rule, e, __uint_as_float(mbits));
                 fg_poll_publish_word(poll, 12 * B + e, mbits);
                 if (flux_B) fg_poll_publish_word(poll, 13 * B + e, __hip_atomic_exchange(reinterpret_cast<fg_bits*>(flux_B) + e, (fg_bits)0, __ATOMIC_RELAXED, __HIP_MEMORY_SCOPE_AGENT));
                 atomicExch(done_B + e, 0);
@@ -691,12 +727,8 @@
 };
 struct FgBvelRw { fg_real* p[6]; };
 template <int DIMS>
-__global__ __launch_bounds__(FG_BLOCK) void k_balance_fluxes(FgGrid g, FgBounds bnd, FgBvelRw bvel_rw_, int free_mask,
-                                                              fg_real atol, const fg_real* __restrict__ dt, FgOutflowFold fold) {
-    const int b = blockIdx.x;
-    const fg_real dtb = fold.dt_n ? fold.dt_v[b] : (dt ? dt[b] : (fg_real)1);
-    if (fold.dt_n && threadIdx.x == 0) fold.dt_out[b] = dtb;
-    if ((dt || fold.dt_n) && !(dtb > 0.f)) return;
+__device__ __forceinline__ void fg_balance_env(const FgGrid& g, const FgBounds& bnd, const FgBvelRw& bvel_rw_, int free_mask, fg_real atol,
+                                               fg_real dtb, const FgOutflowFold& fold, int b) {
     if (fold.mask) {
         for (int face = 0; face < 2 * DIMS; ++face) {
             if (!((fold.mask >> face) & 1)) continue;
@@ -763,6 +795,80 @@
         for (int s = threadIdx.x; s < DIMS * slab_n; s += blockDim.x) v[s] *= scale;
     }
 }
+template <int DIMS>
+__global__ __launch_bounds__(FG_BLOCK) void k_balance_fluxes(FgGrid g, FgBounds bnd, FgBvelRw bvel_rw_, int free_mask,
+                                                              fg_real atol, const fg_real* __restrict__ dt, FgOutflowFold fold) {
+    const int b = blockIdx.x;
+    const fg_real dtb = fold.dt_n ? fold.dt_v[b] : (dt ? dt[b] : (fg_real)1);
+    if (fold.dt_n && threadIdx.x == 0) fold.dt_out[b] = dtb;
+    if ((dt || fold.dt_n) && !(dtb > 0.f)) return;
+    fg_balance_env<DIMS>(g, bnd, bvel_rw_, free_mask, atol, dtb, fold, b);
+}
+
+#if !FG_F64
+template <int DIMS>
+__global__ __launch_bounds__(FG_BLOCK) void k_step_head(FgGrid g, FgBounds bnd, const fg_real* __restrict__ cfl_part, int tiles,
+                                                         fg_real* __restrict__ out_B, int32_t* __restrict__ done_all, fg_real* flux_B, int flux,
+                                                         FgPollOut poll, FgDtRule rule, int balance, FgBvelRw bvel_rw_, int free_mask, fg_real atol,
+                                                         FgOutflowFold fold) {
+    const int b = blockIdx.x, B = (int)gridDim.x;
+    const double t_left = (threadIdx.x == 0 && !rule.reset) ? rule.t_rem[b] : rule.time_step;
+    fg_real mx = 0.f;
+    for (int t = threadIdx.x; t < tiles; t += FG_BLOCK) mx = FG_FMAX(mx, cfl_part[(size_t)b * tiles + t]);
+#pragma unroll
+    for (int f = 0; f < 2 * DIMS; ++f) {
+        if (!g.fixed[f]) continue;
+        const int ax = f >> 1;
+        const int slab_n = fg_slab_size(g, ax);
+        const int edge = (f & 1) ? ((ax == 0) ? g.nx - 1 : (ax == 1) ? g.ny - 1 : g.nz - 1) : 0;
+        for (int s = threadIdx.x; s < slab_n; s += FG_BLOCK) {
+            int i, j, k;
+            if constexpr (DIMS == 2) { k = 0; if (ax == 0) { i = edge; j = s; } else { j = edge; i = s; } }
+            else if (ax == 0) { i = edge; j = s % g.ny; k = s / g.ny; }
+            else if (ax == 1) { j = edge; i = s % g.nx; k = s / g.nx; }
+            else { k = edge; i = s % g.nx; j = s / g.nx; }
+            const fg_real rh[3] = {g.rh[0][i], g.rh[1][j], DIMS == 3 ? g.rh[2][k] : 1.f};
+#pragma unroll
+            for (int q = 0; q < DIMS; ++q)
+                mx = FG_FMAX(mx, FG_FABS(bnd.vel[f][((size_t)b * DIMS + q) * slab_n + s] * rh[q]));
+        }
+    }
+    __shared__ fg_real lds[4];
+    __shared__ fg_real lds_dt;
+    mx = fg_wave_max(mx);
+    if ((threadIdx.x & 63) == 0) lds[threadIdx.x >> 6] = mx;
+    __syncthreads();
+    double total = 0.0;
+    if (flux) total = fg_flux_balance_block<DIMS>(g, bnd, b);
+    fg_bits prev = 0, prevf = 0;
+    if (threadIdx.x == 0) {
+        mx = FG_FMAX(FG_FMAX(lds[0], lds[1]), FG_FMAX(lds[2], lds[3]));
+        lds_dt = fg_dt_rule_env(rule, b, mx, t_left);
+        prev = __hip_atomic_exchange(reinterpret_cast<fg_bits*>(out_B) + b, fg_real_bits(mx), __ATOMIC_RELAXED, __HIP_MEMORY_SCOPE_AGENT);
+        if (flux) prevf = __hip_atomic_exchange(reinterpret_cast<fg_bits*>(flux_B) + b, fg_real_bits((fg_real)total), __ATOMIC_RELAXED, __HIP_MEMORY_SCOPE_AGENT);
+    }
+    if (balance) {
+        __syncthreads();
+        const fg_real dtb = lds_dt;
+        if (dtb > 0.f) fg_balance_env<DIMS>(g, bnd, bvel_rw_, free_mask, atol, dtb, fold, b);
+    }
+    if (threadIdx.x < 64) {
+        const int lane = threadIdx.x;
+        int last_of_all = 0;
+        if (lane == 0) {
+            asm volatile("" ::"v"(prev), "v"(prevf));
+            last_of_all = (atomicAdd(done_all, 1) == B - 1);
+        }
+        if (__shfl(last_of_all, 0, 64)) {
+            for (int e = lane; e < B; e += 64) {
+                fg_poll_publish_word(poll, 12 * B + e, __hip_atomic_exchange(reinterpret_cast<fg_bits*>(out_B) + e, (fg_bits)0, __ATOMIC_RELAXED, __HIP_MEMORY_SCOPE_AGENT));
+                if (flux) fg_poll_publish_word(poll, 13 * B + e, __hip_atomic_exchange(reinterpret_cast<fg_bits*>(flux_B) + e, (fg_bits)0, __ATOMIC_RELAXED, __HIP_MEMORY_SCOPE_AGENT));
+            }
+            if (lane == 0) atomicExch(done_all, 0);
+        }
+    }
+}
+#endif
 
 inline unsigned fg_reduce_wgs(const fg_state* s) {
     if (s->reduce_wgs > 0) return (unsigned)s->reduce_wgs;
@@ -952,10 +1058,16 @@
     const FgLazyRef lz = lazy ? *lazy : FgLazyRef{nullptr, nullptr, nullptr};
     const double cb = (s->grid.dims == 3 ? 36.0 : 28.0) + (vel_copy ? 4.0 * s->grid.dims : 0.0) + ((mean && mean->sums) || (lazy && lazy->p_res) ? 4.0 : 0.0);
     const int slot_c = fg_prof_slot(s, FG_PK_CORRECT, nullptr, s->grid.B, cb * (double)s->grid.n, 5.0 * s->grid.dims * (double)s->grid.n, st);
+    const bool cfl = vel_copy && vel_copy == s->velocity && fg_step_head_grid(s);
     FG_DISPATCH(s, {
         const FgLaunch L = fg_launch_geometry<DIMS, VEC>(s->grid);
-        FG_LAUNCH_P(s, slot_c, (k_correct<DIMS, VEC>), L.grid, dim3(FG_BLOCK), 0, st, s->grid, dt, rA, hvec, p, vel_out, vel_copy, mr, lz,
-                    L.tiles_x, L.tiles_y, L.tiles);
+        if (cfl && L.tiles == s->cfl_tiles)
+            FG_LAUNCH_P(s, slot_c, (k_correct<DIMS, VEC, true>), L.grid, dim3(FG_BLOCK), 0, st, s->grid, dt, rA, hvec, p, vel_out, vel_copy, mr, lz,
+                        L.tiles_x, L.tiles_y, L.tiles, s->cfl_part);
+        else
+            FG_LAUNCH_P(s, slot_c, (k_correct<DIMS, VEC>), L.grid, dim3(FG_BLOCK), 0, st, s->grid, dt, rA, hvec, p, vel_out, vel_copy, mr, lz,
+                        L.tiles_x, L.tiles_y, L.tiles, (fg_real*)nullptr);
+        if (vel_copy) s->cfl_valid = (cfl && L.tiles == s->cfl_tiles) ? 1 : 0;
     });
     FG_HIP_CHECK(hipGetLastError());
     fg_htrace("correct_out");
@@ -1068,6 +1180,52 @@
     return FG_OK;
 }
 
+bool fg_step_head_grid(const fg_state* s) {
+#if FG_F64
+    (void)s;
+    return false;
+#else
+    if (s->grid.dims != 2 || s->dev_dt != 1 || !s->cfl_part || !s->t_rem_dev) return false;
+    for (int f = 0; f < 4; ++f) {
+        if (!s->grid.fixed[f]) continue;
+        if (((f >> 1) == 0 ? (long)s->grid.ny : (long)s->grid.nx) > 4 * FG_BLOCK) return false;
+    }
+    return true;
+#endif
+}
+
+int fg_launch_step_head(const fg_state* s, const FgBounds& bnd, hipStream_t st, FgPollOut poll, bool first, FgDtRule rule, int outflow_mask,
+                        fg_real atol, const fg_real* outflow_velm) {
+#if FG_F64
+    (void)bnd; (void)st; (void)poll; (void)first; (void)rule; (void)outflow_mask; (void)atol; (void)outflow_velm;
+    fg_set_error("fg_launch_step_head: fp32 build only");
+    return FG_ERR_UNSUPPORTED;
+#else
+    const int B = s->grid.B;
+    FG_REQUIRE(fg_step_head_ok(s) && poll.gran && rule.t_rem, FG_ERR_INVALID_ARG, "fg_launch_step_head: no valid per-tile maxima, or not the result-word form");
+    FG_REQUIRE(!outflow_mask || fg_outflow_folds(s, outflow_mask), FG_ERR_INVALID_ARG, "fg_launch_step_head: outflow slabs too large");
+    fg_real* out_B = s->scratch_B + B;
+    int32_t* done_B = reinterpret_cast<int32_t*>(out_B + B);
+    if (!s->maxvel_clean) FG_HIP_CHECK(hipMemsetAsync(out_B, 0, sizeof(fg_real) * B + sizeof(int32_t) * (B + 1), st));
+    s->maxvel_clean = 1;
+    FgOutflowFold fold;
+    fold = FgOutflowFold{};
+    if (outflow_mask) {
+        fold.mask = outflow_mask; fold.vel = s->velocity; fold.scal = s->scalar;
+        for (int a = 0; a < 3; ++a) fold.velm[a] = outflow_velm[a];
+        for (int f = 0; f < 6; ++f) { fold.bscal[f] = s->bscal[f]; fold.nsc[f] = (s->scalar && s->bscal[f]) ? s->cfg.n_scalars : 0; }
+    }
+    FgBvelRw rw;
+    for (int f = 0; f < 6; ++f) rw.p[f] = s->bvel[f];
+    const int slot_m = fg_prof_slot(s, FG_PK_MAXVEL, nullptr, B, 4.0 * (double)s->cfl_tiles, 2.0 * (double)s->cfl_tiles, st);
+    FG_LAUNCH_P(s, slot_m, k_step_head<2>, dim3(B), dim3(FG_BLOCK), 0, st, s->grid, bnd, s->cfl_part, s->cfl_tiles, out_B, done_B + B, s->scratch_B,
+                first ? 1 : 0, poll, rule, outflow_mask ? 1 : 0, rw, outflow_mask, atol, fold);
+    FG_HIP_CHECK(hipGetLastError());
+    s->step_head_launches += 1;
+    return FG_OK;
+#endif
+}
+
 bool fg_outflow_folds(const fg_state* s, int outflow_mask) {
     for (int f = 0; f < 2 * s->grid.dims; ++f) {
         if (!((outflow_mask >> f) & 1)) continue;
diff --git a/fluidgym_amd/csrc/fg_poisson.hip b/fluidgym_amd/csrc/fg_poisson.hip
--- a/fluidgym_amd/csrc/fg_poisson.hip
+++ b/fluidgym_amd/csrc/fg_poisson.hip
@@ -480,6 +480,7 @@
     }
     int first = 1;
     const int fused_reset = (a.reset_steps > 0 && a.reset_steps < 10) ? a.reset_steps : 10;
+    bool strag_open = s->fcg_spec && a.spec.fn && a.lazy_ok && c.mean_sums && s->ref64_outer == 0 && !s->double_fallback;
     for (int it = 0; it < a.max_iterations && !c.done; ++it) {
         if (int rc = fg_fcg_update_fwd(s, v, it, first, ns, st, o.marks_valid, it == 0 ? r0 : nullptr)) return rc;
         if (first) {
@@ -495,13 +496,22 @@
             const FgPollOut po = fg_poll_next(&s->poll);
             hipLaunchKernelGGL(k_cg_check, dim3((B + CG_CHECK_WAVES - 1) / CG_CHECK_WAVES), dim3(64 * CG_CHECK_WAVES), 0, st, s->cg_acc, s->flags, s->info_dev, s->info_pinned, a.tol, it,
                                n, B, final_pass, ns, po);
+            bool strag = false;
+            if (strag_open) {
+                FgCgOutcome ahead;
+                ahead.lazy_z = nullptr; ahead.mean_ready = true; ahead.marks_valid = o.marks_valid;
+                if (int rc = a.spec.fn(a.spec.ctx, ahead)) return rc;
+                strag = true; strag_open = false;
+                s->fcg_strag_spec += 1;
+            }
             fg_htrace("cg_check_launched");
             const int active = fg_poll_wait_active(&s->poll, po, 0, B, s->info_pinned, st);
             if (active < 0) return active;
             fg_htrace("cg_poll_done");
             c.info_fresh = true;
             c.done = (active == 0);
-            if (c.done) break;
+            if (c.done) { o.spec_done = strag; break; }
+            if (strag) s->fcg_strag_missed += 1;
         }
         if (it + 1 < a.max_iterations) {
             judge.it = it;
diff --git a/fluidgym_amd/csrc/fg_switches.h b/fluidgym_amd/csrc/fg_switches.h
--- a/fluidgym_amd/csrc/fg_switches.h
+++ b/fluidgym_amd/csrc/fg_switches.h
@@ -23,7 +23,7 @@
     X(FG_FD_FACFUSE, fd_facfuse, 1, INT, HANDLE, no, "1 (default): the first tridiagonal solve after 1/A changed makes the per-env row-mean factors itself (k_tridiag_y_lds<.., FAC>: same arithmetic, same bits); 0: k_fd_rowmean_factor as a launch of its own (A/B runs)") \
     X(FG_FD_ROWMEAN, fd_rowmean, 1, INT, HANDLE, bits, "1 (default): the fused pressure CG is preconditioned by the row-mean operator (per-env factors, one factorisation per PISO step); 0: the grid's A = 1 factors") \
     X(FG_FCG_FIRST, fcg_first, 1, ON, HANDLE, bits, "1 (default): the fused CG judges its first iterate from I'(0)'s dot products (k_fcg_check0) and stores no pressure when every env ends there; 0: the verdict on the updated residual (A/B runs, tests)") \
-    X(FG_FCG_SPEC, fcg_spec, 1, ON, HANDLE, no, "0: the corrector waits for the verdict on the first iterate instead of being launched behind the verdict kernel (A/B runs)") \
+    X(FG_FCG_SPEC, fcg_spec, 1, ON, HANDLE, no, "0: the corrector waits for the verdict on the first iterate, and for the verdict of the fused loop's first poll, instead of being launched behind the verdict kernel (A/B runs)") \
     X(FG_JAC_SPEC, jac_spec, 1, ON, HANDLE, no, "0: k_h and the divergence kernel of the first corrector wait for the verdict on the velocity sweeps instead of being launched behind the check kernel (A/B runs)") \
     X(FG_JAC_PREFACTOR, jac_prefactor, 1, ON, HANDLE, no, "0: the row-mean factors of the pressure preconditioner are made in front of the first tridiagonal solve instead of behind the sweeps' check kernel (A/B runs)") \
     X(FG_JAC_WARM, jac_warm, -1, TRI, HANDLE, bits, "start vector of the Jacobi sweeps of a step's velocity systems: 1 the block velocity, 0 the BiCGStab start vector (zero on the non-orthogonal branch); unset: the block velocity on on-chip grids of 2^17 cells and more (where it saves a pass)") \
@@ -32,7 +32,7 @@
     X(FG_JAC_SWEEPS, jac_sweeps, 0, INT, HANDLE, bits, "A/B runs: sweeps per pass of the Jacobi sweeps, clamped to what the region allows (unset: 4 / 6 / 8 for full rows, 8 / 12 for bands, by region depth)") \
     X(FG_FORCE_ZMARCH, zmarch_force, 0, INT, HANDLE, bits, "z-march chunk length of the 3-D Poisson kernels (tests on small grids; -1 = brick kernels)") \
     X(FG_ZMARCH_SB, zmarch_sb, -1, INT, HANDLE, no, "single-barrier ring of the z-march kernels: bit per mode forces it on with the caller's chunk length, 0 never, unset = where the launch is one full round") \
-    X(FG_DEV_DT, dev_dt, 1, INT, HANDLE, no, "0: fg_single_step waits for the CFL maxima and computes the adaptive sub-steps on the host before the PISO step, instead of the CFL kernel's last workgroup taking them on the device (FgDtRule: same doubles, same bits) and the host reading the maxima after the step (A/B runs)") \
+    X(FG_DEV_DT, dev_dt, 1, INT, HANDLE, no, "0: fg_single_step waits for the CFL maxima and computes the adaptive sub-steps on the host before the PISO step, instead of the CFL kernel's last workgroup taking them on the device (FgDtRule: same doubles, same bits) and the host reading the maxima after the step; 2: on the device, but always as the CFL pass over the velocity plus the balance launch, instead of k_step_head (one workgroup per env: the last corrector's per-tile maxima, guard, sub-step and balance in one launch) wherever those maxima are valid (A/B runs)") \
     X(FG_PROF_PERIOD, prof_period, 64, POS, HANDLE, no, "sampling period of the live kernel timing: every 64th launch of a kind is timed (8 cost the timed region ~5 %: a count kernel + two events per sample)")
 
 #define FG_MB_SWITCHES(X) \
diff --git a/profiles/step_head_ab.py b/profiles/step_head_ab.py
--- /dev/null
+++ b/profiles/step_head_ab.py
@@ -0,0 +1,52 @@
+import argparse
+import json
+import os
+import statistics
+import subprocess
+import sys
+
+ROOT = os.path.dirname(os.path.dirname(os.path.abspath(__file__)))
+
+
+def reading(parent_lib, extra, timeout):
+    env = dict(os.environ)
+    env.pop("FLUIDGYM_AMD_LIB", None)
+    if parent_lib:
+        env["FLUIDGYM_AMD_LIB"] = parent_lib
+    cmd = [sys.executable, os.path.join(ROOT, "bench.py"), "--gpus", "1", "--steps", "20", "--warmup", "5"] + extra
+    out = subprocess.run(cmd, env=env, cwd=ROOT, capture_output=True, text=True, timeout=timeout)
+    if out.returncode != 0:
+        raise SystemExit(f"bench.py failed ({out.returncode}):\n{out.stderr[-2000:]}")
+    line = json.loads(out.stdout.strip().splitlines()[-1])
+    return float(line["value"])
+
+
+def main():
+    ap = argparse.ArgumentParser()
+    ap.add_argument("--parent-lib", required=True, help="libfluidgym_hip.so built from the parent commit")
+    ap.add_argument("--readings", type=int, default=4)
+    ap.add_argument("--timeout", type=float, default=180.0, help="seconds per reading")
+    ap.add_argument("--out", default=os.path.join(ROOT, "profiles", "step_head_ab.json"))
+    args = ap.parse_args()
+    parent_lib = os.path.abspath(args.parent_lib)
+    assert os.path.exists(parent_lib), parent_lib
+    result = {"command": "bench.py --gpus 1 --steps 20 --warmup 5", "unit": "env-steps/s", "legs": {}}
+    for leg, extra in (("lanes2", []), ("lanes1", ["--lanes", "1"])):
+        rec = {"parent": [], "branch": []}
+        for _ in range(args.readings):
+            for side, lib in (("parent", parent_lib), ("branch", None)):
+                rec[side].append(round(reading(lib, extra, args.timeout), 1))
+                print(leg, side, rec[side][-1], flush=True)
+        mp, mb = statistics.median(rec["parent"]), statistics.median(rec["branch"])
+        spread = max(rec["parent"]) - min(rec["parent"])
+        rec.update(parent_median=mp, branch_median=mb, parent_spread=round(spread, 1), gain_percent=round(100.0 * (mb / mp - 1.0), 2),
+                   passes=bool(mb - mp > 0.5 * spread))
+        result["legs"][leg] = rec
+        with open(args.out, "w") as f:
+            json.dump(result, f, indent=1)
+            f.write("\n")
+    print(json.dumps(result))
+
+
+if __name__ == "__main__":
+    main()
```
